# JuliaGraphics/Hikari.jl

Hardware: AMD Instinct MI355X
Metric: Mrays/s (higher is better)
Workload: dtype f32

## Files before the change

hikari.jl_amd/_abi.py:

```python
import ctypes as C

c_f = C.c_float
c_i = C.c_int32
c_u = C.c_uint32
PF = C.POINTER(C.c_float)

HK_OK = 0
HK_ERR_INVALID, HK_ERR_DEVICE, HK_ERR_UNSUPPORTED = -1, -2, -3
HK_UNSET = -100

(HK_MAT_MATTE, HK_MAT_MIRROR, HK_MAT_GLASS, HK_MAT_CONDUCTOR, HK_MAT_COATED_DIFFUSE, HK_MAT_THIN_DIELECTRIC,
 HK_MAT_DIFFUSE_TRANSMISSION, HK_MAT_COATED_DIFFUSE_TRANSMISSION, HK_MAT_COATED_CONDUCTOR, HK_MAT_MIX,
 HK_MAT_FALLBACK) = range(11)
HK_MATF_REMAP_ROUGHNESS, HK_MATF_USE_ETA_K = 1, 2
(HK_LIGHT_POINT, HK_LIGHT_SPOT, HK_LIGHT_DIRECTIONAL, HK_LIGHT_SUN, HK_LIGHT_AMBIENT, HK_LIGHT_ENVIRONMENT,
 HK_LIGHT_DIFFUSE_AREA) = range(7)
HK_SPEC_RGB, HK_SPEC_ILLUMINANT = 0, 1
HK_TONEMAP_NONE, HK_TONEMAP_REINHARD, HK_TONEMAP_REINHARD_EXT, HK_TONEMAP_ACES, HK_TONEMAP_UNCHARTED2, HK_TONEMAP_FILMIC = range(6)
HK_MEDIUM_HOMOGENEOUS, HK_MEDIUM_GRID, HK_MEDIUM_RGB_GRID, HK_MEDIUM_NANOVDB = range(4)
HK_FILTER_BOX, HK_FILTER_TRIANGLE, HK_FILTER_GAUSSIAN, HK_FILTER_MITCHELL, HK_FILTER_LANCZOS = 1, 2, 3, 4, 5
HK_COHERENCE_NONE, HK_COHERENCE_SORTED, HK_COHERENCE_PER_TYPE = 0, 1, 2


class hk_texture(C.Structure):
# ... 20 lines not shown
class hk_medium_interface(C.Structure):
    _fields_ = [("material", c_i), ("inside", c_i), ("outside", c_i)]


class hk_tri_meta(C.Structure):
    _fields_ = [("medium_interface_idx", c_u), ("primitive_index", c_u), ("arealight_flat_idx_1based", c_u)]


class hk_light(C.Structure):
    _fields_ = [("kind", c_i), ("spectrum_kind", c_i), ("i_rgb", c_f * 4), ("poly", c_f * 3), ("illum_scale", c_f),
                ("scale", c_f), ("position", c_f * 3), ("direction", c_f * 3), ("world_to_light", c_f * 16),
                ("light_to_world", c_f * 16), ("cos_total_width", c_f), ("cos_falloff_start", c_f), ("v", c_f * 9),
                ("normal", c_f * 3), ("area", c_f), ("uv", c_f * 6), ("Le", hk_tex_rgba), ("two_sided", c_i),
                ("envmap", c_i)]


class hk_envmap(C.Structure):
    _fields_ = [("width", c_i), ("height", c_i), ("data", PF), ("rotation", c_f * 9), ("nu", c_i), ("nv", c_i),
                ("conditional_func", PF), ("conditional_cdf", PF), ("conditional_func_int", PF), ("marginal_func", PF),
                ("marginal_cdf", PF), ("marginal_func_int", c_f), ("_pad", c_i)]


class hk_medium(C.Structure):
    _fields_ = [("kind", c_i), ("sigma_a", c_f * 4), ("sigma_s", c_f * 4), ("Le", c_f * 4), ("g", c_f),
                ("sigma_scale", c_f), ("Le_scale", c_f), ("bounds_min", c_f * 3), ("bounds_max", c_f * 3),
                ("render_to_medium", c_f * 16), ("medium_to_render", c_f * 16), ("res", c_i * 3), ("density", PF),
                ("sigma_a_grid", PF), ("sigma_s_grid", PF), ("Le_grid", PF), ("majorant_res", c_i * 3),
                ("majorant", PF), ("max_density", c_f), ("nvdb_bytes", C.POINTER(C.c_uint8)), ("nvdb_size", C.c_int64),
                ("root_offset_1based", C.c_int64), ("upper_offset_1based", C.c_int64),
                ("lower_offset_1based", C.c_int64), ("leaf_offset_1based", C.c_int64), ("upper_count", c_i),
                ("lower_count", c_i), ("leaf_count", c_i), ("root_table_size", c_i), ("inv_mat", c_f * 9),
                ("vec", c_f * 3), ("index_bbox_min", c_i * 3), ("index_bbox_max", c_i * 3)]


class hk_scene_desc(C.Structure):
    _fields_ = [("n_triangles", c_i), ("n_materials", c_i), ("n_textures", c_i), ("n_media_interfaces", c_i),
                ("n_lights", c_i), ("n_envmaps", c_i), ("n_media", c_i), ("n_spectra", c_i), ("positions", PF),
                ("normals", PF), ("uvs", PF), ("tangents", PF), ("meta", C.POINTER(hk_tri_meta)),
                ("materials", C.POINTER(hk_material)), ("textures", C.POINTER(hk_texture)),
                ("media_interfaces", C.POINTER(hk_medium_interface)), ("lights", C.POINTER(hk_light)),
                ("envmaps", C.POINTER(hk_envmap)), ("media", C.POINTER(hk_medium)),
                ("spectra", C.POINTER(hk_pl_spectrum))]


class hk_tables(C.Structure):
    _fields_ = [("sobol_matrices", C.POINTER(c_u)), ("sobol_count", c_i), ("rgb2spec_res", c_i), ("cie_x", PF),
                ("cie_y", PF), ("cie_z", PF), ("rgb2spec_scale", PF), ("rgb2spec_coeffs", PF)]


class hk_integrator_params(C.Structure):
    _fields_ = [("max_depth", c_i), ("samples_per_pixel", c_i), ("russian_roulette_depth", c_i), ("regularize", c_i),
                ("material_coherence", c_i), ("max_component_value", c_f), ("filter_type", c_i),
                ("filter_radius", c_f * 2), ("filter_param1", c_f), ("filter_param2", c_f), ("accumulate_f64", c_i),
                ("sampler_seed", c_u), ("samples_per_pass", c_i)]


class hk_postprocess_params(C.Structure):
    _fields_ = [("exposure", c_f), ("tonemap", c_i), ("inv_gamma", c_f), ("apply_gamma", c_i), ("white_point", c_f),
                ("imaging_ratio", c_f), ("apply_wb", c_i), ("wb", c_f * 9), ("mask_escaped", c_i), ("bg", c_f * 3)]


class hk_denoise_params(C.Structure):
    _fields_ = [("iterations", c_i), ("sigma_color", c_f), ("sigma_normal", c_f), ("sigma_depth", c_f), ("use_variance", c_i)]


class hk_camera(C.Structure):
    _fields_ = [("raster_to_camera", c_f * 16), ("camera_to_world", c_f * 16), ("lens_radius", c_f),
                ("focal_distance", c_f), ("shutter_open", c_f), ("shutter_close", c_f), ("dx_camera", c_f * 3),
                ("dy_camera", c_f * 3)]


class hk_stats(C.Structure):
    _fields_ = [("rays_closest", C.c_uint64), ("rays_shadow", C.c_uint64), ("bvh_nodes_visited", C.c_uint64),
                ("tris_tested", C.c_uint64), ("hits_accepted", C.c_uint64), ("path_vertices", C.c_uint64),
                ("medium_collisions", C.c_uint64), ("light_bvh_nodes", C.c_uint64), ("seconds_trace", C.c_double),
                ("seconds_total", C.c_double), ("trace_launches", C.c_uint64), ("trace_nodes", C.c_uint64),
                ("trace_tris", C.c_uint64), ("shadow_nodes", C.c_uint64), ("shadow_tris", C.c_uint64),
                ("shadow_launches", C.c_uint64), ("shade_launches", C.c_uint64), ("seconds_shadow", C.c_double),
                ("seconds_shade", C.c_double), ("seconds_other", C.c_double), ("bytes_algorithmic_trace", C.c_uint64),
                ("bytes_algorithmic_shadow", C.c_uint64), ("bytes_algorithmic_shade", C.c_uint64), ("seconds_media", C.c_double),
                ("track_collisions", C.c_uint64), ("shadow_collisions", C.c_uint64), ("track_dda_steps", C.c_uint64),
                ("shadow_dda_steps", C.c_uint64), ("scatter_vertices", C.c_uint64), ("media_launches", C.c_uint64),
                ("bytes_algorithmic_media", C.c_uint64), ("seconds_select", C.c_double), ("select_launches", C.c_uint64),
                ("fused_passes", C.c_uint64), ("view_cache_hits", C.c_uint64)]


EXPORTED_SYMBOLS = [
    "hk_ctx_create", "hk_ctx_destroy", "hk_last_error", "hk_ctx_set_tables", "hk_scene_create", "hk_scene_destroy",
    "hk_integrator_create", "hk_integrator_destroy", "hk_film_create", "hk_film_destroy", "hk_film_clear", "hk_render",
    "hk_film_read_rgb", "hk_film_read_accum", "hk_film_accum_device_ptr", "hk_sync", "hk_stats_get", "hk_stats_reset",
    "hk_stats_enable_counters", "hk_trace_closest", "hk_test_sobol", "hk_test_camera", "hk_test_uplift",
    "hk_test_light_bvh", "hk_test_bsdf", "hk_film_postprocess", "hk_film_fill_aux", "hk_postprocess", "hk_test_light", "hk_scene_bvh_info", "hk_scene_light_bvh_copy",
    "hk_denoise", "hk_test_mix", "hk_test_medium", "hk_test_trace_lean",
    "hk_render_tile", "hk_comm_create", "hk_comm_unique_id", "hk_comm_create_rank", "hk_comm_destroy", "hk_film_reduce",
    "hk_ctx_set_option", "hk_ctx_get_option", "hk_trim_cache", "hk_flush", "hk_film_read_rgb_async", "hk_film_read_wait",
    "hk_film_pin_host", "hk_film_unpin_host", "hk_scene_set_transform", "hk_scene_update_materials", "hk_scene_update_lights", "hk_scene_update_envmap",
    "hk_film_update_aux", "hk_film_read_aux", "hk_film_present", "hk_film_present_async",
    "hk_scene_update_medium", "hk_scene_medium_copy", "hk_test_medium_bricks",
]
```

hikari.jl_amd/csrc/hk_ctx.cpp:

```cpp
#include "hk_host.h"

thread_local std::string g_err;
SlabCache g_slabs;

namespace hk {
static thread_local const Knobs* tl_knobs = nullptr;
const char* knob(const char* name) {
    if (!tl_knobs) return nullptr;
    auto it = tl_knobs->kv.find(name);
    return it == tl_knobs->kv.end() ? nullptr : it->second.c_str();
}
static const char* const KNOB_NAMES[] = {
    "HK_BATCH_PATHS_M", "HK_BVH_LEAF", "HK_BVH_BINS", "HK_QNODES", "HK_DEBUG_ALLOC", "HK_DELTA_ADVANCE", "HK_DYNAMIC_SEGMENTS", "HK_GREY", "HK_GREY_COMPACT", "HK_GREY_FLAT", "HK_MAX_PATHS_M",
    "HK_MID_LISTS", "HK_MID_PASS_PATHS_M", "HK_NODE_CACHE", "HK_NVDB_DENSE_MB", "HK_OVERLAP", "HK_PIPELINE", "HK_PIPELINE_AFTER", "HK_PIPELINE_MAX_PATHS_M", "HK_PRESELECT",
    "HK_SELECT_MIN_IDLE", "HK_SHADOW_FEED_ROUNDS", "HK_SHADOW_TRACK_BATCH", "HK_SMALL_PASS", "HK_SMALL_PASS_WAVES", "HK_SOBOL_LO_GB", "HK_SOBOL_TABLE_ONLY",
    "HK_STATE_CACHE_GB", "HK_STATE_SLAB", "HK_TICKET_SHARE", "HK_TRACK_ADVANCE", "HK_TRACK_EXTRA_ADVANCE", "HK_TRACK_MIN_PENDING", "HK_TRACK_POOL", "HK_TRACK_REFILL_IDLE",
    "HK_WALK_POOL", "HK_WALK_REFILL_IDLE", "HK_WALK_SPLIT", "HK_WAVES_PER_CU", "HK_READBACK_PIN", "HK_DEFER_EXTERNAL", "HK_SELECT_POOL", "HK_SMALL_PASS_FUSED", "HK_SMALL_PASS_MERGED", "HK_OCC_SCALE", "HK_ESCAPED_UNROLL", "HK_SHADOW_FINAL", "HK_TRI_PACK", "HK_LEAN_RECORDS", "HK_VIEW_CACHE", "HK_MAJORANT_BLOCK_VOXELS"};
static bool known_knob(const char* name) {
    for (const char* k : KNOB_NAMES)
        if (std::strcmp(k, name) == 0) return true;
    return false;
}
}
KnobScope::KnobScope(const hk::Knobs* k) : prev(hk::tl_knobs) { hk::tl_knobs = k; }
KnobScope::~KnobScope() { hk::tl_knobs = prev; }

void quiesce(hk_ctx* c) {
    if (!c) return;
    (void)hipStreamSynchronize(c->stream);
    if (c->aux) (void)hipStreamSynchronize(c->aux);
    for (auto& l : c->lanes)
        if (l.stream) (void)hipStreamSynchronize(l.stream);
}
int join_lanes(hk_ctx* c) {
    if (!c) return HK_OK;
    if (int e = flush_pending(c)) return e;
    if (!c->lanes_dirty) return HK_OK;
    for (auto& l : c->lanes)
        if (l.done) HIP_TRY(hipStreamWaitEvent(c->stream, l.done, 0));
    c->lanes_dirty = false;
    c->film_chain = false;
    if (c->have_span) HIP_TRY(hipEventRecord(c->ev_end, c->stream));
    return HK_OK;
}
hipEvent_t get_event(hk_ctx* c) {
    if (!c->event_pool.empty()) {
        hipEvent_t e = c->event_pool.back();
        c->event_pool.pop_back();
        return e;
    }
    hipEvent_t e;
    (void)hipEventCreate(&e);
    return e;
}
DCamera make_camera(const hk_camera& c) {
    DCamera d;
    std::memcpy(d.r2c, c.raster_to_camera, 64);
    std::memcpy(d.c2w, c.camera_to_world, 64);
    d.lens_radius = c.lens_radius;
    d.focal_distance = c.focal_distance;
    d.shutter_open = c.shutter_open;
    d.shutter_close = c.shutter_close;
    return d;
}

extern "C" const char* hk_last_error(void) { return g_err.c_str(); }

extern "C" int32_t hk_ctx_create(int32_t device_id, void* stream, hk_ctx** out) {
    if (!out) return fail(HK_ERR_INVALID, "out is null");
    int n = 0;
    HIP_TRY(hipGetDeviceCount(&n));
    if (device_id < 0 || device_id >= n) return fail(HK_ERR_INVALID, "bad device id");
    HIP_TRY(hipSetDevice(device_id));
    hk_ctx* c = new hk_ctx();
    c->device = device_id;
    c->stream = (hipStream_t)stream;
    hipDeviceProp_t prop;
    HIP_TRY(hipGetDeviceProperties(&prop, device_id));
    c->n_cu = prop.multiProcessorCount > 0 ? prop.multiProcessorCount : 256;
    c->own_stream_order = stream == nullptr;
    for (const char* name : hk::KNOB_NAMES)
        if (const char* e = std::getenv(name)) c->knobs.kv[name] = e;
    KnobScope knobs(&c->knobs);
    {
        c->waves_per_cu = hk::knob_int_in("HK_WAVES_PER_CU", 1, INT_MAX, 0);
        c->stat_rows = c->n_cu * 32 * 2;
        if (const char* e = hk::knob("HK_OVERLAP")) c->overlap = std::atoi(e) ? 1 : 0;
        else c->overlap = -1;
        if (const char* e = hk::knob("HK_STATE_CACHE_GB"))
            if (std::atol(e) >= 0) g_slabs.cap_bytes = (size_t)std::atol(e) << 30;
    }
    {
        std::vector<DStats> zero((size_t)c->stat_rows);
        std::memset(zero.data(), 0, zero.size() * sizeof(DStats));
        HIP_TRY(c->stats.upload(zero.data(), zero.size() * sizeof(DStats)));
    }
    HIP_TRY(hipEventCreate(&c->ev_begin));
    HIP_TRY(hipEventCreate(&c->ev_end));
// ... 81 lines not shown
    c->h_r2s_coeffs.assign(t->rgb2spec_coeffs, t->rgb2spec_coeffs + nco);
    c->r2s_host.res = res;
    c->r2s_host.scale = c->h_r2s_scale.data();
    c->r2s_host.coeffs = c->h_r2s_coeffs.data();
    HIP_TRY(c->r2s_scale.upload(t->rgb2spec_scale, res * 4));
    HIP_TRY(c->r2s_coeffs.upload(t->rgb2spec_coeffs, nco * 4));
    {
        const size_t R = (size_t)res;
        std::vector<float> pts(3 * R * R * R * 4);
        for (size_t m = 0; m < 3; ++m)
            for (size_t z = 0; z < R; ++z)
                for (size_t y = 0; y < R; ++y)
                    for (size_t x = 0; x < R; ++x) {
                        float* o = &pts[((((m * R + z) * R + y) * R) + x) * 4];
                        for (size_t k = 0; k < 3; ++k) o[k] = t->rgb2spec_coeffs[m + 3 * (z + R * (y + R * (x + R * k)))];
                        o[3] = 0.0f;
                    }
        HIP_TRY(c->r2s_points.upload(pts.data(), pts.size() * 4));
        bool sorted = true;
        for (int i = 1; i < res; ++i)
            if (!(t->rgb2spec_scale[i - 1] <= t->rgb2spec_scale[i])) sorted = false;
        c->tables.rgb2spec_sorted = sorted ? 1 : 0;
    }
    bool closed = true;
    {
        uint32_t col = 0x80000000u;
        for (int b = 0; b < 52; ++b) {
            uint32_t d0 = b < 32 ? (0x80000000u >> b) : 0u;
            if (t->sobol_matrices[b] != d0) closed = false;
            if (b % 32 == 0) col = 0x80000000u;
            if (t->sobol_matrices[52 + b] != col) closed = false;
            col ^= col >> 1;
        }
    }
    c->tables.sobol = closed ? nullptr : c->sobol.as<uint32_t>();
    c->tables.cie = c->cie.as<float>();
    c->tables.rgb2spec_scale = c->r2s_scale.as<float>();
    c->tables.rgb2spec_coeffs = c->r2s_coeffs.as<float>();
    c->tables.rgb2spec_res = res;
    c->tables.rgb2spec_points = c->r2s_points.as<float4>();
    c->have_tables = true;
    c->tables_epoch++;
    return HK_OK;
}

extern "C" int32_t hk_sync(hk_ctx* c) {
    if (!c) return fail(HK_ERR_INVALID, "null ctx");
    HIP_TRY(hipSetDevice(c->device));
    if (int e = join_lanes(c)) return e;
    HIP_TRY(hipStreamSynchronize(c->stream));
    if (c->aux) HIP_TRY(hipStreamSynchronize(c->aux));
    return HK_OK;
}
extern "C" int32_t hk_stats_enable_counters(hk_ctx* c, int32_t flags) {
    if (!c) return fail(HK_ERR_INVALID, "null ctx");
    if (int e = join_lanes(c)) return e;
    c->count_nodes = (flags & 1) ? 1 : 0;
    c->time_kernels = (flags & 2) ? 1 : 0;
    return HK_OK;
}
extern "C" int32_t hk_stats_reset(hk_ctx* c) {
    if (!c) return fail(HK_ERR_INVALID, "null ctx");
    HIP_TRY(hipSetDevice(c->device));
    if (int e = join_lanes(c)) return e;
    HIP_TRY(hipStreamSynchronize(c->stream));
    HIP_TRY(hipMemset(c->stats.p, 0, (size_t)c->stat_rows * sizeof(DStats)));
    for (auto& l : c->lanes)
        if (l.stats.p) HIP_TRY(hipMemset(l.stats.p, 0, (size_t)c->stat_rows * sizeof(DStats)));
    for (auto& e : c->trace_events) {
        c->event_pool.push_back(e.first);
        c->event_pool.push_back(e.second);
    }
    c->trace_events.clear();
    for (auto& v : c->class_events) {
        for (auto& e : v) {
            c->event_pool.push_back(e.first);
            c->event_pool.push_back(e.second);
        }
        v.clear();
    }
    c->seconds_trace = c->seconds_total = 0.0;
    c->trace_launches = c->shadow_launches = c->shade_launches = c->media_launches = c->select_launches = 0;
    c->fused_passes = c->view_cache_hits = 0;
    c->have_span = false;
    return HK_OK;
}
extern "C" int32_t hk_stats_get(hk_ctx* c, hk_stats* out) {
    if (!c || !out) return fail(HK_ERR_INVALID, "null argument");
    HIP_TRY(hipSetDevice(c->device));
    if (int e = join_lanes(c)) return e;
    HIP_TRY(hipStreamSynchronize(c->stream));
    DStats h{};
    {
        std::vector<const void*> blocks{c->stats.p};
        for (const auto& l : c->lanes)
            if (l.stats.p) blocks.push_back(l.stats.p);
        std::vector<DStats> rows((size_t)c->stat_rows * blocks.size());
        for (size_t b = 0; b < blocks.size(); ++b)
            HIP_TRY(hipMemcpy(rows.data() + b * (size_t)c->stat_rows, blocks[b], (size_t)c->stat_rows * sizeof(DStats), hipMemcpyDeviceToHost));
        for (const DStats& r : rows) {
            h.rays_closest += r.rays_closest;
            h.rays_shadow += r.rays_shadow;
            h.nodes += r.nodes;
            h.tris += r.tris;
            h.hits += r.hits;
            h.vertices += r.vertices;
            h.collisions += r.collisions;
            h.light_nodes += r.light_nodes;
            h.sh_nodes += r.sh_nodes;
            h.sh_tris += r.sh_tris;
            h.sh_collisions += r.sh_collisions;
            h.nvdb_collisions += r.nvdb_collisions;
            h.sh_nvdb_collisions += r.sh_nvdb_collisions;
            h.dda_steps += r.dda_steps;
            h.sh_dda_steps += r.sh_dda_steps;
            h.scatter_vertices += r.scatter_vertices;
            h.sc_light_nodes += r.sc_light_nodes;
#ifdef HK_DEBUG_UTIL
            for (int k = 0; k < 32; ++k) h.dbg[k] += r.dbg[k];
#endif
        }
#ifdef HK_DEBUG_UTIL
        for (int k = 0; k < 16; ++k)
            if (h.dbg[2 * k]) std::fprintf(stderr, "HK_DEBUG_UTIL[%d]: %.3f of %llu lane-slots\n", k, (double)h.dbg[2 * k + 1] / (double)h.dbg[2 * k], h.dbg[2 * k]);
#endif
    }
    double tr = 0.0;
    for (auto& e : c->trace_events) {
        float ms = 0.0f;
        if (hipEventElapsedTime(&ms, e.first, e.second) == hipSuccess) tr += ms * 1e-3;
    }
    double total = 0.0;
    if (c->have_span) {
        float ms = 0.0f;
        if (hipEventElapsedTime(&ms, c->ev_begin, c->ev_end) == hipSuccess) total = ms * 1e-3;
    }
    std::memset(out, 0, sizeof *out);
    out->rays_closest = h.rays_closest;
    out->rays_shadow = h.rays_shadow;
    out->bvh_nodes_visited = h.nodes;
    out->tris_tested = h.tris;
    out->hits_accepted = h.hits;
    out->path_vertices = h.vertices;
    out->medium_collisions = h.collisions + h.sh_collisions;
    out->track_collisions = h.collisions;
    out->shadow_collisions = h.sh_collisions;
    out->track_dda_steps = h.dda_steps;
    out->shadow_dda_steps = h.sh_dda_steps;
    out->scatter_vertices = h.scatter_vertices;
    out->light_bvh_nodes = h.light_nodes + h.sc_light_nodes;
    out->seconds_trace = tr;
    out->seconds_total = total;
    out->trace_launches = c->trace_launches;
    out->trace_nodes = h.nodes;
    out->trace_tris = h.tris;
    out->shadow_nodes = h.sh_nodes;
    out->shadow_tris = h.sh_tris;
    out->bvh_nodes_visited = h.nodes + h.sh_nodes;
    out->tris_tested = h.tris + h.sh_tris;
    out->shadow_launches = c->shadow_launches;
    out->shade_launches = c->shade_launches;
    out->media_launches = c->media_launches;
    double cls[6] = {0, 0, 0, 0, 0, 0};
    for (int k = 1; k < 6; ++k)
        for (auto& e : c->class_events[k]) {
            float ms = 0.0f;
            if (hipEventElapsedTime(&ms, e.first, e.second) == hipSuccess) cls[k] += ms * 1e-3;
        }
    out->seconds_shadow = cls[1];
    out->seconds_shade = cls[2] + cls[5];
    out->seconds_other = cls[3];
    out->seconds_media = cls[4];
    out->seconds_select = cls[5];
    out->select_launches = c->select_launches;
    out->fused_passes = c->fused_passes;
    out->view_cache_hits = c->view_cache_hits;
    {
        const uint64_t hits_closest = h.hits < h.rays_closest ? h.hits : h.rays_closest;
        out->bytes_algorithmic_trace = h.rays_closest * (32 + 16) + 64 * h.nodes + 36 * h.tris + 96 * hits_closest;
        out->bytes_algorithmic_shadow = h.rays_shadow * (32 + 16) + 64 * h.sh_nodes + 36 * h.sh_tris;
        out->bytes_algorithmic_shade = h.vertices * (2 * 104 + 64 + 96) + 60 * h.light_nodes;
        out->bytes_algorithmic_media = h.collisions * 36 + h.nvdb_collisions * (84 - 36) + 4 * h.dda_steps + h.scatter_vertices * (2 * 104 + 96) + 60 * h.sc_light_nodes;
        out->bytes_algorithmic_shadow += h.sh_collisions * 36 + h.sh_nvdb_collisions * (84 - 36) + 4 * h.sh_dda_steps;
    }
    return HK_OK;
}
```

hikari.jl_amd/csrc/hk_device.h:

```cpp
#pragma once
#include <hip/hip_runtime.h>
#include <math.h>
#include <stdint.h>

#include "hk_types.h"

#include "hk_nanovdb.h"

#define HKD __device__ __forceinline__

namespace hkd {

static constexpr float PI_F = 3.14159265358979323846f;
static constexpr float INF_F = __builtin_huge_valf();

struct v3 {
    float x, y, z;
};
struct v2 {
    float x, y;
};
HKD v3 mk3(float x, float y, float z) { return v3{x, y, z}; }
HKD v2 mk2(float x, float y) { return v2{x, y}; }
HKD v3 operator+(v3 a, v3 b) { return mk3(a.x + b.x, a.y + b.y, a.z + b.z); }
// ... 238 lines not shown
    return murmur64a_words<2>(w);
}
struct SobolCtx {
    int px, py;
    int pix_slot, x0, y0, tiles_x;
    int sample_idx;
    const uint32_t* mats;
    const uint2* hi;
    const uint16_t* lo;
    int lo_rows;
    uint32_t lo_row_stride;
    int hi_rows, hi_stride;
    int log2_spp, n_digits;
    uint32_t seed;
};
HKD void sobol_ctx_tables(SobolCtx& c, const DSobol& s, const uint32_t* mats, int sample_idx, int pix_slot, int k) {
    c.sample_idx = sample_idx;
    c.pix_slot = pix_slot;
    c.mats = mats;
    const bool cached = s.hi_table != nullptr && pix_slot >= 0 && ((unsigned)sample_idx >> s.log2_spp) == 0u;
    c.hi = cached ? s.hi_table + pix_slot : nullptr;
    const bool low = cached && s.lo_table != nullptr && k >= 0 && (unsigned)(s.lo_offset + k) < (unsigned)s.lo_count;
    c.lo = low ? s.lo_table + ((size_t)pix_slot * s.lo_count + (size_t)(s.lo_offset + k)) : nullptr;
    c.lo_rows = low ? s.lo_rows : 0;
    c.lo_row_stride = (uint32_t)s.hi_stride * (uint32_t)s.lo_count;
    c.hi_rows = s.hi_rows;
    c.hi_stride = s.hi_stride;
    c.log2_spp = s.log2_spp;
    c.n_digits = s.n_base4_digits;
    c.seed = s.seed;
}
HKD SobolCtx sobol_ctx(const DSobol& s, const uint32_t* mats, int px, int py, int sample_idx, int pix_slot = -1, int k = -1) {
    SobolCtx c;
    c.px = px;
    c.py = py;
    c.x0 = c.y0 = 0;
    c.tiles_x = 1;
    sobol_ctx_tables(c, s, mats, sample_idx, pix_slot, k);
    return c;
}
HKD SobolCtx sobol_ctx_slot(const DSobol& s, const uint32_t* mats, int x0, int y0, int tiles_x, int pix_slot, int k, int sample_idx) {
    SobolCtx c;
    c.px = c.py = 0;
    c.x0 = x0;
    c.y0 = y0;
    c.tiles_x = tiles_x;
    sobol_ctx_tables(c, s, mats, sample_idx, pix_slot, k);
    return c;
}
HKD uint64_t sobol_morton_base(const SobolCtx& c) {
    int px = c.px, py = c.py;
    if (px == 0) {
        const int tile = c.pix_slot >> 6, l = c.pix_slot & 63;
        const int ty = tile / c.tiles_x, tx = tile - ty * c.tiles_x;
        px = c.x0 + tx * 8 + (l & 7) + 1;
        py = c.y0 + ty * 8 + (l >> 3) + 1;
    }
    const uint64_t m = (left_shift2((uint64_t)(uint32_t)py) << 1) | left_shift2((uint64_t)(uint32_t)px);
    return (m << c.log2_spp) | (uint64_t)(int64_t)c.sample_idx;
}
template <bool TABLE_ONLY = false>
HKD uint64_t sobol_index(const SobolCtx& c, int dim) {
    const int row = sobol_row(dim);
    if (TABLE_ONLY) return ((uint64_t)c.hi[(size_t)row * c.hi_stride].x << c.log2_spp) | (uint64_t)c.lo[(size_t)row * c.lo_row_stride];
    if (c.hi != nullptr && row >= 0 && row < c.hi_rows) {
        const uint2 e = c.hi[(size_t)row * c.hi_stride];
        if (row < c.lo_rows) return ((uint64_t)e.x << c.log2_spp) | (uint64_t)c.lo[(size_t)row * c.lo_row_stride];
        return zsobol_sample_index_cached(sobol_morton_base(c), dim, c.log2_spp, e.x, e.y);
    }
    return zsobol_sample_index(sobol_morton_base(c), dim, c.log2_spp, c.n_digits);
}
template <bool TABLE_ONLY = false>
HKD float sobol_1d(const SobolCtx& c, int dim) {
    uint64_t idx = sobol_index<TABLE_ONLY>(c, dim);
    uint32_t h = (uint32_t)zsobol_hash(dim + 1, c.seed);
    return sobol_sample(idx, 0, h, c.mats);
}
template <bool TABLE_ONLY = false>
HKD v2 sobol_2d(const SobolCtx& c, int dim) {
    uint64_t idx = sobol_index<TABLE_ONLY>(c, dim);
    uint64_t bits = zsobol_hash(dim + 2, c.seed);
    return mk2(sobol_sample(idx, 0, (uint32_t)bits, c.mats), sobol_sample(idx, 1, (uint32_t)(bits >> 32), c.mats));
}

HKD float jl_sin_kernel(double y) {
    const double S1 = -0.16666666641626524, S2 = 0.008333329385889463, S3 = -0.00019839334836096632, S4 = 2.718311493989822e-6;
    double z = y * y, w = z * z;
    double r = S3 + z * S4, s = z * y;
    return (float)((y + s * (S1 + z * S2)) + s * w * r);
}
HKD float jl_cos_kernel(double y) {
    const double C0 = -0.499999997251031, C1 = 0.04166662332373906, C2 = -0.001388676377460993, C3 = 2.439044879627741e-5;
    double z = y * y, w = z * z;
    double r = C2 + z * C3;
    return (float)(((1.0 + z * C0) + w * C1) + (w * z) * r);
}
HKD int jl_rem_pio2(float x, double& y) {
    const double PI = 3.141592653589793;
    const double xd = (double)x, ax = fabs(xd);
    if (ax <= PI * 5 / 4) {
        if (ax <= PI * 3 / 4) {
            y = x > 0 ? xd - PI / 2 : xd + PI / 2;
            return x > 0 ? 1 : -1;
        }
        y = x > 0 ? xd - PI : xd + PI;
        return x > 0 ? 2 : -2;
    }
    if (ax <= PI * 9 / 4) {
        if (ax <= PI * 7 / 4) {
            y = x > 0 ? xd - 3 * (PI / 2) : xd + 3 * (PI / 2);
            return x > 0 ? 3 : -3;
        }
        y = x > 0 ? xd - 2 * PI : xd + 2 * PI;
        return x > 0 ? 4 : -4;
    }
    const double fn = rint(xd * 6.36619772367581382433e-01);
    const double r = xd - fn * 1.57079631090164184570e+00, w = fn * 1.58932547735281966916e-08;
    y = r - w;
    return (int)fn;
}
HKD void jl_sincos(float x, float& s, float& c) {
    const float ax = fabsf(x);
    if (ax < 0.7853982f) {
        s = ax < 0.00034526698f ? x : jl_sin_kernel((double)x);
        c = ax < 0.00024414062f ? 1.0f : jl_cos_kernel((double)x);
        return;
    }
    if (!(ax < 2.1e8f)) {
        s = sinf(x);
        c = cosf(x);
        return;
    }
    double y;
    const int n = jl_rem_pio2(x, y) & 3;
    const float sk = jl_sin_kernel(y), ck = jl_cos_kernel(y);
    s = n == 0 ? sk : (n == 1 ? ck : (n == 2 ? -sk : -ck));
    c = n == 0 ? ck : (n == 1 ? -sk : (n == 2 ? -ck : sk));
}

HKD v2 concentric_sample_disk(v2 u) {
    float ox = 2.0f * u.x - 1.0f, oy = 2.0f * u.y - 1.0f;
    float sx = ox + 1.0e-10f, sy = oy + 1.0e-10f;
    bool xl = fabsf(ox) > fabsf(oy);
    float r = xl ? ox : oy;
    float theta = xl ? ((oy / sx) * PI_F) / 4.0f : PI_F / 2.0f - ((ox / sy) * PI_F) / 4.0f;
    float st, ct;
    jl_sincos(theta, st, ct);
    return mk2(r * ct, r * st);
}
HKD v3 cosine_sample_hemisphere(v2 u) {
    v2 d = concentric_sample_disk(u);
    float z = sqrtf(maxf(0.0f, 1.0f - d.x * d.x - d.y * d.y));
    return mk3(d.x, d.y, z);
}

HKD float atanh_sampler(float x) { return 0.34657359027997264f * __builtin_amdgcn_logf((1.0f + x) * __builtin_amdgcn_rcpf(1.0f - x)); }
HKD float cosh_sampler(float y) {
    const float e = __builtin_amdgcn_exp2f(1.4426950408889634f * y);
    return 0.5f * (e + __builtin_amdgcn_rcpf(e));
}
HKD float visible_wavelengths_pdf(float l) {
    if (l < 360.0f || l > 830.0f) return 0.0f;
    float c = cosh_sampler(0.0072f * (l - 538.0f));
    return 0.0039398042f / (c * c);
}
HKD float sample_visible_wavelength(float u) { return 538.0f - 138.888889f * atanh_sampler(0.85691062f - 1.82750197f * u); }
// ... 254 lines not shown
}
HKD void filter_sample(const DFilter& f, v2 u, float& px, float& py, float& weight) {
    if (f.type == HK_FILTER_BOX) {
        px = lerpf(-f.rx, f.rx, u.x);
        py = lerpf(-f.ry, f.ry, u.y);
        weight = 1.0f;
        return;
    }
    if (f.type == HK_FILTER_TRIANGLE) {
        px = sample_tent(u.x, f.rx);
        py = sample_tent(u.y, f.ry);
        weight = 1.0f;
        return;
    }
    int ny = f.ny, nx = f.nx;
    int o = clampi(find_interval20(f.marginal_cdf, u.y, ny), 1, ny);
    float du = u.y - f.marginal_cdf[o - 1];
    float diff = f.marginal_cdf[o] - f.marginal_cdf[o - 1];
    du = diff > 0.0f ? du / diff : 0.0f;
    float pdf_y = f.func_integral > 0.0f ? f.marginal_func[o - 1] / f.func_integral : 0.0f;
    py = lerpf(f.dmin_y, f.dmax_y, ((float)(o - 1) + du) / (float)ny);
    float row_integral = f.marginal_func[o - 1];
    const float* row = f.conditional_cdf + (size_t)(o - 1) * (nx + 1);
    int ox = clampi(find_interval20(row, u.x, nx), 1, nx);
    float dux = u.x - row[ox - 1];
    float diffx = row[ox] - row[ox - 1];
    dux = diffx > 0.0f ? dux / diffx : 0.0f;
    float fval = f.func[(size_t)(o - 1) * nx + (ox - 1)];
    float pdf_x = row_integral > 0.0f ? fval / row_integral : 0.0f;
    px = lerpf(f.dmin_x, f.dmax_x, ((float)(ox - 1) + dux) / (float)nx);
    float pdf = pdf_x * pdf_y;
    weight = pdf > 0.0f ? fval / pdf : 0.0f;
}
HKD v3 xform_point(const float* m, v3 p) {
    float x = m[0] * p.x + m[1] * p.y + m[2] * p.z + m[3];
    float y = m[4] * p.x + m[5] * p.y + m[6] * p.z + m[7];
    float z = m[8] * p.x + m[9] * p.y + m[10] * p.z + m[11];
    float w = m[12] * p.x + m[13] * p.y + m[14] * p.z + m[15];
    if (w == 1.0f) return mk3(x, y, z);
    float inv = 1.0f / w;
    return mk3(x * inv, y * inv, z * inv);
}
HKD v3 xform_vector(const float* m, v3 v) {
    return mk3(m[0] * v.x + m[1] * v.y + m[2] * v.z, m[4] * v.x + m[5] * v.y + m[6] * v.z, m[8] * v.x + m[9] * v.y + m[10] * v.z);
}
HKD void generate_ray(const DCamera& cam, v2 film, v2 lens, float time_u, v3& ro, v3& rd, float& time) {
    v3 pc = xform_point(cam.r2c, mk3(film.x, film.y, 0.0f));
    v3 o = mk3(0.0f, 0.0f, 0.0f);
    v3 d = normalize(pc);
    if (cam.lens_radius > 0) {
        v2 dsk = concentric_sample_disk(lens);
        float plx = cam.lens_radius * dsk.x, ply = cam.lens_radius * dsk.y;
        float t = -cam.focal_distance / d.z;
        v3 pf = o + d * t;
        o = mk3(plx, ply, 0.0f);
        d = normalize(pf - o);
    }
    time = lerpf(cam.shutter_open, cam.shutter_close, time_u);
    ro = xform_point(cam.c2w, o);
    rd = normalize(xform_vector(cam.c2w, d));
}

HKD bool intersect_triangle(v3 o, v3 d, float t_max, v3 v0, v3 e1, v3 e2, float& t, float& u, float& v) {
    v3 p = cross(d, e2);
    float det = dot(e1, p);
    if (det == 0.0f) return false;
    float inv = 1.0f / det;
    v3 s = o - v0;
    u = dot(s, p) * inv;
    if (!(u >= 0.0f) || u > 1.0f) return false;
    v3 q = cross(s, e1);
    v = dot(d, q) * inv;
    if (!(v >= 0.0f) || u + v > 1.0f) return false;
    t = dot(e2, q) * inv;
    return t > 0.0f && t < t_max;
}

struct HitRec {
    float t;
    int prim;
    float u, v;
};

struct RaySlab {
    float ix, iy, iz, ox, oy, oz, eps3;
};
HKD RaySlab ray_slab(v3 o, v3 d) {
    RaySlab r;
    r.ix = clampf(1.0f / d.x, -1e30f, 1e30f), r.iy = clampf(1.0f / d.y, -1e30f, 1e30f), r.iz = clampf(1.0f / d.z, -1e30f, 1e30f);
    r.ox = -o.x * r.ix, r.oy = -o.y * r.iy, r.oz = -o.z * r.iz;
    r.eps3 = 3.0f * (2.4e-7f * fmaxf(fmaxf(fabsf(r.ix) < 1e30f ? fabsf(r.ox) : 0.0f, fabsf(r.iy) < 1e30f ? fabsf(r.oy) : 0.0f), fabsf(r.iz) < 1e30f ? fabsf(r.oz) : 0.0f));
    return r;
}
HKD RaySlab ray_slab_grid(const DScene& sc, v3 o, v3 d) {
    RaySlab r = ray_slab(o, d);
    r.ox = fmaf(sc.q_base[0], r.ix, r.ox), r.oy = fmaf(sc.q_base[1], r.iy, r.oy), r.oz = fmaf(sc.q_base[2], r.iz, r.oz);
    r.ix *= sc.q_cell[0], r.iy *= sc.q_cell[1], r.iz *= sc.q_cell[2];
    return r;
}
typedef float hk_f2 __attribute__((ext_vector_type(2)));
typedef float hk_f4v __attribute__((ext_vector_type(4)));
typedef int hk_i2v __attribute__((ext_vector_type(2)));
typedef __attribute__((address_space(3))) hk_f4v lds_float4;
typedef __attribute__((address_space(3))) hk_i2v lds_int2;
struct NodeCache {
    const lds_float4* box;
    const lds_int2* child;
    int nc;
    const lds_float4* tri;
    int nt;
};
template <int NC = 0, bool QN = false>
HKD void node_step(const DScene& sc, const RaySlab& rs, float t_best, int* __restrict__ stack, int lane, int& cur, int& sp, const NodeCache& cache = NodeCache()) {
    float4 A, B, C;
    int c0, c1;
    if (QN && !(NC > 0 && cur < cache.nc)) {
        const uint4* qp = reinterpret_cast<const uint4*>(sc.qnodes) + 2 * (size_t)cur;
        const uint4 P = qp[0], Q = qp[1];
        A = make_float4((float)(P.x & 0xffffu), (float)(P.x >> 16), (float)(P.y & 0xffffu), (float)(P.y >> 16));
        B = make_float4((float)(P.z & 0xffffu), (float)(P.z >> 16), (float)(P.w & 0xffffu), (float)(P.w >> 16));
        C = make_float4((float)(Q.x & 0xffffu), (float)(Q.x >> 16), (float)(Q.y & 0xffffu), (float)(Q.y >> 16));
        c0 = (int)Q.z, c1 = (int)Q.w;
    } else if (NC > 0 && cur < cache.nc) {
        const hk_f4v a = cache.box[cur], b = cache.box[NC + cur], c = cache.box[2 * NC + cur];
        const hk_i2v ch = cache.child[cur];
        A = make_float4(a.x, a.y, a.z, a.w), B = make_float4(b.x, b.y, b.z, b.w), C = make_float4(c.x, c.y, c.z, c.w);
        c0 = ch.x, c1 = ch.y;
        asm volatile("" : "+v"(c0));
    } else {
        const float4* np = reinterpret_cast<const float4*>(sc.nodes) + 4 * (size_t)cur;
        A = np[0], B = np[1], C = np[2];
        const float4 D = np[3];
        c0 = __float_as_int(D.x), c1 = __float_as_int(D.y);
    }
    const hk_f2 IX = {rs.ix, rs.ix}, IY = {rs.iy, rs.iy}, IZ = {rs.iz, rs.iz}, OX = {rs.ox, rs.ox}, OY = {rs.oy, rs.oy}, OZ = {rs.oz, rs.oz};
    const hk_f2 x0 = __builtin_elementwise_fma((hk_f2){A.x, A.y}, IX, OX), y0 = __builtin_elementwise_fma((hk_f2){A.z, A.w}, IY, OY);
    const hk_f2 z0 = __builtin_elementwise_fma((hk_f2){B.x, B.y}, IZ, OZ), x1 = __builtin_elementwise_fma((hk_f2){B.z, B.w}, IX, OX);
    const hk_f2 y1 = __builtin_elementwise_fma((hk_f2){C.x, C.y}, IY, OY), z1 = __builtin_elementwise_fma((hk_f2){C.z, C.w}, IZ, OZ);
    const float n0 = fmaxf(fmaxf(fminf(x0.x, x0.y), fminf(y0.x, y0.y)), fmaxf(fminf(z0.x, z0.y), 0.0f));
    const float f0 = fminf(fminf(fmaxf(x0.x, x0.y), fmaxf(y0.x, y0.y)), fminf(fmaxf(z0.x, z0.y), t_best));
    const float n1 = fmaxf(fmaxf(fminf(x1.x, x1.y), fminf(y1.x, y1.y)), fmaxf(fminf(z1.x, z1.y), 0.0f));
    const float f1 = fminf(fminf(fmaxf(x1.x, x1.y), fmaxf(y1.x, y1.y)), fminf(fmaxf(z1.x, z1.y), t_best));
    const bool h0 = n0 <= fmaf(f0, 1.00003f, rs.eps3);
    const bool h1 = n1 <= fmaf(f1, 1.00003f, rs.eps3);
    const bool both = h0 && h1, any = h0 || h1;
    const bool first0 = n0 <= n1;
    const bool pick0 = h0 & (!h1 | first0);
    const int near_c = pick0 ? c0 : c1;
    if (both) stack[sp * 64 + lane] = pick0 ? c1 : c0;
    sp += both ? 1 : 0;
    const bool pop = !any && sp > 0;
    sp -= pop ? 1 : 0;
    int popped = (int)0x80000000;
    if (pop) popped = stack[sp * 64 + lane];
    cur = any ? near_c : popped;
}

template <int MODE, bool COUNT, int NC = 0, int NT = 0>
HKD HitRec traverse(const DScene& sc, v3 o, v3 d, float t_max, int* __restrict__ stack, int lane, unsigned& n_nodes, unsigned& n_tris, bool& opaque_hit,
                    const NodeCache& cache = NodeCache()) {
    HitRec best;
    best.t = t_max;
    best.prim = -1;
    best.u = best.v = 0.0f;
    opaque_hit = false;
    if (sc.n_tris == 0) return best;
    const RaySlab rs = ray_slab(o, d);
    int sp = 0;
    int cur = sc.root_ref;
    const int DONE = (int)0x80000000;
    while (cur != DONE) {
        for (;;) {
            const unsigned long long in_nodes = __ballot(cur >= 0);
            if (in_nodes == 0ull) break;
// ... 1266 lines not shown
```

hikari.jl_amd/csrc/hk_host.h:

```cpp
#pragma once
#include <hip/hip_runtime.h>

#include <climits>
#include <cstddef>
#include <cmath>
#include <cstdio>
#include <cstdlib>
#include <cstring>
#include <limits>
#include <map>
#include <memory>
#include <mutex>
#include <string>
#include <unordered_map>
#include <vector>

#include "bvh_build.h"
#include "hikari_mi355x.h"
#include "hk_launch.h"
#include "hk_nanovdb.h"
#include "hk_types.h"

#pragma GCC visibility push(hidden)

// ... 70 lines not shown
    void trim(int dev) {
        std::vector<void*> drop;
        {
            std::lock_guard<std::mutex> g(m);
            for (int i = (int)free_list.size() - 1; i >= 0; --i)
                if (dev < 0 || free_list[i].dev == dev) {
                    drop.push_back(free_list[i].p);
                    free_list.erase(free_list.begin() + i);
                }
        }
        for (void* q : drop) (void)hipFree(q);
    }
};
extern SlabCache g_slabs;
struct DevBuf {
    void* p = nullptr;
    size_t bytes = 0;
    int slab_dev = -1;
    void release() {
        if (p && slab_dev >= 0) {
            g_slabs.give(slab_dev, p, bytes);
        } else if (p)
            (void)hipFree(p);
        p = nullptr, bytes = 0, slab_dev = -1;
    }
    ~DevBuf() { release(); }
    hipError_t alloc(size_t n) {
        release();
        bytes = n;
        if (n == 0) return hipSuccess;
        hipError_t e = hipMalloc(&p, n);
        if (e != hipSuccess) {
            (void)hipGetLastError();
            g_slabs.trim(-1);
            e = hipMalloc(&p, n);
        }
        if (e != hipSuccess) p = nullptr, bytes = 0;
        return e;
    }
    hipError_t alloc_slab(int dev, size_t n) {
        release();
        size_t got = 0;
        if (void* q = g_slabs.take(dev, n, got)) {
            p = q, bytes = got, slab_dev = dev;
            return hipSuccess;
        }
        const hipError_t e = alloc(n);
        if (e == hipSuccess) slab_dev = dev;
        return e;
    }
    hipError_t upload(const void* src, size_t n) {
        hipError_t e = alloc(n ? n : 4);
        if (e != hipSuccess) return e;
        if (n) e = hipMemcpy(p, src, n, hipMemcpyHostToDevice);
        return e;
    }
    template <class T>
    T* as() const {
        return reinterpret_cast<T*>(p);
    }
};

struct hk_ctx {
    int device = 0;
    hk::Knobs knobs;
    bool own_stream_order = true;
    hipStream_t stream = nullptr;
    hipStream_t aux = nullptr;
    hipEvent_t ev_fork = nullptr, ev_join = nullptr;
    int overlap = -1;
    int small_streak = 0;
    int n_cu = 256;
    int waves_per_cu = 0;
    int stat_rows = 8192;
    DevBuf sobol, cie, r2s_scale, r2s_coeffs, r2s_points, stats;
    DTables tables{};
    bool have_tables = false;
    unsigned tables_epoch = 0;
    std::vector<float> h_r2s_scale, h_r2s_coeffs;
    hk::RGB2Spec r2s_host;
    int count_nodes = 0, time_kernels = 0;
    unsigned long long fused_passes = 0;
    unsigned long long view_cache_hits = 0;
    std::vector<std::pair<hipEvent_t, hipEvent_t>> trace_events;
    std::vector<std::pair<hipEvent_t, hipEvent_t>> class_events[6];
    uint64_t shadow_launches = 0, shade_launches = 0, media_launches = 0, select_launches = 0;
    std::vector<hipEvent_t> event_pool;
    hipEvent_t ev_begin = nullptr, ev_end = nullptr;
    bool have_span = false;
    double seconds_trace = 0.0, seconds_total = 0.0;
    uint64_t trace_launches = 0;
    DStats host_stats{};
    struct Lane {
        hipStream_t stream = nullptr;
        hipEvent_t done = nullptr;
        DevBuf stats;
    };
    enum { MAX_LANES = 16 };
    Lane lanes[MAX_LANES];
    int next_lane = 0;
    struct Pending {
        bool active = false;
        hk_scene* sc = nullptr;
        hk_integrator* I = nullptr;
        hk_film* film = nullptr;
        hk_camera cam{};
        int first = 0, n = 0, stride = 1, x0 = 0, y0 = 0, x1 = 0, y1 = 0, calls = 0;
    } pending;
    bool lanes_dirty = false;
    bool film_chain = false;
    hipEvent_t ev_main = nullptr, ev_film = nullptr;
};

void quiesce(hk_ctx* c);
int flush_pending(hk_ctx* c);
int join_lanes(hk_ctx* c);
hipEvent_t get_event(hk_ctx* c);
DCamera make_camera(const hk_camera& c);

struct hk_scene {
    hk_ctx* ctx = nullptr;
    DevBuf nodes, qnodes, leaf_tris, positions, normals, uvs, tangents, meta, tri_shade, materials, textures, spectra, mis, lights, lnodes, trails, infinite;
    DevBuf envmaps;
    DevBuf media;
    DScene d{};
    uint32_t kinds_mask = 0;
    int n_materials = 0;
    int bvh_nodes = 0, bvh_leaf_tris = 0, bvh_depth = 0;
    hk::LightBVH lbvh;
    std::vector<hk_material> h_materials;
    std::vector<hk_light> h_lights;
    std::vector<DEnvMap> h_envmaps;
    int n_textures = 0, n_spectra = 0;
    std::vector<int> level_start;
    DevBuf base_pos, base_nrm, base_tan, slot_of_prim;
    bool have_base = false;
    bool qnodes_built = false;
    enum { XF_BLOCK = 1024 };
    std::vector<float> block_box;
    struct Xf {
        int end;
        bool identity;
        float m[12];
    };
    std::map<int, Xf> xf;
    struct Staging {
        void* host = nullptr;
        size_t bytes = 0;
        hipEvent_t ev = nullptr;
    };
    std::vector<Staging> staging;
    struct Medium {
        hk_medium rec{};
        DMedium d{};
        DevBuf *majorant = nullptr, *maj_zero = nullptr, *density = nullptr, *rgb[3] = {nullptr, nullptr, nullptr};
        DevBuf *nvdb = nullptr, *blocks = nullptr, *bricks = nullptr;
    };
    std::vector<Medium> h_media;
    std::vector<std::unique_ptr<DevBuf>> owned;
    DevBuf& own() {
        owned.emplace_back(new DevBuf());
        return *owned.back();
    }
    ~hk_scene() {
        for (auto& st : staging) {
            if (st.ev) (void)hipEventSynchronize(st.ev), (void)hipEventDestroy(st.ev);
            if (st.host) (void)hipHostFree(st.host);
        }
    }
};
void bake_material(const hk::RGB2Spec& t, const hk_material& m, DMaterial& o);
bool material_alpha_tested(const hk_material& m);
void bake_light(const hk::RGB2Spec& r2s, const hk_light& l, DLight& o);
std::string check_medium_record(const hk_medium& m);
void bake_medium_fields(const hk::RGB2Spec& r2s, const hk_medium& m, DMedium& o);
struct NvdbPlan {
    int nvb_min[3] = {0, 0, 0}, nvb_dim[3] = {0, 0, 0};
    float background = 0.0f;
    long long total = 0;
    std::vector<uint2> table;
    bool bricks = false;
    void fill(DMedium& o) const;
};
int plan_nanovdb(const hk_medium& m, NvdbPlan& p);
struct MediaClasses {
    int media_mask = 0, all_grey = 0, grey_pool = 0, grey_bricks = 0;
};
MediaClasses classify_media(const std::vector<DMedium>& dmed, int n_media);
inline size_t light_table_capacity(int n_lights) { return n_lights > 0 ? (size_t)n_lights : 1; }

struct hk_film {
    hk_ctx* ctx = nullptr;
    int width = 0, height = 0;
    bool f64 = false;
    DevBuf own;
    void* accum = nullptr;
    bool external = false;
    bool exposed = false;
    DevBuf readback;
    float* staging[2] = {nullptr, nullptr};
    int staging_next = 0, staging_last = -1;
    bool read_in_flight = false;
    hipEvent_t ev_read = nullptr;
    void* last_out = nullptr;
    void* pinned_user = nullptr;
    bool pinned_explicit = false;
    void* pin_failed = nullptr;
    DevBuf guides, albedo;
    DevBuf frame[2], variance;
    bool have_aux = false;
};

struct hk_integrator {
    hk_ctx* ctx = nullptr;
    hk_integrator_params p{};
    DFilter filter{};
    DevBuf f_func, f_mcdf, f_mfunc, f_ccdf;
    DPathState st{};
    std::vector<std::unique_ptr<DevBuf>> bufs;
    int st_capacity = 0, st_depth = 0, st_media = -1;
    DPathGen cam_gen{};
    bool cam_unfit = false;
    std::string view_key;
    bool mid_pass = false;
    int slab_mode = 0;
    void* slab_base = nullptr;
    size_t slab_off = 0;
    DevBuf sobol_table;
    int sobol_rows = 0, sobol_stride = 0, sobol_log2 = -1, sobol_digits = -1, sobol_x0 = -1, sobol_y0 = -1, sobol_tiles_x = -1;
    DevBuf sobol_lo;
    int lo_rows = 0, lo_base = -1, lo_sample_stride = -1, lo_count = 0;
    struct StateSet {
        DPathState st{};
        std::vector<std::unique_ptr<DevBuf>> bufs;
        int st_capacity = 0, st_depth = 0, st_media = -1;
        DPathGen cam_gen{};
        bool cam_unfit = false;
        std::string view_key;
    };
    std::vector<StateSet> lane_sets;
    void swap_set(StateSet& o) {
        std::swap(st, o.st);
        std::swap(bufs, o.bufs);
        std::swap(st_capacity, o.st_capacity);
        std::swap(st_depth, o.st_depth);
        std::swap(st_media, o.st_media);
        std::swap(cam_gen, o.cam_gen);
        std::swap(cam_unfit, o.cam_unfit);
        std::swap(view_key, o.view_key);
    }
};
int ceil_log2(long v);
DSobol make_sobol(const hk_integrator_params& p, int w, int h);

struct hk_comm {
    std::vector<hk_ctx*> ctxs;
    std::vector<void*> comms;
    int world = 1;
};

#pragma GCC visibility pop
```

hikari.jl_amd/csrc/hk_kernels.hip:

```cpp
#include <hip/hip_runtime.h>
#include <type_traits>
#include <cstdlib>
#include <cstdio>

#include "hikari_mi355x.h"
#include "hk_device.h"

using namespace hkd;

namespace {

__device__ __forceinline__ int lane_id() { return (int)(threadIdx.x & 63); }

struct WaveQ {
    uint32_t* base;
    int count;
};
__device__ __forceinline__ int global_wave() {
    const int w = (int)(threadIdx.x >> 6), b = (int)blockIdx.x;
    if (blockDim.x == 1024 && (gridDim.x & 7) == 0) return ((((b >> 3) * 4 + (w >> 2)) * 8 + (b & 7)) << 2) + (w & 3);
    if (blockDim.x == 512 && (gridDim.x & 7) == 0) return ((((b >> 3) * 2 + (w >> 2)) * 8 + (b & 7)) << 2) + (w & 3);
    return b * (int)(blockDim.x >> 6) + w;
}
__device__ __forceinline__ int physical_waves() { return (int)(gridDim.x * (blockDim.x >> 6)); }
// ... 278 lines not shown
        slot_to_pixel(fr, pix, px, py, inside);
        const int dim = sobol_row_dim(row);
        uint64_t m = (left_shift2((uint64_t)(uint32_t)(py + 1)) << 1) | left_shift2((uint64_t)(uint32_t)(px + 1));
        uint64_t morton = m << sob.log2_spp;
        const int pow2 = sob.log2_spp & 1;
        const uint64_t dmix = 0x55555555ull * (uint64_t)(int64_t)dim;
        uint64_t hi = zsobol_digits(morton, dmix, pow2, sob.n_base4_digits - 1, zsobol_first_pixel_digit(sob.log2_spp));
        table[i] = make_uint2((uint32_t)(hi >> sob.log2_spp), zsobol_top_perms(morton, dmix, sob.log2_spp));
    }
}

struct SegQueues {
    int n;
    int depth[HK_MAX_KINDS + 6], q[HK_MAX_KINDS + 6];
};
#define HK_LIST_SPLIT 8
__global__ void __launch_bounds__(1024) k_segment_lists(DPathState st, SegQueues qs) {
    __shared__ int wave_total[16];
    const int d = qs.depth[blockIdx.x], q = qs.q[blockIdx.x];
    const int* __restrict__ cnt = st.counters + (size_t)(d * Q_COUNT + q) * st.n_waves;
    int* __restrict__ out = st.seg_list + (size_t)(d * Q_COUNT + q) * st.n_waves;
    const int lane = (int)(threadIdx.x & 63), wave = (int)(threadIdx.x >> 6);
    const int share = (st.n_waves + HK_LIST_SPLIT - 1) / HK_LIST_SPLIT;
    const int begin = (int)blockIdx.y * share < st.n_waves ? (int)blockIdx.y * share : st.n_waves, end = begin + share < st.n_waves ? begin + share : st.n_waves;
    int mine = 0;
    for (int i = (int)threadIdx.x; i < begin; i += 1024) mine += cnt[i] != 0 ? 1 : 0;
    for (int off = 32; off > 0; off >>= 1) mine += __shfl_down(mine, off);
    if (lane == 0) wave_total[wave] = mine;
    __syncthreads();
    int base = 0;
    for (int w = 0; w < 16; ++w) base += wave_total[w];
    for (int start = begin; start < end; start += 1024) {
        const int i = start + (int)threadIdx.x;
        const bool nz = i < end && cnt[i] != 0;
        const unsigned long long m = __ballot(nz);
        __syncthreads();
        if (lane == 0) wave_total[wave] = __popcll(m);
        __syncthreads();
        int before = 0, total = 0;
        for (int w = 0; w < 16; ++w) {
            const int t = wave_total[w];
            before += w < wave ? t : 0;
            total += t;
        }
        if (nz) out[base + before + __popcll(m & ((1ull << lane) - 1ull))] = i;
        base += total;
    }
    if (blockIdx.y == HK_LIST_SPLIT - 1 && threadIdx.x == 0) st.seg_list_n[d * Q_COUNT + q] = base;
}

__global__ void __launch_bounds__(256) k_sobol_lo_table(DSobol sob, DFrame fr, uint16_t* table, int rows, int base, int stride, int count) {
    const long groups = count >> 4;
    const long total = (long)rows * fr.n_pixels_padded * groups;
    const uint32_t mask = (1u << sob.log2_spp) - 1u;
    const int pow2 = sob.log2_spp & 1;
    for (long i = (long)blockIdx.x * blockDim.x + threadIdx.x; i < total; i += (long)gridDim.x * blockDim.x) {
        const long rp = i / groups;
        const int q = (int)(i - rp * groups);
        const int row = (int)(rp / fr.n_pixels_padded), pix = (int)(rp - (long)row * fr.n_pixels_padded);
        int px, py;
        bool inside;
        slot_to_pixel(fr, pix, px, py, inside);
        const int dim = sobol_row_dim(row);
        const uint64_t dmix = 0x55555555ull * (uint64_t)(int64_t)dim;
        const uint64_t m = ((left_shift2((uint64_t)(uint32_t)(py + 1)) << 1) | left_shift2((uint64_t)(uint32_t)(px + 1))) << sob.log2_spp;
        const uint2 e = sob.hi_table[(size_t)row * sob.hi_stride + pix];
        uint32_t v[16];
        const int s0 = base + 16 * q * stride;
        if (stride == 1 && pow2 == 0 && (s0 & 15) == 0 && sob.log2_spp >= 4) {
            const uint64_t morton = m | (uint64_t)(uint32_t)s0;
            const uint32_t upper = (uint32_t)zsobol_sample_index_cached(morton, dim, sob.log2_spp, e.x, e.y) & mask & ~15u;
            const int p1 = zsobol_perm_index(morton >> 4, dmix);
            for (int d1 = 0; d1 < 4; ++d1) {
                const uint32_t hi = upper | ((uint32_t)zsobol_permute_digit(p1, d1) << 2);
                const int p0 = zsobol_perm_index((morton | ((uint64_t)d1 << 2)) >> 2, dmix);
                for (int d0 = 0; d0 < 4; ++d0) v[4 * d1 + d0] = hi | (uint32_t)zsobol_permute_digit(p0, d0);
            }
        } else {
            for (int t = 0; t < 16; ++t) v[t] = (uint32_t)zsobol_sample_index_cached(m | (uint64_t)(uint32_t)(s0 + t * stride), dim, sob.log2_spp, e.x, e.y) & mask;
        }
        uint4* out = reinterpret_cast<uint4*>(table) + 2 * i;
        out[0] = make_uint4(v[0] | (v[1] << 16), v[2] | (v[3] << 16), v[4] | (v[5] << 16), v[6] | (v[7] << 16));
        out[1] = make_uint4(v[8] | (v[9] << 16), v[10] | (v[11] << 16), v[12] | (v[13] << 16), v[14] | (v[15] << 16));
    }
}

__device__ __forceinline__ void camera_body(const DPathState& st, const DFrame& fr, const DTables& T, const DFilter& flt, const DCamera& cam, const DSobol& sob, const SegTickets& src) {
    const int total = fr.n_pixels_padded * fr.samples_in_pass;
    const int n_chunks = total >> 6;
    const DPathGen g0 = st.gen_cam;
    HK_FOR_EACH_SEGMENT_FROM(gw, st, src) {
    WavePos out{0};
    const size_t seg = (size_t)gw * st.wave_cap;
    for (int chunk = gw; chunk < n_chunks; chunk += st.n_waves) {
        int slot = chunk * 64 + lane_id();
        int pix, k;
        split_slot(fr, (uint32_t)slot, pix, k);
        int px, py;
        bool active;
        slot_to_pixel(fr, pix, px, py, active);
        const size_t p = seg + (size_t)wp_push(out, active);
        if (active) {
            int sample_idx = fr.first_sample + k * fr.sample_stride;
            int x = px + 1, y = py + 1;
            SobolCtx sc = sobol_ctx(sob, T.sobol, x, y, sample_idx, pix, k);
            float wavelength_u = sobol_1d(sc, 1);
            v2 jit = sobol_2d(sc, 3);
            float time_u = 0.0f;
            v2 lens = mk2(0.0f, 0.0f);
            if (cam.lens_radius > 0) {
                time_u = sobol_1d(sc, 4);
                lens = sobol_2d(sc, 6);
            }
            float fx, fy, fw;
            filter_sample(flt, jit, fx, fy, fw);
            S4 lambda, pdf;
            sample_wavelengths_visible(wavelength_u, lambda, pdf);
            v2 pfilm = mk2((float)x + 0.5f + fx, (float)fr.height - (float)y + 1.0f + 0.5f + fy);
            v3 ro, rd;
            float time;
            generate_ray(cam, pfilm, lens, time_u, ro, rd, time);
            if (!st.const_origin || p == seg) stream_st(&g0.ray_o[p], make_float4(ro.x, ro.y, ro.z, INF_F));
            stream_st(&g0.ray_d[p], make_float4(rd.x, rd.y, rd.z, (st.compact && !fr.implicit_ones) ? 1.0f : 0.0f));
            st_lambda(g0, p, lambda);
            if (!fr.implicit_ones) {
                st4(&g0.beta[p], s4(1.0f));
                st_ru_rl(g0, p, s4(1.0f), s4(1.0f), st.compact != 0);
            }
            st_meta(st, g0, p, (uint32_t)(*st.initial_medium + 1) << 16, (uint32_t)slot);
            stream_st(&st.lambda_s[slot], lambda);
            stream_st(&st.L[slot], s4(0.0f));
            stream_st(&st.filter_w[slot], fw);
        }
    }
    if (lane_id() == 0) *count_ptr(st, 0, Q_RAY, gw) = out.count;
    }
}
__global__ void __launch_bounds__(256) k_camera(DPathState st, DFrame fr, DTables T, DFilter flt, DCamera cam, DSobol sob, int initial_medium) {
    camera_body(st, fr, T, flt, cam, sob, seg_open(st, ticket_ptr(st, st.ticket_rows - 1, TK_CAMERA), st.dynamic_segments != 0, -1, 0));
}

template <int NC, int BLOCK, bool QN = false>
HKD NodeCache node_cache_fill(const DScene& sc, float4* __restrict__ box, int2* __restrict__ child) {
    NodeCache c;
    c.box = (const lds_float4*)box, c.child = (const lds_int2*)child;
    c.tri = nullptr, c.nt = 0;
    c.nc = sc.n_nodes < NC ? sc.n_nodes : NC;
    if (NC > 0) {
        for (int i = threadIdx.x; i < c.nc; i += BLOCK) {
            if (QN) {
                const uint4* qp = reinterpret_cast<const uint4*>(sc.qnodes) + 2 * (size_t)i;
                const uint4 P = qp[0], Q = qp[1];
                box[i] = make_float4((float)(P.x & 0xffffu), (float)(P.x >> 16), (float)(P.y & 0xffffu), (float)(P.y >> 16));
                box[NC + i] = make_float4((float)(P.z & 0xffffu), (float)(P.z >> 16), (float)(P.w & 0xffffu), (float)(P.w >> 16));
                box[2 * NC + i] = make_float4((float)(Q.x & 0xffffu), (float)(Q.x >> 16), (float)(Q.y & 0xffffu), (float)(Q.y >> 16));
                child[i] = make_int2((int)Q.z, (int)Q.w);
                continue;
            }
            const float4* np = reinterpret_cast<const float4*>(sc.nodes) + 4 * (size_t)i;
            const float4 D = np[3];
            box[i] = np[0], box[NC + i] = np[1], box[2 * NC + i] = np[2];
            child[i] = make_int2(__float_as_int(D.x), __float_as_int(D.y));
        }
        __syncthreads();
    }
    return c;
// ... 1428 lines not shown
}

__device__ __forceinline__ bool escaped_one(const DPathState& st, const DScene& sc, const DTables& T, const DPathGen& g, bool ones, uint32_t slot, S4& fin, uint32_t& pslot, int depth) {
    const uint2 meta = ld_meta(st, g, slot, depth);
    pslot = meta.y;
    S4 lambda = ld_lambda(st, g, slot, meta.y);
    S4 Le = s4(0.0f);
    v3 rd = mk3(0, 0, 1);
    bool have_dir = false;
    for (int li = 0; li < sc.n_lights; ++li) {
        const DLight& l = sc.lights[li];
        if (l.kind == HK_LIGHT_AMBIENT) Le = Le + l.scale * light_spectrum(l, lambda);
        if (l.kind == HK_LIGHT_ENVIRONMENT) {
            if (!have_dir) {
                float4 D = g.ray_d[slot];
                rd = mk3(D.x, D.y, D.z);
                have_dir = true;
            }
            float4 t = env_eval(sc.envmaps[l.Le_tex], rd);
            Le = Le + eval_illuminant(coef_illuminant(T, t.x * l.Le_rgba[0], t.y * l.Le_rgba[1], t.z * l.Le_rgba[2]), lambda);
        }
    }
    S4 beta = ld_throughput(g.beta, slot, ones);
    S4 contribution = beta * Le;
    if (is_black(contribution)) return false;
    uint32_t fl = meta.x;
    int pdepth = (int)(fl & 0xff);
    bool specular = (fl >> 8) & 1u;
    S4 r_u = ld_ru(g, slot, ones, st.compact != 0);
    if (pdepth == 0 || specular)
        fin = contribution / average(r_u);
    else {
        float choice = sc.n_lights > 0 ? 1.0f / (float)sc.n_lights : 0.0f;
        float light_pdf = 0.0f;
        if (sc.n_envmaps > 0)
            for (int li = 0; li < sc.n_lights; ++li) {
                const DLight& l = sc.lights[li];
                light_pdf = light_pdf + (l.kind == HK_LIGHT_ENVIRONMENT ? env_pdf_li(sc.envmaps[l.Le_tex], rd) : 0.0f);
            }
        S4 rl = ld_rl(g, slot, ones, st.compact != 0) * choice * light_pdf;
        float den = average(r_u + rl);
        fin = den > 1e-10f ? contribution / den : contribution / average(r_u);
    }
    return true;
}
template <int UNROLL>
__device__ __forceinline__ void escaped_body(const DPathState& st, const DScene& sc, const DTables& T, int depth, int implicit_ones, const SegTickets& src) {
    HK_FOR_EACH_SEGMENT_FROM(gw, st, src) {
    const uint32_t* __restrict__ queue = st.escaped_q + (size_t)gw * st.wave_cap;
    const int n = *count_ptr(st, depth, Q_ESCAPED, gw);
    const DPathGen g = gen_at(st, depth);
    const bool ones = depth == 0 && implicit_ones;
    int i = lane_id();
    if (UNROLL == 2) {
        for (; i + 64 < n; i += 128) {
            const uint32_t slot0 = queue[i], slot1 = queue[i + 64];
            S4 fin0, fin1;
            uint32_t p0, p1;
            const bool a0 = escaped_one(st, sc, T, g, ones, slot0, fin0, p0, depth);
            const bool a1 = escaped_one(st, sc, T, g, ones, slot1, fin1, p1, depth);
            S4 L0 = s4(0.0f), L1 = s4(0.0f);
            if (a0) L0 = ld4(&st.L[p0]);
            if (a1) L1 = ld4(&st.L[p1]);
            if (a0) st4(&st.L[p0], L0 + fin0);
            if (a1) st4(&st.L[p1], L1 + fin1);
        }
    }
    for (; i < n; i += 64) {
        S4 fin;
        uint32_t pslot;
        if (escaped_one(st, sc, T, g, ones, queue[i], fin, pslot, depth)) st4(&st.L[pslot], ld4(&st.L[pslot]) + fin);
    }
    }
}
template <int UNROLL>
__global__ void __launch_bounds__(256) k_escaped(DPathState st, DScene sc, DTables T, int depth, int implicit_ones) {
    escaped_body<UNROLL>(st, sc, T, depth, implicit_ones, seg_open(st, ticket_ptr(st, depth, TK_ESCAPED), st.dynamic_segments != 0, depth, Q_ESCAPED));
}

#define HK_PRESELECT_MIN 64
#ifndef HK_SELECT_MIN_IDLE
#define HK_SELECT_MIN_IDLE 24
#endif
template <bool FT>
__global__ void __launch_bounds__(256) k_light_select(DPathState st, DScene sc, DTables T, DFrame fr, DSobol sob, int depth, uint32_t kinds_mask, int min_idle, DStats* stats) {
    const int lane = lane_id();
    const unsigned long long lt_mask = (1ull << lane) - 1ull;
    unsigned n_lnodes = 0;
    const DPathGen g = gen_at(st, depth);
    const int base_dim = 6 + 7 * depth;
    const int ninf = sc.num_infinite_lights, nbvh = sc.num_bvh_lights;
    const bool has_bvh = nbvh > 0;
    const float p_inf = (float)ninf / (float)(ninf + (has_bvh ? 1 : 0));
    HK_FOR_EACH_WAVE_SEGMENT(gw, st, ticket_ptr(st, depth, TK_SELECT), depth, Q_RAY) {
        int kind = -1, n = 0, cursor = 0;
        const uint32_t* __restrict__ queue = st.mat_q;
        bool more = true;
        bool busy = false, done = false;
        uint32_t slot = 0, bits = 0, child = 0;
        int ni = 1, res_light = 0, lvl = 0;
        float ub = 0.0f, pmf = 0.0f, res_pmf = 0.0f;
        v3 p = mk3(0, 0, 0), nn = mk3(0, 0, 1);
        for (;;) {
            const unsigned long long run_m = __ballot(busy && !done);
            if (run_m == 0ull || (64 - __popcll(run_m) >= min_idle && (cursor < n || more))) {
                if (busy && done) {
                    st.sel_light[slot] = make_uint2((uint32_t)res_light, __float_as_uint(res_pmf));
                    busy = false;
                }
                while (more && cursor >= n) {
                    ++kind;
                    while (kind < HK_MAX_KINDS && !(kinds_mask & (1u << kind))) ++kind;
                    if (kind >= HK_MAX_KINDS) {
                        more = false;
                        break;
                    }
                    queue = st.mat_q + ((size_t)kind * st.n_waves + gw) * st.wave_cap;
                    n = *count_ptr(st, depth, Q_MAT0 + kind, gw);
                    cursor = 0;
                }
                const unsigned long long want = __ballot(!busy);
                const int avail = n - cursor;
                const int rank = __popcll(want & lt_mask);
                if (!busy && rank < avail) {
                    slot = queue[cursor + rank];
                    const float4 H = st.hit[slot], O = ld_ray_o(st, g, slot, depth, (size_t)gw * st.wave_cap), D = g.ray_d[slot];
                    const Surface sf = surface_at(sc, __float_as_int(H.y), H.z, H.w, mk3(O.x, O.y, O.z), mk3(D.x, D.y, D.z), H.x);
                    p = sf.pi;
                    nn = sf.ns;
                    int pix, k;
                    split_slot(fr, ld_meta(st, g, slot, depth).y, pix, k);
                    const SobolCtx sctx = sobol_ctx_slot(sob, T.sobol, fr.x0, fr.y0, fr.tiles_x, pix, k, fr.first_sample + k * fr.sample_stride);
                    const float u = sobol_1d<FT>(sctx, base_dim + 1);
                    busy = true;
                    done = true;
                    res_light = 0;
                    res_pmf = 0.0f;
                    if (ninf + nbvh > 0) {
                        if (ninf > 0 && u < p_inf) {
                            const float ur = u / p_inf;
                            int idx = (int)floorf(ur * (float)ninf);
                            idx = (idx < ninf - 1 ? idx : ninf - 1) + 1;
                            res_pmf = p_inf / (float)ninf;
                            res_light = sc.infinite_lights[idx - 1];
                        } else if (has_bvh) {
                            ub = ninf > 0 ? minf((u - p_inf) / (1.0f - p_inf), 0.99999994f) : minf(u, 0.99999994f);
                            pmf = 1.0f - p_inf;
                            ni = 1;
                            const DLightNode root = load_light_node(sc.lnodes, 0);
                            bits = root.bits, child = root.child1_or_light;
                            lvl = 0;
                            done = false;
                        }
                    }
                }
                const int want_n = __popcll(want);
                cursor += want_n < avail ? want_n : (avail > 0 ? avail : 0);
                if (__ballot(busy) == 0ull) {
                    if (cursor >= n && !more) break;
                    continue;
                }
            }
            if (busy && !done) {
                if (lvl >= 64) {
                    res_light = 0;
                    res_pmf = 0.0f;
                    done = true;
                } else if (bits & 2u) {
                    res_pmf = pmf;
                    res_light = (int)child;
                    done = true;
                } else {
                    ++lvl;
                    const DLightNode n0 = load_light_node(sc.lnodes, (int)child), n1 = load_light_node(sc.lnodes, (int)child + 1);
                    const float c0 = node_importance(n0, p, nn);
                    const float c1 = node_importance(n1, p, nn);
                    n_lnodes += 2;
                    if (c0 == 0.0f && c1 == 0.0f) {
                        res_light = 0;
                        res_pmf = 0.0f;
                        done = true;
                    } else {
                        const float p0 = c0 / (c0 + c1);
                        if (ub < p0) {
                            pmf *= p0;
                            ub = ub / p0;
                            bits = n0.bits, child = n0.child1_or_light;
                        } else {
                            pmf *= (1.0f - p0);
                            ub = (ub - p0) / (1.0f - p0);
                            bits = n1.bits, child = n1.child1_or_light;
                        }
                    }
                }
            }
        }
    }
    stats += global_wave();
    wave_add(&stats->light_nodes, n_lnodes);
}

#ifndef HK_SELECT_NTOP
#define HK_SELECT_NTOP 512
#endif
#ifndef HK_SELECT_BLOCK
#define HK_SELECT_BLOCK 256
#endif
template <int NTOP>
HKD DLightNode lds_light_node(const lds_float4* top, int i) {
    const hk_f4v a = top[i], b = top[NTOP + i], c = top[2 * NTOP + i], d = top[3 * NTOP + i];
    DLightNode n;
    n.centre[0] = a.x, n.centre[1] = a.y, n.centre[2] = a.z, n.half_diag = a.w;
    n.r2 = b.x, n.w[0] = b.y, n.w[1] = b.z, n.w[2] = b.w;
    n.phi = c.x, n.cos_o = c.y, n.cos_e = c.z, n.sin_o = c.w;
    n.bits = __float_as_uint(d.x), n.child1_or_light = __float_as_uint(d.y);
    n.pad[0] = n.pad[1] = 0u;
    return n;
}
#ifndef HK_SELECT_WAVES
#define HK_SELECT_WAVES 4
#endif
template <bool FT, int BLOCK = HK_SELECT_BLOCK, int NTOP = HK_SELECT_NTOP>
__global__ void __attribute__((amdgpu_flat_work_group_size(BLOCK, BLOCK), amdgpu_waves_per_eu(HK_SELECT_WAVES))) k_light_select_pool(DPathState st, DScene sc, DTables T, DFrame fr, DSobol sob, int depth, uint32_t kinds_mask, DStats* stats) {
    __shared__ uint32_t lds_pool[BLOCK / 64][8][64];
    __shared__ float4 lds_top[NTOP > 0 ? 4 * NTOP : 1];
    uint32_t (*pool)[64] = lds_pool[threadIdx.x >> 6];
    const lds_float4* top = (const lds_float4*)lds_top;
    const int n_top = NTOP > 0 ? (2 * sc.num_bvh_lights < NTOP ? 2 * sc.num_bvh_lights : NTOP) : 0;
    if (NTOP > 0) {
        for (int i = threadIdx.x; i < n_top; i += BLOCK) {
            const float4* q = reinterpret_cast<const float4*>(sc.lnodes + i);
            lds_top[i] = q[0], lds_top[NTOP + i] = q[1], lds_top[2 * NTOP + i] = q[2], lds_top[3 * NTOP + i] = q[3];
        }
        __syncthreads();
    }
    const int lane = lane_id();
    const unsigned long long lt_mask = (1ull << lane) - 1ull;
    unsigned n_lnodes = 0;
    const DPathGen g = gen_at(st, depth);
    const int base_dim = 6 + 7 * depth;
    const int ninf = sc.num_infinite_lights, nbvh = sc.num_bvh_lights;
    const bool has_bvh = nbvh > 0;
    const float p_inf = (float)ninf / (float)(ninf + (has_bvh ? 1 : 0));
    uint32_t root_bits = 2u, root_child = 0u;
    if (has_bvh) {
        const DLightNode root = load_light_node(sc.lnodes, 0);
        root_bits = __builtin_amdgcn_readfirstlane(root.bits), root_child = __builtin_amdgcn_readfirstlane(root.child1_or_light);
    }
    SegStream stream = stream_open(st, ticket_ptr(st, depth, TK_SELECT), false, depth, Q_RAY);
    int gw = -1, kind = HK_MAX_KINDS, n = 0, cursor = 0;
    const uint32_t* __restrict__ queue = st.mat_q;
    bool more = true;
    int pool_n = 0, pool_head = 0;
    bool busy = false;
    uint32_t slot = 0, bits = 0, child = 0;
    int lvl = 0;
    float ub = 0.0f, pmf = 0.0f;
    v3 p = mk3(0, 0, 0), nn = mk3(0, 0, 1);
    for (;;) {
        const unsigned long long free_m = __ballot(!busy);
        if (free_m != 0ull) {
            if (pool_head == pool_n && more) {
                while (more && cursor >= n) {
                    ++kind;
                    while (kind < HK_MAX_KINDS && !(kinds_mask & (1u << kind))) ++kind;
                    if (kind >= HK_MAX_KINDS) {
                        gw = stream_next(stream, st.n_waves);
                        if (gw >= st.n_waves) {
                            more = false;
                            break;
                        }
                        kind = -1;
                        continue;
                    }
                    queue = st.mat_q + ((size_t)kind * st.n_waves + gw) * st.wave_cap;
                    n = *count_ptr(st, depth, Q_MAT0 + kind, gw);
                    cursor = 0;
                }
                pool_n = pool_head = 0;
                if (more) {
                    const int take = n - cursor < 64 ? n - cursor : 64;
                    bool descend = false;
                    uint32_t e = 0;
                    float u_b = 0.0f;
                    v3 sp = mk3(0, 0, 0), sn = mk3(0, 0, 1);
                    if (lane < take) {
                        e = queue[cursor + lane];
                        const float4 H = st.hit[e], O = ld_ray_o(st, g, e, depth, (size_t)gw * st.wave_cap), D = g.ray_d[e];
                        const Surface sf = surface_at(sc, __float_as_int(H.y), H.z, H.w, mk3(O.x, O.y, O.z), mk3(D.x, D.y, D.z), H.x);
                        sp = sf.pi;
                        sn = sf.ns;
                        int pix, k;
                        split_slot(fr, ld_meta(st, g, e, depth).y, pix, k);
                        const SobolCtx sctx = sobol_ctx_slot(sob, T.sobol, fr.x0, fr.y0, fr.tiles_x, pix, k, fr.first_sample + k * fr.sample_stride);
                        const float u = sobol_1d<FT>(sctx, base_dim + 1);
                        int res_light = 0;
                        float res_pmf = 0.0f;
                        if (ninf + nbvh > 0) {
                            if (ninf > 0 && u < p_inf) {
                                const float ur = u / p_inf;
                                int idx = (int)floorf(ur * (float)ninf);
                                idx = (idx < ninf - 1 ? idx : ninf - 1) + 1;
                                res_pmf = p_inf / (float)ninf;
                                res_light = sc.infinite_lights[idx - 1];
                            } else if (has_bvh) {
                                u_b = ninf > 0 ? minf((u - p_inf) / (1.0f - p_inf), 0.99999994f) : minf(u, 0.99999994f);
                                if (root_bits & 2u) {
                                    res_pmf = 1.0f - p_inf;
                                    res_light = (int)root_child;
                                } else
                                    descend = true;
                            }
                        }
                        if (!descend) st.sel_light[e] = make_uint2((uint32_t)res_light, __float_as_uint(res_pmf));
                    }
                    cursor += take;
                    const unsigned long long dm = __ballot(descend);
                    if (descend) {
                        const int at = __popcll(dm & lt_mask);
                        pool[0][at] = e;
                        pool[1][at] = __float_as_uint(sp.x), pool[2][at] = __float_as_uint(sp.y), pool[3][at] = __float_as_uint(sp.z);
                        pool[4][at] = __float_as_uint(sn.x), pool[5][at] = __float_as_uint(sn.y), pool[6][at] = __float_as_uint(sn.z);
                        pool[7][at] = __float_as_uint(u_b);
                    }
                    pool_n = __popcll(dm);
                    __builtin_amdgcn_wave_barrier();
                }
            }
            const int avail = pool_n - pool_head;
            if (avail > 0) {
                const int rank = __popcll(free_m & lt_mask);
                if (!busy && rank < avail) {
                    const int at = pool_head + rank;
                    slot = pool[0][at];
                    p = mk3(__uint_as_float(pool[1][at]), __uint_as_float(pool[2][at]), __uint_as_float(pool[3][at]));
                    nn = mk3(__uint_as_float(pool[4][at]), __uint_as_float(pool[5][at]), __uint_as_float(pool[6][at]));
                    ub = __uint_as_float(pool[7][at]);
                    pmf = 1.0f - p_inf;
                    bits = root_bits, child = root_child;
                    lvl = 0;
                    busy = true;
                }
                const int free_n = __popcll(free_m);
                pool_head += free_n < avail ? free_n : avail;
            }
            if (__ballot(busy) == 0ull) {
                if (!more && pool_head == pool_n) break;
                continue;
            }
        }
        if (busy) {
            int res_light = -1;
            float res_pmf = 0.0f;
            if (lvl >= 64) {
                res_light = 0;
            } else {
                ++lvl;
                DLightNode n0, n1;
                if (NTOP > 0 && (int)child + 1 < n_top) {
                    n0 = lds_light_node<NTOP>(top, (int)child), n1 = lds_light_node<NTOP>(top, (int)child + 1);
                    asm volatile("" : "+v"(n0.bits));
                } else
                    n0 = load_light_node(sc.lnodes, (int)child), n1 = load_light_node(sc.lnodes, (int)child + 1);
                const float c0 = node_importance(n0, p, nn);
                const float c1 = node_importance(n1, p, nn);
                n_lnodes += 2;
                if (c0 == 0.0f && c1 == 0.0f) {
                    res_light = 0;
                } else {
                    const float p0 = c0 / (c0 + c1);
                    if (ub < p0) {
                        pmf *= p0;
                        ub = ub / p0;
                        bits = n0.bits, child = n0.child1_or_light;
                    } else {
                        pmf *= (1.0f - p0);
                        ub = (ub - p0) / (1.0f - p0);
                        bits = n1.bits, child = n1.child1_or_light;
                    }
                    if ((bits & 2u) && lvl < 64) {
                        res_light = (int)child;
                        res_pmf = pmf;
                    }
                }
            }
            if (res_light >= 0) {
                st.sel_light[slot] = make_uint2((uint32_t)res_light, __float_as_uint(res_pmf));
                busy = false;
            }
        }
    }
    stats += global_wave();
    wave_add(&stats->light_nodes, n_lnodes);
}

#ifndef HK_SHADE_WAVES_MATTE
#define HK_SHADE_WAVES_MATTE 4
#endif
#ifndef HK_SHADE_WAVES
#define HK_SHADE_WAVES 3
#endif
template <bool TWO_PLANES, bool SIMPLE>
HKD void shade_emission(const DPathState& st, const DPathGen& g, bool ones, const DScene& sc, const DTables& T, uint32_t slot, unsigned& n_lnodes, int depth, size_t seg) {
    const float4 H = st.hit[slot];
    const float4 O = ld_ray_o(st, g, slot, depth, seg), D = g.ray_d[slot];
    const v3 ro = mk3(O.x, O.y, O.z), rd = mk3(D.x, D.y, D.z);
    const float t_hit = H.x;
    const int prim = __float_as_int(H.y);
    const DTriMeta meta = tri_meta(sc, prim);
    if (meta.arealight <= 0) return;
    const Surface sf = surface_at(sc, prim, H.z, H.w, ro, rd, t_hit);
    const v3 wo = -rd;
    const uint2 pmeta = ld_meta(st, g, slot, depth);
    const S4 lambda = ld_lambda(st, g, slot, pmeta.y);
    const DLight& light = sc.lights[meta.arealight - 1];
    S4 Le = arealight_Le<TWO_PLANES, SIMPLE>(sc, T, light, wo, sf.n, sf.uv, lambda);
    if (is_black(Le)) return;
    const S4 beta = ld_throughput(g.beta, slot, ones), r_u = ld_ru(g, slot, ones, st.compact != 0), r_l = ld_rl(g, slot, ones, st.compact != 0);
    const uint32_t fl = pmeta.x;
    const int pdepth = (int)(fl & 0xff);
    const bool specular_bounce = (fl >> 8) & 1u;
    S4 contribution = beta * Le;
    S4 fin;
    if (pdepth == 0 || specular_bounce)
        fin = contribution / average(r_u);
    else {
        float choice = bvh_pmf(sc, sf.pi, sf.n, (int)meta.arealight, n_lnodes);
        float ct = fabsf(dot(sf.n, normalize(rd)));
        float light_pdf = 0.0f;
        if (ct > 0.0f && sf.area > 0.0f) light_pdf = choice * ((t_hit * t_hit) / (ct * sf.area));
        S4 rl = r_l * light_pdf;
        float den = average(r_u + rl);
        fin = den > 1e-10f ? contribution / den : contribution / average(r_u);
    }
    st4(&st.L[pmeta.y], ld4(&st.L[pmeta.y]) + fin);
}

template <int KIND>
struct ShadeWaves {
    static constexpr int value = (KIND == HK_MAT_COATED_DIFFUSE || KIND == HK_MAT_COATED_DIFFUSE_TRANSMISSION) ? 1 : (KIND == HK_MAT_MATTE ? HK_SHADE_WAVES_MATTE : HK_SHADE_WAVES);
};
#ifndef HK_SHADE_MIN_WAVES
#define HK_SHADE_MIN_WAVES 1
#endif
template <int KIND, bool SIMPLE, bool FT, bool PRE>
__device__ __forceinline__ void shade_body(const DPathState& st, const DScene& sc, const DTables& T, const DFrame& fr, const DSobol& sob, int depth, int first_kind, DStats* stats, const SegTickets& src,
                                           uint32_t* __restrict__ elist) {
    const int lane = lane_id();
    unsigned n_vertices = 0, n_lnodes = 0;
    HK_FOR_EACH_SEGMENT_FROM(gw, st, src) {
    const uint32_t* __restrict__ queue = st.mat_q + ((size_t)KIND * st.n_waves + gw) * st.wave_cap;
    const int n = *count_ptr(st, depth, Q_MAT0 + KIND, gw);
    const DPathGen g = gen_at(st, depth), gn = st.gen[(depth + 1) & 1];
    const size_t seg = (size_t)gw * st.wave_cap;
    const bool ones = depth == 0 && fr.implicit_ones;
    WavePos q_shadow{0}, q_next{0};
    if (!first_kind) {
        q_shadow.count = *count_ptr(st, depth, Q_SHADOW, gw);
        q_next.count = *count_ptr(st, depth + 1, Q_RAY, gw);
    }
    {
        int n_emit = 0;
        for (int base = 0; base < n || n_emit > 0; base += 64) {
            if (base < n) {
                const int i = base + lane;
                const uint32_t cand = i < n ? queue[i] : 0u;
                const bool em = i < n && (st.mat_id[cand] & HK_MAT_EMISSIVE_BIT) != 0;
                const unsigned long long m = __ballot(em);
                if (em) elist[n_emit + __popcll(m & ((1ull << lane) - 1ull))] = cand;
                n_emit += __popcll(m);
                if (n_emit < 64 && base + 64 < n) continue;
            }
            __builtin_amdgcn_fence(__ATOMIC_SEQ_CST, "wavefront");
            const int take = n_emit < 64 ? n_emit : 64;
            if (lane < take) shade_emission<KIND == HK_MAT_MATTE, SIMPLE>(st, g, ones, sc, T, elist[lane], n_lnodes, depth, seg);
            const int rest = n_emit - take;
            const uint32_t moved = lane < rest ? elist[64 + lane] : 0u;
            __builtin_amdgcn_fence(__ATOMIC_SEQ_CST, "wavefront");
            if (lane < rest) elist[lane] = moved;
            n_emit = rest;
        }
    }
    for (int base = 0; base < n; base += 64) {
        int i = base + lane;
        bool active = i < n;
        uint32_t slot = active ? queue[i] : 0u;
        bool push_shadow = false, push_ray = false;
        float4 H = make_float4(0, 0, 0, 0);
        Surface sf;
        v3 wo = mk3(0, 0, 1);
        DTriMeta meta{0u, 0u, 0u};
        S4 lambda = s4(0.0f), beta = s4(0.0f), r_u = s4(0.0f), kd_matte = s4(0.0f);
        uint32_t fl = 0, pslot = 0;
        int pdepth = 0, medium = -1;
        bool any_non_specular = false;
        SobolCtx sctx;
        const int base_dim = 6 + 7 * depth;
        float4 shO = make_float4(0, 0, 0, 0), shD = shO;
        S4 shLd = s4(0.0f), shRu = s4(0.0f), shRl = s4(0.0f);
        if (active) {
            ++n_vertices;
            H = stream_ld(&st.hit[slot]);
            float4 O = ld_ray_o(st, g, slot, depth, seg), D = stream_ld(&g.ray_d[slot]);
            v3 ro = mk3(O.x, O.y, O.z), rd = mk3(D.x, D.y, D.z);
            float t_hit = H.x;
            int prim = __float_as_int(H.y);
            sf = surface_at(sc, prim, H.z, H.w, ro, rd, t_hit);
            wo = -rd;
            meta = tri_meta(sc, prim);
            const uint2 pmeta = ld_meta(st, g, slot, depth);
            lambda = ld_lambda(st, g, slot, pmeta.y);
            if (ones)
                beta = s4(1.0f);
            else {
                const float4 bv = stream_ld(&g.beta[slot]);
                beta = s4(bv.x, bv.y, bv.z, bv.w);
            }
            r_u = ld_ru(g, slot, ones, st.compact != 0);
            fl = pmeta.x;
            pslot = pmeta.y;
            pdepth = (int)(fl & 0xff);
            any_non_specular = (fl >> 9) & 1u;
            medium = (int)(fl >> 16) - 1;

            int pix, k;
            split_slot(fr, pslot, pix, k);
            sctx = sobol_ctx_slot(sob, T.sobol, fr.x0, fr.y0, fr.tiles_x, pix, k, fr.first_sample + k * fr.sample_stride);

            if (KIND == HK_MAT_MATTE) kd_matte = matte_kd<SIMPLE>(sc, T, sc.materials[st.mat_id[slot] & ~HK_MAT_EMISSIVE_BIT], TexCtx(sf.uv, meta.prim_index, H.z, H.w), lambda);
#ifdef HK_ABLATE
            {
                float sink = 0.0f;
                if (HK_ABLATE == 1) {
                    uint32_t ps2 = pslot;
                    int d2 = base_dim;
                    asm volatile("" : "+v"(ps2));
                    asm volatile("" : "+s"(d2));
                    int pix2, k2;
                    split_slot(fr, ps2, pix2, k2);
                    SobolCtx c2 = sobol_ctx_slot(sob, T.sobol, fr.x0, fr.y0, fr.tiles_x, pix2, k2, fr.first_sample + k2 * fr.sample_stride);
                    v2 a = sobol_2d(c2, d2 + 3), b = sobol_2d(c2, d2 + 6);
                    sink = sobol_1d(c2, d2 + 1) + a.x + a.y + b.x + b.y + sobol_1d(c2, d2 + 7);
                }
                if (HK_ABLATE == 2 && sc.n_lights > 0) {
                    float u2 = H.z, pmf2;
                    asm volatile("" : "+v"(u2));
                    unsigned dummy = 0;
                    sink = (float)bvh_sample_light(sc, sf.pi, sf.ns, u2, pmf2, dummy) + pmf2;
                }
                if (HK_ABLATE == 3 && sc.n_lights > 0) {
                    uint32_t li = pslot;
                    asm volatile("" : "+v"(li));
                    LightSample l2 = sample_light(sc, T, sc.lights[li % (uint32_t)sc.n_lights], sf.pi, lambda, mk2(H.z, H.w));
                    sink = l2.pdf + l2.Li.x + l2.Li.w + l2.wi.x + l2.p_light.z;
                }
                if (HK_ABLATE == 4) {
                    S4 l2 = lambda;
                    asm volatile("" : "+v"(l2.x), "+v"(l2.y), "+v"(l2.z), "+v"(l2.w));
                    S4 k2 = matte_kd(sc, T, sc.materials[st.mat_id[slot] & ~HK_MAT_EMISSIVE_BIT], TexCtx(sf.uv, meta.prim_index, H.z, H.w), l2);
                    sink = k2.x + k2.y + k2.z + k2.w;
                }
                if (HK_ABLATE == 5) {
                    float b2 = H.z;
                    asm volatile("" : "+v"(b2));
                    Surface s2 = surface_at(sc, prim, b2, H.w, ro, rd, t_hit);
                    sink = s2.pi.x + s2.n.y + s2.ns.z + s2.uv.x + s2.area;
                }
                if (HK_ABLATE == 6) {
                    v3 w2 = wo;
                    asm volatile("" : "+v"(w2.x), "+v"(w2.y), "+v"(w2.z));
                    float p2;
                    S4 f2 = eval_matte_kd(kd_matte, w2, sf.n, sf.ns, p2);
                    BSDFSample s2 = sample_matte_kd(sc, sc.materials[st.mat_id[slot] & ~HK_MAT_EMISSIVE_BIT], kd_matte, w2, sf.ns, TexCtx(sf.uv, meta.prim_index, H.z, H.w), mk2(H.z, H.w));
                    sink = f2.x + f2.w + p2 + s2.pdf + s2.wi.x + s2.f.y;
                }
                asm volatile("" : : "v"(sink));
            }
#endif

            if (sc.n_lights > 0) {
                const DMaterial& mat = sc.materials[st.mat_id[slot] & ~HK_MAT_EMISSIVE_BIT];
                float light_pmf;
                int light_idx;
                if constexpr (PRE) {
                    const uint2 pre = st.sel_light[slot];
                    light_idx = (int)pre.x;
                    light_pmf = __uint_as_float(pre.y);
                } else {
                    float light_select = sobol_1d<FT>(sctx, base_dim + 1);
                    light_idx = bvh_sample_light(sc, sf.pi, sf.ns, light_select, light_pmf, n_lnodes);
                }
                if (light_idx >= 1 && light_idx <= sc.n_lights && light_pmf > 0.0f) {
                    const DLight& sel = sc.lights[light_idx - 1];
                    v2 u_light = mk2(0.0f, 0.0f);
                    if (sel.kind >= HK_LIGHT_AMBIENT) u_light = sobol_2d<FT>(sctx, base_dim + 3);
                    LightSample ls = sample_light<KIND == HK_MAT_MATTE, SIMPLE>(sc, T, sel, sf.pi, lambda, u_light);
                    if (ls.pdf > 0.0f && !is_black(ls.Li)) {
                        float bsdf_pdf;
                        S4 f = KIND == HK_MAT_MATTE ? eval_matte_kd(kd_matte, wo, ls.wi, sf.ns, bsdf_pdf)
                                                    : eval_bsdf<KIND>(sc, T, mat, wo, ls.wi, sf.ns, TexCtx(sf.uv, meta.prim_index, H.z, H.w), lambda, bsdf_pdf);
                        if (!is_black(f)) {
                            float ct = fabsf(dot(ls.wi, sf.ns));
                            S4 Ld = beta * f * ls.Li * ct;
                            if (!is_black(Ld)) {
                                v3 off = 1e-4f * sf.ns;
                                v3 so = dot(ls.wi, sf.ns) > 0.0f ? sf.pi + off : sf.pi - off;
                                v3 tl = ls.p_light - so;
                                float tmax = sqrtf(dot(tl, tl)) - 1e-3f;
                                float nbp = ls.is_delta ? 0.0f : bsdf_pdf;
                                shO = make_float4(so.x, so.y, so.z, tmax);
                                shD = make_float4(ls.wi.x, ls.wi.y, ls.wi.z, __int_as_float(medium));
                                shLd = Ld;
                                shRu = r_u * nbp;
                                shRl = (r_u * ls.pdf) * light_pmf;
                                push_shadow = true;
                            }
                        }
                    }
                }
            }
        }
        {
            const size_t ps = seg + (size_t)wp_push(q_shadow, push_shadow);
            if (push_shadow && st.sh_final) {
                const S4 mis = s4(shRu.x) * s4(1.0f) + s4(shRl.x) * s4(1.0f);
                shD.w = average(mis);
                stream_st(&st.sh_o[ps], shO);
                stream_st(&st.sh_d[ps], shD);
                stream_st(&st.sh_Ld[ps], shLd);
                stream_st(&st.sh_slot[ps], pslot);
            } else if (push_shadow) {
                stream_st(&st.sh_o[ps], shO);
                stream_st(&st.sh_d[ps], shD);
                stream_st(&st.sh_Ld[ps], shLd);
                if (st.compact) {
#if HK_NT
                    __builtin_nontemporal_store((hk_f2){shRu.x, shRl.x}, (hk_f2*)(reinterpret_cast<float2*>(st.sh_ru) + ps));
#else
                    reinterpret_cast<float2*>(st.sh_ru)[ps] = make_float2(shRu.x, shRl.x);
#endif
                } else
                    st_shadow_weights(st, ps, shRu, shRl);
                stream_st(&st.sh_slot[ps], pslot);
            }
        }
        float4 nO = make_float4(0, 0, 0, 0), nD = nO;
        S4 nb = s4(0.0f), nrl = s4(0.0f);
        uint32_t nflags = 0;
        if (active) {
            int new_depth = pdepth + 1;
            if (new_depth < fr.max_depth) {
                const DMaterial& mat = sc.materials[st.mat_id[slot] & ~HK_MAT_EMISSIVE_BIT];
                const DMediumInterface mi = sc.mis[meta.mi];
                float uc = (KIND == HK_MAT_GLASS || KIND > HK_MAT_CONDUCTOR) && KIND != HK_MAT_FALLBACK ? sobol_1d<FT>(sctx, base_dim + 4) : 0.0f;
                v2 u = (KIND == HK_MAT_MIRROR || KIND == HK_MAT_GLASS || KIND == HK_MAT_THIN_DIELECTRIC) ? mk2(0.0f, 0.0f) : sobol_2d<FT>(sctx, base_dim + 6);
                bool regularize = fr.regularize && any_non_specular;
                BSDFSample s = KIND == HK_MAT_MATTE ? sample_matte_kd<SIMPLE>(sc, mat, kd_matte, wo, sf.ns, TexCtx(sf.uv, meta.prim_index, H.z, H.w), u)
                                                    : sample_bsdf<KIND>(sc, T, mat, wo, sf.ns, TexCtx(sf.uv, meta.prim_index, H.z, H.w), lambda, u, uc, regularize);
                if (s.pdf > 0.0f && !is_black(s.f)) {
                    float ct = fabsf(dot(s.wi, sf.ns));
                    nb = s.is_specular ? beta * s.f : beta * s.f * ct / s.pdf;
                    nrl = s.is_specular ? r_u : r_u / s.pdf;
                    bool cont = true;
                    if (new_depth > 3) {
                        float rr = sobol_1d<FT>(sctx, base_dim + 7);
                        float q = maxf(0.05f, 1.0f - max_component(nb));
                        if (rr < q)
                            cont = false;
                        else
                            nb = nb * (1.0f / (1.0f - q));
                    }
                    if (cont) {
                        int new_medium = (mi.inside != mi.outside) ? (dot(s.wi, sf.n) > 0.0f ? mi.outside : mi.inside) : medium;
                        v3 off = dot(s.wi, sf.n) > 0.0f ? sf.n : -sf.n;
                        v3 no = sf.pi + off * 0.0001f;
                        nO = make_float4(no.x, no.y, no.z, INF_F);
                        nD = make_float4(s.wi.x, s.wi.y, s.wi.z, 0.0f);
                        bool ans = any_non_specular || !s.is_specular;
                        nflags = (uint32_t)new_depth | ((s.is_specular ? 1u : 0u) << 8) | ((ans ? 1u : 0u) << 9) | ((uint32_t)(new_medium + 1) << 16);
                        push_ray = true;
                    }
                }
            }
        }
        {
            const size_t pn = seg + (size_t)wp_push(q_next, push_ray);
            if (push_ray) {
                stream_st(&gn.ray_o[pn], nO);
                if (st.compact) nD.w = nrl.x;
                stream_st(&gn.ray_d[pn], nD);
                stream_st(&gn.beta[pn], nb);
                st_ru_rl(gn, pn, r_u, nrl, st.compact != 0);
                st_lambda(gn, pn, lambda);
                st_meta(st, gn, pn, nflags, pslot);
            }
        }
    }
    if (lane == 0) {
        *count_ptr(st, depth, Q_SHADOW, gw) = q_shadow.count;
        *count_ptr(st, depth + 1, Q_RAY, gw) = q_next.count;
    }
    }
    stats += global_wave();
    wave_add(&stats->vertices, n_vertices);
    wave_add(&stats->light_nodes, n_lnodes);
}
template <int KIND, bool SIMPLE = false, bool FT = false, bool PRE = false>
__global__ void __attribute__((amdgpu_flat_work_group_size(256, 256), amdgpu_waves_per_eu(ShadeWaves<KIND>::value))) k_shade(DPathState st, DScene sc, DTables T, DFrame fr, DSobol sob, int depth, int first_kind, DStats* stats) {
    __shared__ uint32_t emit_list[4 * 128];
    shade_body<KIND, SIMPLE, FT, PRE>(st, sc, T, fr, sob, depth, first_kind, stats, seg_open(st, ticket_ptr(st, depth, TK_SHADE0 + KIND), st.dynamic_segments != 0, depth, Q_MAT0 + KIND),
                                      emit_list + (threadIdx.x >> 6) * 128);
}

template <class W> HKD W wone();
template <> HKD float wone<float>() { return 1.0f; }
template <> HKD S4 wone<S4>() { return s4(1.0f); }
HKD S4 wide(S4 v) { return v; }
HKD S4 wide(float v) { return s4(v); }
HKD bool is_black(float v) { return v == 0.0f; }
template <bool COMPACT>
HKD void shadow_contribute(const DPathState& st, uint32_t rec, S4 T_ray, S4 tr_u, S4 tr_l) {
    if (is_black(T_ray)) return;
    S4 w_u, w_l;
    ld_shadow_weights<COMPACT>(st, rec, w_u, w_l);
    S4 mis = w_u * tr_u + w_l * tr_l;
    float den = average(mis);
    if (den > 1e-10f) {
        S4 fin = ld4(&st.sh_Ld[rec]) * T_ray / den;
        if (!is_black(fin)) {
            const uint32_t pslot = st.sh_slot[rec];
            st4(&st.L[pslot], ld4(&st.L[pslot]) + fin);
        }
    }
}

HKD void shadow_contribute_final(const DPathState& st, uint32_t rec, float den) {
    if (den > 1e-10f) {
        const S4 fin = ld4(&st.sh_Ld[rec]) * s4(1.0f) / den;
        if (!is_black(fin)) {
            const uint32_t pslot = st.sh_slot[rec];
            st4(&st.L[pslot], ld4(&st.L[pslot]) + fin);
        }
    }
}
HKD void shadow_contribute_rt(const DPathState& st, uint32_t rec, S4 T_ray, S4 tr_u, S4 tr_l) {
    if (st.compact)
        shadow_contribute<true>(st, rec, T_ray, tr_u, tr_l);
    else
        shadow_contribute<false>(st, rec, T_ray, tr_u, tr_l);
}

template <bool COUNT, int NC, bool QN = false>
__device__ __forceinline__ void shadow_body(const DPathState& st, const DScene& sc, int depth, DStats* stats, SegStream stream, int* __restrict__ stack, const NodeCache& cache) {
    const int lane = lane_id();
    const unsigned long long lt_mask = (1ull << lane) - 1ull;
    const int DONE = (int)0x80000000;
    unsigned n_nodes = 0, n_tris = 0, n_casts = 0, n_hits = 0;
    HK_DBG_DECL
    uint32_t seg = 0;
    int n = 0, cursor = 0;
    bool more = true;
    bool have = false;
    uint32_t slot = 0;
    float rec_den = 0.0f;
    LaneRay r;
    r.cur = r.pend = DONE;
    for (;;) {
        const unsigned long long run_m = __ballot(have && r.cur != DONE);
        if (run_m == 0ull || (64 - __popcll(run_m) >= HK_TRACE_MIN_IDLE && (cursor < n || more))) {
            if (have && r.cur == DONE) {
                if (r.best.prim < 0) {
                    if (st.sh_final)
                        shadow_contribute_final(st, slot, rec_den);
                    else
                        shadow_contribute<true>(st, slot, s4(1.0f), s4(1.0f), s4(1.0f));
                } else
                    ++n_hits;
                have = false;
            }
            while (more && cursor >= n) {
                const int gw = stream_next(stream, st.n_waves);
                if (gw >= st.n_waves) {
                    more = false;
                    break;
                }
                seg = (uint32_t)gw * (uint32_t)st.wave_cap;
                n = *count_ptr(st, depth, Q_SHADOW, gw);
                cursor = 0;
            }
            const unsigned long long want = __ballot(!have);
// ... 1704 lines not shown
```

hikari.jl_amd/csrc/hk_launch.h:

```cpp
#pragma once
#include "hikari_mi355x.h"
#include "hk_types.h"

namespace hk {

inline bool lean_scene(const DScene& sc) { return sc.all_opaque != 0 && sc.n_media == 0; }
inline int walk_split_mode() { return knob_int("HK_WALK_SPLIT", 0); }

bool grey_compact_ok(const DScene& sc);
bool preselect_lights(const DScene& sc, const DPathState& st);
bool small_pass_fusable(const DScene& sc, uint32_t kinds_mask);

void launch_camera(hipStream_t s, int n_cu, const DPathState& st, const DFrame& fr, const DTables& T, const DFilter& flt, const DCamera& cam, const DSobol& sob, int initial_medium);
void launch_trace(hipStream_t s, int n_cu, const DPathState& st, const DScene& sc, const DTables& T, const DFrame& fr, int depth, DStats* stats);
void launch_shadow(hipStream_t s, int n_cu, const DPathState& st, const DScene& sc, const DTables& T, const DFrame& fr, int depth, DStats* stats);
void launch_escaped(hipStream_t s, int n_cu, const DPathState& st, const DScene& sc, const DTables& T, const DFrame& fr, int depth);
void launch_medium(hipStream_t s, int n_cu, const DPathState& st, const DScene& sc, const DTables& T, const DFrame& fr, const DSobol& sob, int depth, DStats* stats);
void launch_detect_camera_medium(hipStream_t s, const DPathState& st, const DScene& sc, float x, float y, float z, DStats* stats);
void launch_light_select(hipStream_t s, int n_cu, const DPathState& st, const DScene& sc, const DTables& T, const DFrame& fr, const DSobol& sob, int depth, uint32_t kinds_mask, DStats* stats);
void launch_shade(hipStream_t s, int n_cu, int kind, const DPathState& st, const DScene& sc, const DTables& T, const DFrame& fr, const DSobol& sob, int depth, int first_kind, DStats* stats);
bool launch_small_pass(hipStream_t s, int n_cu, const DPathState& st, const DScene& sc, const DTables& T, const DFrame& fr, const DFilter& flt, const DCamera& cam, const DSobol& sob, int max_depth,
                       uint32_t kinds_mask, DStats* stats, bool dry, void* accum, int film_mode);
void launch_segment_lists(hipStream_t s, const DPathState& st, int n, const int* depths, const int* queues);
void launch_film(hipStream_t s, const DPathState& st, const DFrame& fr, const DTables& T, void* accum, bool f64);

void launch_sobol_table(hipStream_t s, const DSobol& sob, const DFrame& fr, uint2* table, int rows);
void launch_sobol_lo_table(hipStream_t s, const DSobol& sob, const DFrame& fr, uint16_t* table, int rows, int base, int stride, int count);
template <class Layout> void launch_finalize(hipStream_t s, const void* accum, bool f64, Layout out, int w, int h);
template <class Layout> void launch_aux(hipStream_t s, const DScene& sc, const DCamera& cam, int h, int w, float miss_depth, float* albedo, Layout out);
template <class Layout> void launch_variance(hipStream_t s, Layout src, float* variance, int h, int w);
template <class Layout> void launch_postprocess(hipStream_t s, const hk_postprocess_params& P, Layout src, float* out, int h, int w);
void launch_atrous(hipStream_t s, const hk_denoise_params& P, int step, PlanarPixels src, const float* variance, PlanarPixels dst, int h, int w);
void launch_atrous(hipStream_t s, const hk_denoise_params& P, int step, PackedPixels src, const float* variance, PackedPixels dst, float* out, const hk_postprocess_params* pp, int h, int w);
void launch_slot_of_prim(hipStream_t s, const float4* leaf, int n, int* slot_of_prim);
void launch_xform_tris(hipStream_t s, const DXform& X, int first, int n, const float* bp, const float* bn, const float* bt, const int* slot_of_prim, float* pos, float* nrm, float* tan, float* shade,
                       float4* leaf);
void launch_refit_level(hipStream_t s, int begin, int end, DNode* nodes, DQNode* qnodes, const DQGrid& grid, const float4* leaf, const float* pos);
void launch_envmap_tables(hipStream_t s, const DEnvMap& e, DEnvMap* record);
void launch_majorant_grid(hipStream_t s, const DMedium& m);
void launch_majorant_nanovdb(hipStream_t s, const DMedium& m, const DIndexBox& index_bbox);
void launch_nvdb_bricks(hipStream_t s, const DMedium& m, size_t n_blocks);

void launch_test_trace(hipStream_t s, const DScene& sc, int n, const float* o, const float* d, const float* tmax, float* t, int* prim, float* uv);
void launch_test_trace_lean(hipStream_t s, int n_cu, const DScene& sc, int anyhit, int n, const float* o, const float* d, const float* tmax, float* t, int* prim, float* uv);
void launch_test_sobol(hipStream_t s, const DTables& T, const DSobol& sob, int n, const int* px, const int* py, const int* si, const int* dim, float* o1, float* o2);
void launch_test_camera(hipStream_t s, const DTables& T, const DFilter& flt, const DCamera& cam, const DSobol& sob, int height, int n, const int* px, const int* py, const int* si, float* out);
void launch_test_uplift(hipStream_t s, const DTables& T, int mode, int n, const float* rgb, const float* lam, float* out);
void launch_test_light_bvh(hipStream_t s, const DScene& sc, int n, const float* p, const float* nn, const float* u, int* out_light, float* out_pmf, const int* query, float* out_qpmf);
void launch_test_light(hipStream_t s, const DScene& sc, const DTables& T, int mode, int light_idx, int n, const float* p3, const float* in3, const float* lambda, float* out);
void launch_test_bsdf(hipStream_t s, const DScene& sc, const DTables& T, int mode, int mat_idx, int regularize, int n, const float* wo, const float* wi, const float* ns, const float* lambda,
                      const float* u, const float* uc, float* out);
void launch_test_mix(hipStream_t s, const DScene& sc, int mat_idx, int n, const float* p3, const float* wo3, const float* uv2, int* out);
void launch_test_medium(hipStream_t s, const DScene& sc, const DTables& T, int mode, int medium_idx, int n, const float* a3, const float* b3, const float* tmax, const float* lambda, float* out);
int test_majorant_stride();

}
```

hikari.jl_amd/csrc/hk_launch_impl.h:

```cpp
#pragma once
#include "hk_launch.h"

namespace hk {

template <bool V>
using bool_c = std::bool_constant<V>;
template <int V>
using int_c = std::integral_constant<int, V>;
template <class F>
static void with_bool(bool b, F&& f) {
    if (b) f(bool_c<true>{});
    else f(bool_c<false>{});
}
template <int V0, int... Vs, class F>
static void with_int(int v, F&& f) {
    if constexpr (sizeof...(Vs) == 0) f(int_c<V0>{});
    else if (v == V0) f(int_c<V0>{});
    else with_int<Vs...>(v, f);
}

#ifndef HK_OCC_SCALE_DEFAULT
#define HK_OCC_SCALE_DEFAULT 1.0f
#endif
static inline int grid_for(int n, int block, int cap) {
    long g = ((long)n + block - 1) / block;
    if (g < 1) g = 1;
    if (g > cap) g = cap;
    return (int)g;
}

template <class K>
static int resident_blocks(K kernel, int block) {
    int per_cu = 0;
    if (hipOccupancyMaxActiveBlocksPerMultiprocessor(&per_cu, kernel, block, 0) != hipSuccess || per_cu < 1) per_cu = 1;
    return per_cu;
}
static float occ_scale() {
    const char* e = hk::knob("HK_OCC_SCALE");
    const float v = e ? (float)std::atof(e) : HK_OCC_SCALE_DEFAULT;
    return v >= 0.25f && v <= 8.0f ? v : 1.0f;
}
#define HK_MAX_DEVICES 64
template <auto Kernel>
static int cached_blocks(int block, int n_cu, int cap_per_cu) {
    static int cache[HK_MAX_DEVICES];
    int dev = 0, per_cu;
    if (hipGetDevice(&dev) != hipSuccess || dev < 0 || dev >= HK_MAX_DEVICES)
        per_cu = resident_blocks(Kernel, block);
    else {
        if (cache[dev] == 0) {
            cache[dev] = resident_blocks(Kernel, block);
            if (hk::knob("HK_DEBUG_ALLOC")) std::fprintf(stderr, "HK_DEBUG_ALLOC occupancy API: %d blocks of %d per CU for %s\n", cache[dev], block, __PRETTY_FUNCTION__);
        }
        per_cu = cache[dev];
    }
    per_cu = (int)((float)per_cu * occ_scale() + 0.5f);
    if (per_cu < 1) per_cu = 1;
    if (per_cu > cap_per_cu) per_cu = cap_per_cu;
    return per_cu * n_cu;
}
static int clamp_blocks(int blocks, const DPathState& st, int waves_per_block = 4) {
    const int units = st.n_waves / waves_per_block;
    if (blocks >= units) return units;
    if (st.dynamic_segments) return blocks;
    int best = 1;
    for (int b = blocks; b >= 1; --b)
        if (units % b == 0) {
            best = b;
            break;
        }
    return best * 4 >= blocks * 3 ? best : blocks;
}
template <auto K, class... A>
static void launch_resident(hipStream_t s, int n_cu, const DPathState& st, int block, int cap_per_cu, A&&... args) {
    const int blocks = cached_blocks<K>(block, n_cu, cap_per_cu);
    hipLaunchKernelGGL(K, dim3(clamp_blocks(blocks, st, block / 64)), dim3(block), 0, s, st, args...);
}

static bool node_cache_on() { return knob_on("HK_NODE_CACHE"); }
static int grey_mode() { return knob_int("HK_GREY", 1); }
static int grey_flat_mode() { return knob_int("HK_GREY_FLAT", 1); }
static int walk_pool_mode() { return knob_int("HK_WALK_POOL", 1); }
static int track_pool_mode() { return knob_int("HK_TRACK_POOL", 1); }
static bool sobol_tables_cover(const DSobol& sob, int depth) {
    return sob.hi_table != nullptr && sob.lo_table != nullptr && 9 + 5 * depth < sob.lo_rows && 9 + 5 * depth < sob.hi_rows && knob_on("HK_SOBOL_TABLE_ONLY");
}
static int media_mask_class(const DScene& sc) {
    int m = sc.media_mask;
    return (m == 1 || m == 2 || m == 4 || m == 8) ? m : 15;
}

void launch_camera(hipStream_t s, int n_cu, const DPathState& st, const DFrame& fr, const DTables& T, const DFilter& flt, const DCamera& cam, const DSobol& sob, int initial_medium) {
    launch_resident<k_camera>(s, n_cu, st, 256, 8, fr, T, flt, cam, sob, initial_medium);
}

#ifndef HK_SHADOW_NC16
#define HK_SHADOW_NC16 560
#endif
#ifndef HK_SHADOW_BLOCK16
#define HK_SHADOW_BLOCK16 768
#endif
#ifndef HK_SHADOW_NC32
#define HK_SHADOW_NC32 0
#endif
#ifndef HK_TRACE_NC32
#define HK_TRACE_NC32 128
#endif
template <int B16, int NC16, int NC32, class F>
static void lean_dispatch(const DScene& sc, const DFrame& fr, F&& launch) {
    with_bool(fr.count_nodes != 0, [&](auto COUNT) {
        with_bool(node_cache_on(), [&](auto CACHE) {
            constexpr bool cache = decltype(CACHE)::value;
            if (sc.bvh_depth <= 16) launch(COUNT, int_c<16>{}, int_c<cache ? B16 : HK_TRACE_BLOCK>{}, int_c<cache ? NC16 : 0>{}, bool_c<false>{});
            else with_bool(sc.qnodes != nullptr, [&](auto QN) { launch(COUNT, int_c<HK_LDS_STACK>{}, int_c<HK_TRACE_BLOCK>{}, int_c<cache ? NC32 : 0>{}, QN); });
        });
    });
}
void launch_trace(hipStream_t s, int n_cu, const DPathState& st, const DScene& sc, const DTables& T, const DFrame& fr, int depth, DStats* stats) {
    if (lean_scene(sc)) {
        lean_dispatch<1024, 1536, HK_TRACE_NC32>(sc, fr, [&](auto COUNT, auto STACK, auto BLOCK, auto NC, auto QN) {
            constexpr int block = decltype(BLOCK)::value;
            launch_resident<k_trace_lean<decltype(COUNT)::value, decltype(STACK)::value, block, decltype(NC)::value, decltype(QN)::value>>(s, n_cu, st, block, 8, sc, depth, stats);
        });
        return;
    }
    with_bool(fr.count_nodes != 0, [&](auto COUNT) { launch_resident<k_trace<decltype(COUNT)::value>>(s, n_cu, st, HK_TRACE_BLOCK, 8, sc, T, fr, depth, stats); });
}
template <bool C, int MM>
static void launch_walk_split(hipStream_t s, int n_cu, const DPathState& st, const DScene& sc, const DFrame& fr, int depth, DStats* stats) {
    const int cb = clamp_blocks(cached_blocks<k_walk_cast<C, MM, 16>>(HK_TRACE_BLOCK, n_cu, 8), st);
    const int tb = clamp_blocks(cached_blocks<k_walk_track<MM>>(256, n_cu, 8), st);
    for (int round = 0; round < HK_WALK_ROUNDS; ++round) {
        hipLaunchKernelGGL((k_walk_cast<C, MM, 16>), dim3(cb), dim3(HK_TRACE_BLOCK), 0, s, st, sc, depth, round, stats, sc.media);
        hipLaunchKernelGGL((k_walk_track<MM>), dim3(tb), dim3(256), 0, s, st, sc, depth, round, fr.walk_tune, stats, sc.media);
    }
}
bool grey_compact_ok(const DScene& sc) {
    if (!knob_on("HK_GREY_COMPACT")) return false;
    const int mc = sc.n_media > 0 ? media_mask_class(sc) : 0;
    return sc.n_media == 1 && sc.all_grey && sc.grey_pool && (mc == 2 || mc == 8) && sc.bvh_depth <= 16 && grey_mode() && grey_flat_mode() && track_pool_mode() && walk_pool_mode() &&
           !walk_split_mode();
}
template <bool C, int MM>
static void launch_shadow_walk(hipStream_t s, int n_cu, const DPathState& st, const DScene& sc, const DTables& T, const DFrame& fr, int depth, DStats* stats) {
    constexpr bool grey_kind = MM == 2 || MM == 8;
    constexpr int M2 = grey_kind ? MM : 8;
    const bool shallow = sc.bvh_depth <= 16;
    const int pool = walk_pool_mode();
    if (shallow && grey_kind && sc.grey_pool && grey_mode() && grey_flat_mode() && pool) {
        if (M2 == 8 && sc.grey_bricks && sc.bvh_depth <= 8 && pool == 1)
            launch_resident<k_walk_pool<C, 8, true, 8, 64>>(s, n_cu, st, HK_TRACE_BLOCK, 8, sc, depth, fr.walk_tune, fr.track_gate, stats, sc.media);
        else if (M2 == 8 && sc.grey_bricks)
            launch_resident<k_walk_pool<C, 8, true, 16, 56>>(s, n_cu, st, HK_TRACE_BLOCK, 8, sc, depth, fr.walk_tune, fr.track_gate, stats, sc.media);
        else
            launch_resident<k_walk_pool<C, M2, false, 16, 56>>(s, n_cu, st, HK_TRACE_BLOCK, 8, sc, depth, fr.walk_tune, fr.track_gate, stats, sc.media);
    } else if (shallow && grey_kind && sc.all_grey && grey_mode())
        launch_resident<k_shadow_walk<C, M2, 16, true>>(s, n_cu, st, HK_TRACE_BLOCK, 8, sc, T, depth, fr.walk_tune, stats, sc.media);
    else if (shallow)
        launch_resident<k_shadow_walk<C, MM, 16>>(s, n_cu, st, HK_TRACE_BLOCK, 8, sc, T, depth, fr.walk_tune, stats, sc.media);
    else
        launch_resident<k_shadow_walk<C, MM>>(s, n_cu, st, HK_TRACE_BLOCK, 8, sc, T, depth, fr.walk_tune, stats, sc.media);
}
void launch_shadow(hipStream_t s, int n_cu, const DPathState& st, const DScene& sc, const DTables& T, const DFrame& fr, int depth, DStats* stats) {
    if (lean_scene(sc)) {
        lean_dispatch<HK_SHADOW_BLOCK16, HK_SHADOW_NC16, HK_SHADOW_NC32>(sc, fr, [&](auto COUNT, auto STACK, auto BLOCK, auto NC, auto QN) {
            constexpr int block = decltype(BLOCK)::value;
            launch_resident<k_shadow<decltype(COUNT)::value, decltype(STACK)::value, block, decltype(NC)::value, decltype(QN)::value>>(s, n_cu, st, block, 8, sc, depth, stats);
        });
        return;
    }
    const int mc = sc.n_media > 0 ? media_mask_class(sc) : 0;
    const bool split = sc.all_grey && grey_mode() && walk_split_mode() && sc.bvh_depth <= 16 && st.wq_a != nullptr;
    with_bool(fr.count_nodes != 0, [&](auto COUNT) {
        constexpr bool c = decltype(COUNT)::value;
        if (split && mc == 8) launch_walk_split<c, 8>(s, n_cu, st, sc, fr, depth, stats);
        else if (split && mc == 2) launch_walk_split<c, 2>(s, n_cu, st, sc, fr, depth, stats);
        else with_int<0, 1, 2, 4, 8, 15>(mc, [&](auto MM) { launch_shadow_walk<c, decltype(MM)::value>(s, n_cu, st, sc, T, fr, depth, stats); });
    });
}
void launch_segment_lists(hipStream_t s, const DPathState& st, int n, const int* depths, const int* queues) {
    if (n <= 0) return;
    SegQueues qs;
    qs.n = n;
    for (int i = 0; i < n; ++i) {
        qs.depth[i] = depths[i];
        qs.q[i] = queues[i];
    }
    hipLaunchKernelGGL(k_segment_lists, dim3(n, HK_LIST_SPLIT), dim3(1024), 0, s, st, qs);
}
void launch_medium(hipStream_t s, int n_cu, const DPathState& st, const DScene& sc, const DTables& T, const DFrame& fr, const DSobol& sob, int depth, DStats* stats) {
    {
        const int d = depth, q = Q_MEDIUM;
        launch_segment_lists(s, st, 1, &d, &q);
    }
    const bool grey = sc.all_grey && grey_mode();
    const bool flat = grey && grey_flat_mode();
    const bool pool = flat && track_pool_mode() && sc.grey_pool;
    auto track = [&](auto MM, auto GREY) { launch_resident<k_track<decltype(MM)::value, decltype(GREY)::value>>(s, n_cu, st, 256, 8, sc, T, fr, depth, stats, sc.media); };
    auto track_flat = [&](auto MM, auto BRICKS) {
        constexpr int mm = decltype(MM)::value;
        constexpr bool bricks = decltype(BRICKS)::value;
        if (pool) launch_resident<k_track_pool<mm, bricks>>(s, n_cu, st, 256, 8, sc, fr, depth, stats, sc.media);
        else launch_resident<k_track_flat<mm, bricks>>(s, n_cu, st, 256, 8, sc, fr, depth, stats, sc.media);
    };
    switch (media_mask_class(sc)) {
        case 1: track(int_c<1>{}, bool_c<false>{}); break;
        case 2:
            if (flat) track_flat(int_c<2>{}, bool_c<false>{});
            else with_bool(grey, [&](auto GREY) { track(int_c<2>{}, GREY); });
            break;
        case 4: track(int_c<4>{}, bool_c<false>{}); break;
        case 8:
            if (flat) with_bool(sc.grey_bricks != 0, [&](auto BRICKS) { track_flat(int_c<8>{}, BRICKS); });
            else with_bool(grey, [&](auto GREY) { track(int_c<8>{}, GREY); });
            break;
        default: track(int_c<15>{}, bool_c<false>{}); break;
    }
    {
        const int d = depth, q = Q_SCATTER;
        launch_segment_lists(s, st, 1, &d, &q);
    }
    with_bool(sobol_tables_cover(sob, depth), [&](auto FT) { launch_resident<k_scatter<decltype(FT)::value>>(s, n_cu, st, 256, 8, sc, T, fr, sob, depth, stats); });
}
void launch_detect_camera_medium(hipStream_t s, const DPathState& st, const DScene& sc, float x, float y, float z, DStats* stats) {
    hipLaunchKernelGGL(k_detect_camera_medium, dim3(1), dim3(64), 0, s, st, sc, x, y, z, stats);
}
void launch_escaped(hipStream_t s, int n_cu, const DPathState& st, const DScene& sc, const DTables& T, const DFrame& fr, int depth) {
    with_bool(knob_int("HK_ESCAPED_UNROLL", 1) != 2, [&](auto ONE) { launch_resident<k_escaped<decltype(ONE)::value ? 1 : 2>>(s, n_cu, st, 256, 8, sc, T, depth, fr.implicit_ones); });
}
bool preselect_lights(const DScene& sc, const DPathState& st) {
    return sc.n_media == 0 && sc.num_bvh_lights >= HK_PRESELECT_MIN && st.sel_light != nullptr && knob_on("HK_PRESELECT");
}
void launch_light_select(hipStream_t s, int n_cu, const DPathState& st, const DScene& sc, const DTables& T, const DFrame& fr, const DSobol& sob, int depth, uint32_t kinds_mask, DStats* stats) {
    const int min_idle = knob_int_in("HK_SELECT_MIN_IDLE", 1, 64, HK_SELECT_MIN_IDLE);
    const bool pool = knob_on("HK_SELECT_POOL");
    with_bool(sobol_tables_cover(sob, depth), [&](auto FT) {
        constexpr bool ft = decltype(FT)::value;
        if (pool) launch_resident<k_light_select_pool<ft>>(s, n_cu, st, HK_SELECT_BLOCK, 8, sc, T, fr, sob, depth, kinds_mask, stats);
        else launch_resident<k_light_select<ft>>(s, n_cu, st, 256, 8, sc, T, fr, sob, depth, kinds_mask, min_idle, stats);
    });
}
void launch_shade(hipStream_t s, int n_cu, int kind, const DPathState& st, const DScene& sc, const DTables& T, const DFrame& fr, const DSobol& sob, int depth, int first_kind, DStats* stats) {
    auto shade = [&](auto KIND, auto SIMPLE, auto FT, auto PRE) {
        launch_resident<k_shade<decltype(KIND)::value, decltype(SIMPLE)::value, decltype(FT)::value, decltype(PRE)::value>>(s, n_cu, st, 256, 8, sc, T, fr, sob, depth, first_kind, stats);
    };
    const bool ft = sobol_tables_cover(sob, depth);
    const bool light_kind = kind == HK_MAT_MATTE || kind == HK_MAT_MIRROR || kind == HK_MAT_GLASS || kind == HK_MAT_CONDUCTOR;
    if (light_kind && preselect_lights(sc, st))
        with_int<HK_MAT_MATTE, HK_MAT_MIRROR, HK_MAT_GLASS, HK_MAT_CONDUCTOR>(kind, [&](auto KIND) { with_bool(ft, [&](auto FT) { shade(KIND, bool_c<false>{}, FT, bool_c<true>{}); }); });
    else if (kind == HK_MAT_MATTE && sc.simple_lights)
        with_bool(ft, [&](auto FT) { shade(int_c<HK_MAT_MATTE>{}, bool_c<true>{}, FT, bool_c<false>{}); });
    else if (light_kind && ft)
        with_int<HK_MAT_MATTE, HK_MAT_MIRROR, HK_MAT_GLASS, HK_MAT_CONDUCTOR>(kind, [&](auto KIND) { shade(KIND, bool_c<false>{}, bool_c<true>{}, bool_c<false>{}); });
    else
        with_int<HK_MAT_MATTE, HK_MAT_MIRROR, HK_MAT_GLASS, HK_MAT_CONDUCTOR, HK_MAT_COATED_DIFFUSE, HK_MAT_THIN_DIELECTRIC, HK_MAT_DIFFUSE_TRANSMISSION, HK_MAT_COATED_DIFFUSE_TRANSMISSION,
                 HK_MAT_COATED_CONDUCTOR, HK_MAT_FALLBACK>(kind, [&](auto KIND) { shade(KIND, bool_c<false>{}, bool_c<false>{}, bool_c<false>{}); });
}
#ifndef HK_SMALL_PASS_NC
#define HK_SMALL_PASS_NC 1536
#endif
static int small_pass_class(const DScene& sc, uint32_t kinds_mask) {
    const int mode = knob_int("HK_SMALL_PASS_FUSED", 2);
    if (mode == 0) return 0;
    if (!(lean_scene(sc) && sc.bvh_depth <= HK_LDS_STACK && node_cache_on())) return 0;
    if (kinds_mask == (1u << HK_MAT_MATTE) && sc.simple_lights && !sc.has_escape_lights && sc.bvh_depth <= 16 && sc.num_bvh_lights < HK_PRESELECT_MIN) return 1;
    const uint32_t light_kinds = (1u << HK_MAT_MATTE) | (1u << HK_MAT_MIRROR) | (1u << HK_MAT_GLASS) | (1u << HK_MAT_CONDUCTOR);
    return (mode >= 2 && kinds_mask != 0 && (kinds_mask & ~light_kinds) == 0) ? 2 : 0;
}
bool small_pass_fusable(const DScene& sc, uint32_t kinds_mask) { return small_pass_class(sc, kinds_mask) != 0; }
template <int BLOCK, bool GENERAL, int STACK, class... A>
static bool small_pass_blocks(hipStream_t s, int n_cu, const DPathState& st, bool dry, A&&... args) {
    constexpr auto kernel = k_small_pass<HK_SMALL_PASS_NC, BLOCK, GENERAL, STACK>;
    int blocks = cached_blocks<kernel>(BLOCK, n_cu, 1);
    if (blocks * (BLOCK / 64) > st.n_waves) blocks = st.n_waves / (BLOCK / 64);
    if (blocks < 1) return false;
    if (!dry) hipLaunchKernelGGL(kernel, dim3(blocks), dim3(BLOCK), 0, s, st, args...);
    return true;
}
bool launch_small_pass(hipStream_t s, int n_cu, const DPathState& st, const DScene& sc, const DTables& T, const DFrame& fr, const DFilter& flt, const DCamera& cam, const DSobol& sob, int max_depth,
                       uint32_t kinds_mask, DStats* stats, bool dry, void* accum, int film_mode) {
    const int cls = small_pass_class(sc, kinds_mask);
    if (cls == 0 || !st.small_pass || st.dynamic_segments || fr.count_nodes) return false;
    if (((long)st.capacity + 63) / 64 / 16 > 4L * n_cu) return false;
    for (int depth = 0; depth < max_depth; ++depth)
        if (sobol_tables_cover(sob, depth)) return false;
    const int merged = knob_on("HK_SMALL_PASS_MERGED") ? 1 : 0;
    if (st.n_waves > 8 * n_cu) return false;
    bool launched = false;
    auto pass = [&](auto GENERAL, auto STACK) {
        with_bool(st.n_waves > 4 * n_cu, [&](auto WIDE) {
            launched = small_pass_blocks<decltype(WIDE)::value ? 512 : 256, decltype(GENERAL)::value, decltype(STACK)::value>(s, n_cu, st, dry, sc, T, fr, flt, cam, sob, max_depth, sc.n_lights > 0 ? 1 : 0, merged,
                                                                                                                       accum, film_mode, kinds_mask, stats);
        });
    };
    if (cls == 2 && sc.bvh_depth > 16) pass(bool_c<true>{}, int_c<HK_LDS_STACK>{});
    else if (cls == 2) pass(bool_c<true>{}, int_c<16>{});
    else pass(bool_c<false>{}, int_c<16>{});
    return launched;
}
void launch_film(hipStream_t s, const DPathState& st, const DFrame& fr, const DTables& T, void* accum, bool f64) {
    int g = grid_for(fr.n_pixels_padded >> 6, 4, 4096);
    if (f64)
        hipLaunchKernelGGL(k_film<double>, dim3(g), dim3(256), 0, s, st, fr, T, (double*)accum);
    else
        hipLaunchKernelGGL(k_film<float>, dim3(g), dim3(256), 0, s, st, fr, T, (float*)accum);
}
void launch_sobol_table(hipStream_t s, const DSobol& sob, const DFrame& fr, uint2* table, int rows) {
    hipLaunchKernelGGL(k_sobol_table, dim3(grid_for((long)rows * fr.n_pixels_padded > 0x3fffffff ? 0x3fffffff : rows * fr.n_pixels_padded, 256, 8192)), dim3(256), 0, s, sob, fr, table, rows);
}
void launch_sobol_lo_table(hipStream_t s, const DSobol& sob, const DFrame& fr, uint16_t* table, int rows, int base, int stride, int count) {
    hipLaunchKernelGGL(k_sobol_lo_table, dim3(65536), dim3(256), 0, s, sob, fr, table, rows, base, stride, count);
}
template <class Layout>
void launch_finalize(hipStream_t s, const void* accum, bool f64, Layout out, int w, int h) {
    int g = grid_for(w * h, 256, 4096);
    if (f64)
        hipLaunchKernelGGL((k_finalize<double, Layout>), dim3(g), dim3(256), 0, s, (const double*)accum, out, w, h);
    else
        hipLaunchKernelGGL((k_finalize<float, Layout>), dim3(g), dim3(256), 0, s, (const float*)accum, out, w, h);
}
template <class Layout>
void launch_aux(hipStream_t s, const DScene& sc, const DCamera& cam, int h, int w, float miss_depth, float* albedo, Layout out) {
    hipLaunchKernelGGL(k_aux<Layout>, dim3(grid_for(h * w, HK_TRACE_BLOCK, 2048)), dim3(HK_TRACE_BLOCK), 0, s, sc, cam, h, w, miss_depth, albedo, out);
}
template <class Layout>
void launch_variance(hipStream_t s, Layout src, float* variance, int h, int w) {
    hipLaunchKernelGGL(k_variance<Layout>, dim3(grid_for(h * w, 256, 8192)), dim3(256), 0, s, src, variance, h, w);
}
template <class Layout>
void launch_postprocess(hipStream_t s, const hk_postprocess_params& P, Layout src, float* out, int h, int w) {
    hipLaunchKernelGGL(k_postprocess<Layout>, dim3(grid_for(h * w, 256, 8192)), dim3(256), 0, s, P, src, out, h, w);
}
template void launch_finalize<PlanarPixels>(hipStream_t, const void*, bool, PlanarPixels, int, int);
template void launch_aux<PlanarPixels>(hipStream_t, const DScene&, const DCamera&, int, int, float, float*, PlanarPixels);
template void launch_variance<PlanarPixels>(hipStream_t, PlanarPixels, float*, int, int);
template void launch_postprocess<PlanarPixels>(hipStream_t, const hk_postprocess_params&, PlanarPixels, float*, int, int);
template void launch_finalize<PackedPixels>(hipStream_t, const void*, bool, PackedPixels, int, int);
template void launch_aux<PackedPixels>(hipStream_t, const DScene&, const DCamera&, int, int, float, float*, PackedPixels);
template void launch_variance<PackedPixels>(hipStream_t, PackedPixels, float*, int, int);
template void launch_postprocess<PackedPixels>(hipStream_t, const hk_postprocess_params&, PackedPixels, float*, int, int);
template <class Layout, bool FINAL>
static void atrous(hipStream_t s, const hk_denoise_params& P, int step, Layout src, const float* variance, Layout dst, float* out, const hk_postprocess_params* pp, int h, int w) {
    const hk_postprocess_params PP = pp ? *pp : hk_postprocess_params{};
    hipLaunchKernelGGL((k_atrous<Layout, FINAL>), dim3(grid_for(h * w, 256, 8192)), dim3(256), 0, s, P, PP, pp ? 1 : 0, step, src, variance, dst, out, h, w);
}
void launch_atrous(hipStream_t s, const hk_denoise_params& P, int step, PlanarPixels src, const float* variance, PlanarPixels dst, int h, int w) {
    atrous<PlanarPixels, false>(s, P, step, src, variance, dst, nullptr, nullptr, h, w);
}
void launch_atrous(hipStream_t s, const hk_denoise_params& P, int step, PackedPixels src, const float* variance, PackedPixels dst, float* out, const hk_postprocess_params* pp, int h, int w) {
    with_bool(out != nullptr, [&](auto FINAL) { atrous<PackedPixels, decltype(FINAL)::value>(s, P, step, src, variance, dst, out, pp, h, w); });
}
void launch_slot_of_prim(hipStream_t s, const float4* leaf, int n, int* slot_of_prim) {
    hipLaunchKernelGGL(k_slot_of_prim, dim3(grid_for(n, 256, 8192)), dim3(256), 0, s, leaf, n, slot_of_prim);
}
void launch_xform_tris(hipStream_t s, const DXform& X, int first, int n, const float* bp, const float* bn, const float* bt, const int* slot_of_prim, float* pos, float* nrm,
                       float* tan, float* shade, float4* leaf) {
    hipLaunchKernelGGL(k_xform_tris, dim3(grid_for(n, 256, 8192)), dim3(256), 0, s, X, first, n, bp, bn, bt, slot_of_prim, pos, nrm, tan, shade, leaf);
}
void launch_refit_level(hipStream_t s, int begin, int end, DNode* nodes, DQNode* qnodes, const DQGrid& grid, const float4* leaf, const float* pos) {
    hipLaunchKernelGGL(k_refit_level, dim3(grid_for(end - begin, 256, 8192)), dim3(256), 0, s, begin, end, nodes, qnodes, grid, leaf, pos);
}
void launch_envmap_tables(hipStream_t s, const DEnvMap& e, DEnvMap* record) {
    hipLaunchKernelGGL(k_envmap_rows, dim3((e.nv + 63) / 64), dim3(64), 0, s, e.data, e.nu, e.nv, const_cast<float*>(e.cond_func), const_cast<float*>(e.cond_cdf),
                       const_cast<float*>(e.cond_func_int), const_cast<float*>(e.marg_func));
    hipLaunchKernelGGL(k_envmap_marginal, dim3(1), dim3(64), 0, s, e.nv, e.marg_func, const_cast<float*>(e.marg_cdf), record);
}

static int majorant_block_per_cell(double box_voxels) { return box_voxels > (double)knob_int("HK_MAJORANT_BLOCK_VOXELS", 8192) ? 1 : 0; }
static void majorant_zero_mask(hipStream_t s, const DMedium& m, int ncell) {
    hipLaunchKernelGGL(k_majorant_zero_mask, dim3((unsigned)(((long long)ncell + 255) / 256)), dim3(256), 0, s, m.majorant, ncell, const_cast<uint32_t*>(m.maj_zero));
}
void launch_majorant_grid(hipStream_t s, const DMedium& m) {
    const int ncell = m.mres[0] * m.mres[1] * m.mres[2];
    const int per_block = majorant_block_per_cell((double)m.res[0] * m.res[1] * m.res[2] / ncell);
    const dim3 grid((unsigned)(per_block ? ncell : ((long long)ncell + 3) / 4));
    with_bool(m.kind == HK_MEDIUM_RGB_GRID, [&](auto RGB) {
        hipLaunchKernelGGL((k_majorant_grid<decltype(RGB)::value>), grid, dim3(256), 0, s, m, ncell, per_block, const_cast<float*>(m.majorant));
    });
    majorant_zero_mask(s, m, ncell);
}
void launch_majorant_nanovdb(hipStream_t s, const DMedium& m, const DIndexBox& ib) {
    const int ncell = m.mres[0] * m.mres[1] * m.mres[2];
    double box = 1.0;
    for (int k = 0; k < 3; ++k) box *= ((double)ib.hi[k] - ib.lo[k] + 1.0) / m.mres[k] + 3.0;
    const int per_block = majorant_block_per_cell(box);
    hipLaunchKernelGGL(k_majorant_nanovdb, dim3((unsigned)(per_block ? ncell : ((long long)ncell + 3) / 4)), dim3(256), 0, s, m, ib, ncell, per_block, const_cast<float*>(m.majorant));
    majorant_zero_mask(s, m, ncell);
}
void launch_nvdb_bricks(hipStream_t s, const DMedium& m, size_t n_blocks) {
    const unsigned long long n_out = (unsigned long long)n_blocks * 729u;
    hipLaunchKernelGGL(k_nvdb_bricks, dim3((unsigned)std::min<unsigned long long>((n_out + 255) / 256, 1u << 20)), dim3(256), 0, s, m, n_out, const_cast<float*>(m.nv_bricks));
}

}
```

hikari.jl_amd/csrc/hk_render.cpp:

```cpp
#include "hk_host.h"

namespace {
float gaussian_1d(float x, float sigma) { return std::exp(-(x * x) / (2.0f * (sigma * sigma))); }
float mitchell_1d(float x, float B, float C) {
    x = std::fabs(x);
    if (x <= 1.0f) return ((12.0f - 9.0f * B - 6.0f * C) * (x * x * x) + (-18.0f + 12.0f * B + 6.0f * C) * (x * x) + (6.0f - 2.0f * B)) / 6.0f;
    if (x <= 2.0f) return ((-B - 6.0f * C) * (x * x * x) + (6.0f * B + 30.0f * C) * (x * x) + (-12.0f * B - 48.0f * C) * x + (8.0f * B + 24.0f * C)) / 6.0f;
    return 0.0f;
}
float sinc1(float x) {
    x = std::fabs(x);
    if (x < 1e-5f) return 1.0f;
    x *= 3.14159265358979323846f;
    return std::sin(x) / x;
}
float wsinc(float x, float r, float tau) {
    x = std::fabs(x);
    if (x > r) return 0.0f;
    return sinc1(x) * sinc1(x / tau);
}
float filter_eval(const hk_integrator_params& p, float ex, float ey, float x, float y) {
    float rx = p.filter_radius[0], ry = p.filter_radius[1];
    switch (p.filter_type) {
        case HK_FILTER_BOX: return (std::fabs(x) <= rx && std::fabs(y) <= ry) ? 1.0f : 0.0f;
// ... 220 lines not shown
        if (small) {
            I->st.dynamic_segments = 0;
            const int w = hk::knob_int_in("HK_SMALL_PASS_WAVES", 1, INT_MAX, 0);
            long per_cu = w > 0 ? w : (users ? (media ? 4 : 8) : (((open_scene && !media) || fusable) ? 8 : 16));
            const long chunks = ((long)capacity + 63) / 64;
            while (per_cu > 4 && per_cu * n_cu > chunks) per_cu /= 2;
            if (I->ctx->waves_per_cu <= 0) W_want = (per_cu * n_cu + 3) / 4 * 4;
        }
    }
    const bool want_split = media && hk::walk_split_mode();
    const bool want_cam = !media && !users && hk::knob_on("HK_VIEW_CACHE");
    if (I->st_capacity >= capacity && I->st_depth >= I->p.max_depth && I->st.n_waves == (int)W_want && I->st_media == (media ? 1 : 0) && (!want_split || I->st.wq_a != nullptr) &&
        (!want_cam || I->cam_gen.ray_d != nullptr || I->cam_unfit))
        return HK_OK;
    I->view_key.clear();
    if (users) HIP_TRY(hipStreamSynchronize(users));
    if (!I->bufs.empty()) quiesce(I->ctx);
    I->bufs.clear();
    DPathState& s = I->st;
    const int W = (int)W_want;
    const int chunks = (capacity + 63) / 64;
    s.capacity = capacity;
    s.n_waves = W;
    s.wave_cap = ((chunks + W - 1) / W) * 64;
    if (hk::knob_on("HK_STATE_SLAB")) {
        bool cam = want_cam;
        for (;;) {
            I->slab_mode = 1, I->slab_off = 0;
            if (int e = layout_state(I, media, want_split, cam)) {
                I->slab_mode = 0;
                return e;
            }
            size_t free_b = 0, total_b = 0;
            const bool known = hipMemGetInfo(&free_b, &total_b) == hipSuccess;
            if (!known) (void)hipGetLastError();
            hipError_t he = hipErrorOutOfMemory;
            if (!(cam && known && I->slab_off > free_b + g_slabs.total(I->ctx->device))) {
                I->bufs.emplace_back(new DevBuf());
                he = I->bufs.back()->alloc_slab(I->ctx->device, I->slab_off);
            }
            if (he == hipSuccess) break;
            (void)hipGetLastError();
            I->bufs.clear();
            if (!cam) {
                I->slab_mode = 0;
                return fail(HK_ERR_DEVICE, "path-state slab allocation failed");
            }
            cam = false;
        }
        I->slab_base = I->bufs.back()->p;
        I->slab_mode = 2, I->slab_off = 0;
        const int e = layout_state(I, media, want_split, cam);
        I->slab_mode = 0;
        if (e) return e;
        I->cam_unfit = want_cam && !cam;
    } else if (int e = layout_state(I, media, want_split, want_cam))
        return e;
    I->st_capacity = capacity;
    I->st_depth = I->p.max_depth;
    I->st_media = media ? 1 : 0;
    if (hk::knob("HK_DEBUG_ALLOC"))
        std::fprintf(stderr, "HK_DEBUG_ALLOC capacity %d Q %zu: ray_o %p ray_d %p beta %p hit %p sh_o %p L %p medium_q %p mat_q %p counters %p\n", capacity, (size_t)W * s.wave_cap, (void*)s.gen[0].ray_o,
                     (void*)s.gen[0].ray_d, (void*)s.gen[0].beta, (void*)s.hit, (void*)s.sh_o, (void*)s.L, (void*)s.medium_q, (void*)s.mat_q, (void*)s.counters);
    return HK_OK;
}
}
int ceil_log2(long v) {
    int l = 0;
    while ((1L << l) < v) ++l;
    return l;
}
DSobol make_sobol(const hk_integrator_params& p, int w, int h) {
    DSobol s;
    int spp = p.samples_per_pixel > 4096 ? p.samples_per_pixel : 4096;
    s.log2_spp = ceil_log2(spp < 1 ? 1 : spp);
    int res_log2 = ceil_log2(w > h ? w : h);
    s.n_base4_digits = res_log2 + (s.log2_spp + 1) / 2;
    s.seed = p.sampler_seed;
    s.width = w;
    s.hi_table = nullptr;
    s.hi_rows = s.hi_stride = 0;
    s.lo_table = nullptr;
    s.lo_rows = s.lo_count = s.lo_offset = 0;
    return s;
}

namespace {
int choose_samples_per_pass(hk_ctx* c, const hk_integrator* I, const DFrame& fr, int n_samples, int& S_out) {
    int S = I->p.samples_per_pass;
    if (S <= 0) {
        long max_paths = 192L << 20;
        if (const char* e = hk::knob("HK_MAX_PATHS_M")) max_paths = std::atol(e) > 0 ? std::atol(e) << 20 : max_paths;
        S = (int)(max_paths / fr.n_pixels_padded);
        if (S < 1) S = 1;
        if (S > 256) S = 256;
        size_t free_b = 0, total_b = 0;
        if (hipMemGetInfo(&free_b, &total_b) == hipSuccess) {
            free_b += g_slabs.total(c->device);
            while (S > 1 && (size_t)S * fr.n_pixels_padded * 440 > free_b / 2) S /= 2;
        }
    }
    if (S > n_samples) S = n_samples;
    if ((long)S * fr.n_pixels_padded > 0x3fffffffL) return fail(HK_ERR_INVALID, "pass too large");
    S_out = S;
    return HK_OK;
}
int pick_lane(hk_ctx* c, hk_integrator* I, const DFrame& fr, int S, int n_samples, int& lane_idx) {
    lane_idx = -1;
    int n_lanes = 1;
    long max_paths = 8L << 20;
    n_lanes = hk::knob_int_in("HK_PIPELINE", 1, 16, n_lanes);
    if (const char* e = hk::knob("HK_PIPELINE_MAX_PATHS_M")) max_paths = std::atol(e) > 0 ? std::atol(e) << 20 : max_paths;
    {
        const long by_memory = (8L << 30) / (440L * (long)S * fr.n_pixels_padded);
        if (n_lanes > by_memory) n_lanes = by_memory < 1 ? 1 : (int)by_memory;
    }
    const bool small_call = n_samples <= S && (long)S * fr.n_pixels_padded <= max_paths;
    int after = 4;
    after = hk::knob_int_in("HK_PIPELINE_AFTER", 0, INT_MAX, after);
    c->small_streak = small_call ? c->small_streak + 1 : 0;
    const bool lanes_started = c->ev_main != nullptr;
    if (n_lanes > 1 && !c->time_kernels && small_call && (lanes_started || c->small_streak > after)) {
        if ((int)I->lane_sets.size() < (int)hk_ctx::MAX_LANES) I->lane_sets.resize(hk_ctx::MAX_LANES);
        lane_idx = c->next_lane % n_lanes;
        c->next_lane = (lane_idx + 1) % n_lanes;
        hk_ctx::Lane& L = c->lanes[lane_idx];
        if (!L.stream) HIP_TRY(hipStreamCreateWithFlags(&L.stream, hipStreamNonBlocking));
        if (!L.done) {
            HIP_TRY(hipEventCreateWithFlags(&L.done, hipEventDisableTiming));
            std::vector<DStats> zero((size_t)c->stat_rows);
            std::memset(zero.data(), 0, zero.size() * sizeof(DStats));
            HIP_TRY(L.stats.upload(zero.data(), zero.size() * sizeof(DStats)));
        }
        if (!c->ev_main) {
            HIP_TRY(hipEventCreateWithFlags(&c->ev_main, hipEventDisableTiming));
            HIP_TRY(hipEventCreateWithFlags(&c->ev_film, hipEventDisableTiming));
        }
    } else {
        if (int e = join_lanes(c)) return e;
    }
    return HK_OK;
}
int ensure_sobol_tables(hk_ctx* c, hk_integrator* I, const DFrame& fr, DSobol& sob, int first_sample_idx, int n_samples, int sample_stride) {
    const int x0 = fr.x0, y0 = fr.y0;
    const int rows = 4 + 5 * (I->p.max_depth + 1);
    const bool table_same = !(I->sobol_rows != rows || I->sobol_stride != fr.n_pixels_padded || I->sobol_log2 != sob.log2_spp || I->sobol_digits != sob.n_base4_digits ||
                              I->sobol_x0 != x0 || I->sobol_y0 != y0 || I->sobol_tiles_x != fr.tiles_x);
    if (!table_same) {
        if (c->lanes_dirty) {
            if (int e = join_lanes(c)) return e;
            HIP_TRY(hipStreamSynchronize(c->stream));
        }
        HIP_TRY(I->sobol_table.alloc((size_t)rows * fr.n_pixels_padded * sizeof(uint2)));
        hk::launch_sobol_table(c->stream, sob, fr, I->sobol_table.as<uint2>(), rows);
        HIP_TRY(hipGetLastError());
        I->sobol_rows = rows;
        I->sobol_stride = fr.n_pixels_padded;
        I->sobol_log2 = sob.log2_spp;
        I->sobol_digits = sob.n_base4_digits;
        I->sobol_x0 = x0, I->sobol_y0 = y0, I->sobol_tiles_x = fr.tiles_x;
    }
    sob.hi_table = I->sobol_table.as<uint2>();
    sob.hi_rows = rows;
    sob.hi_stride = fr.n_pixels_padded;
    const long last_idx = (long)first_sample_idx + (long)(n_samples - 1) * sample_stride;
    if (n_samples >= 16 && sob.log2_spp >= 2 && sob.log2_spp <= 16 && (last_idx >> sob.log2_spp) == 0) {
        const int base = sample_stride == 1 ? (first_sample_idx & ~15) : first_sample_idx;
        const int count = (int)((((last_idx - base) / sample_stride + 1) + 15) & ~15L);
        bool same = table_same && I->lo_base == base && I->lo_sample_stride == sample_stride && I->lo_count == count && I->lo_rows > 0;
        if (!same) {
            if (c->lanes_dirty) {
                if (int e = join_lanes(c)) return e;
                HIP_TRY(hipStreamSynchronize(c->stream));
            }
            double gb = 32.0;
            if (const char* e = hk::knob("HK_SOBOL_LO_GB")) gb = std::atof(e);
            size_t budget = (size_t)(gb * 1e9), free_b = 0, total_b = 0;
            if (hipMemGetInfo(&free_b, &total_b) == hipSuccess && (free_b + I->sobol_lo.bytes) / 4 < budget) budget = (free_b + I->sobol_lo.bytes) / 4;
            const size_t per_row = (size_t)fr.n_pixels_padded * count * sizeof(uint16_t);
            int lo_rows = (int)(budget / per_row < (size_t)rows ? budget / per_row : (size_t)rows);
            I->lo_rows = 0;
            if (lo_rows > 0 && (size_t)fr.n_pixels_padded * count < 0xffffffffull) {
                bool have_buf = true;
                if (I->sobol_lo.bytes < per_row * lo_rows || I->sobol_lo.bytes > 2 * per_row * lo_rows) {
                    while (lo_rows > 0 && I->sobol_lo.alloc(per_row * lo_rows) != hipSuccess) {
                        (void)hipGetLastError();
                        lo_rows /= 2;
                    }
                    have_buf = lo_rows > 0;
                }
                if (have_buf) {
                    hk::launch_sobol_lo_table(c->stream, sob, fr, I->sobol_lo.as<uint16_t>(), lo_rows, base, sample_stride, count);
                    HIP_TRY(hipGetLastError());
                    I->lo_rows = lo_rows;
                    I->lo_base = base;
                    I->lo_sample_stride = sample_stride;
                    I->lo_count = count;
                }
            }
        }
        if (I->lo_rows > 0) {
            sob.lo_table = I->sobol_lo.as<uint16_t>();
            sob.lo_rows = I->lo_rows;
            sob.lo_count = I->lo_count;
        }
    }
    return HK_OK;
}
int detect_camera_medium(hipStream_t s, hk_integrator* I, const hk_scene* sc, const hk_camera* cam, DStats* dstats) {
    if (sc->d.n_media > 0) {
        const float* m = cam->camera_to_world;
        float w = m[15];
        float cx = m[3], cy = m[7], cz = m[11];
        if (w != 1.0f) {
            float inv = 1.0f / w;
            cx *= inv;
            cy *= inv;
            cz *= inv;
        }
        hk::launch_detect_camera_medium(s, I->st, sc->d, cx, cy, cz, dstats);
    } else
        HIP_TRY(hipMemsetAsync(I->st.initial_medium, 0xff, sizeof(int), s));
    return HK_OK;
}
struct ShadowStream {
    hk_ctx* c;
    bool overlap;
    bool in_flight = false;
    ~ShadowStream() {
        if (in_flight && c->aux) (void)hipStreamSynchronize(c->aux);
    }
};
struct PassCtx {
    hk_ctx* c;
    hk_scene* sc;
    hk_integrator* I;
    hk_film* film;
    DFrame fr;
    DSobol sob;
    DCamera dc;
    DStats* dstats;
    hipStream_t s;
    bool piped;
    int first_sample_idx, sample_stride;
    int view_mode = 0;
    std::string view_key_of() const;

    template <class F>
    int timed(int cls, F&& fn) {
        hipEvent_t e0 = nullptr, e1 = nullptr;
        if (c->time_kernels) {
            e0 = get_event(c);
            e1 = get_event(c);
            if (hipEventRecord(e0, s) != hipSuccess) return fail(HK_ERR_DEVICE, "event record failed");
        }
        fn();
        if (c->time_kernels) {
            if (hipEventRecord(e1, s) != hipSuccess) return fail(HK_ERR_DEVICE, "event record failed");
            (cls == 0 ? c->trace_events : c->class_events[cls]).emplace_back(e0, e1);
        }
        return HK_OK;
    }
    int lists(std::initializer_list<std::pair<int, int>> dq, bool kinds_of_depth = false, int kd = 0) {
        int dd[HK_MAX_KINDS + 6], qq[HK_MAX_KINDS + 6], n = 0;
        for (auto& e : dq) dd[n] = e.first, qq[n] = e.second, ++n;
        if (kinds_of_depth)
            for (int kind = 0; kind < HK_MAX_KINDS; ++kind)
                if (sc->kinds_mask & (1u << kind)) dd[n] = kd, qq[n] = Q_MAT0 + kind, ++n;
        if (I->st.small_pass) return HK_OK;
        return timed(3, [&] { hk::launch_segment_lists(s, I->st, n, dd, qq); });
    }
    int enqueue_depth(ShadowStream& sh, int depth);
    int enqueue_stages(bool view_hit);
    int enqueue_pass(int k, int done);
};
std::string PassCtx::view_key_of() const {
    std::string k;
    auto put = [&k](const void* p, size_t n) { k.append(static_cast<const char*>(p), n); };
    put(&dc, sizeof dc);
    put(&I->filter, sizeof I->filter);
    const int v[] = {fr.width, fr.height, fr.x0, fr.y0, fr.x1, fr.y1, fr.first_sample, fr.sample_stride, fr.samples_in_pass, sob.log2_spp, sob.n_base4_digits, (int)sob.seed, sob.width,
                     fr.implicit_ones, I->st.compact, I->st.meta32, I->st.const_origin, I->st.n_waves, I->st.wave_cap, I->st.dynamic_segments, view_mode, (int)c->tables_epoch};
    put(v, sizeof v);
    return k;
}
int PassCtx::enqueue_depth(ShadowStream& sh, int depth) {
    if (int e = timed(0, [&] { hk::launch_trace(s, c->n_cu, I->st, sc->d, c->tables, fr, depth, dstats); })) return e;
    c->trace_launches++;
    if (sh.in_flight) {
// ... 12 lines not shown
    } else if (int e = lists({}, true, depth))
        return e;
    if (sc->d.n_lights > 0 && hk::preselect_lights(sc->d, I->st)) {
        if (int e = timed(5, [&] { hk::launch_light_select(s, c->n_cu, I->st, sc->d, c->tables, fr, sob, depth, sc->kinds_mask, dstats); })) return e;
        c->select_launches++;
    }
    for (int kind = 0; kind < HK_MAX_KINDS; ++kind)
        if (sc->kinds_mask & (1u << kind)) {
            if (int e = timed(2, [&] { hk::launch_shade(s, c->n_cu, kind, I->st, sc->d, c->tables, fr, sob, depth, first_kind, dstats); })) return e;
            first_kind = 0;
            c->shade_launches++;
        }
    if (int e = lists({{depth, Q_SHADOW}, {depth + 1, Q_RAY}})) return e;
    if (sc->d.n_lights > 0) {
        if (sh.overlap) {
            HIP_TRY(hipEventRecord(c->ev_fork, s));
            HIP_TRY(hipStreamWaitEvent(c->aux, c->ev_fork, 0));
            hk::launch_shadow(c->aux, c->n_cu, I->st, sc->d, c->tables, fr, depth, dstats + c->stat_rows / 2);
            HIP_TRY(hipEventRecord(c->ev_join, c->aux));
            sh.in_flight = true;
        } else
            if (int e = timed(1, [&] { hk::launch_shadow(s, c->n_cu, I->st, sc->d, c->tables, fr, depth, dstats); })) return e;
        c->shadow_launches++;
    }
    return HK_OK;
}
int PassCtx::enqueue_stages(bool view_hit) {
    HIP_TRY(hipMemsetAsync(I->st.tickets, 0, (size_t)I->st.ticket_rows * HK_TICKET_COLS * HK_TICKET_WAYS * HK_TICKET_STRIDE * sizeof(int), s));
    const size_t kept = view_hit ? (size_t)I->st.n_waves : 0;
    HIP_TRY(hipMemsetAsync(I->st.counters + kept, 0, ((size_t)(I->st_depth + 2) * Q_COUNT * I->st.n_waves - kept) * sizeof(int), s));
    if (I->st.wq_ctl) HIP_TRY(hipMemsetAsync(I->st.wq_ctl, 0, (size_t)(I->st_depth + 2) * 11 * 4 * sizeof(int), s));
    if (!view_hit) {
        if (int e = timed(3, [&] { hk::launch_camera(s, c->n_cu, I->st, fr, c->tables, I->filter, dc, sob, -1); })) return e;
    } else if (view_mode == 2)
        HIP_TRY(hipMemsetAsync(I->st.L, 0, (size_t)fr.n_pixels_padded * fr.samples_in_pass * sizeof(float4), s));
    if (int e = lists({{0, Q_RAY}})) return e;
    if (const char* e = hk::knob("HK_OVERLAP")) c->overlap = std::atoi(e) ? 1 : 0;
    else c->overlap = -1;
    const bool want_overlap = c->overlap < 0 ? sc->d.bvh_depth > 16 : c->overlap != 0;
    const bool overlap = want_overlap && !c->time_kernels && sc->d.n_lights > 0 && sc->d.n_media == 0 && !piped && (!I->mid_pass || c->overlap == 1);
    if (overlap && !c->aux) {
        HIP_TRY(hipStreamCreateWithFlags(&c->aux, hipStreamNonBlocking));
        HIP_TRY(hipEventCreateWithFlags(&c->ev_fork, hipEventDisableTiming));
        HIP_TRY(hipEventCreateWithFlags(&c->ev_join, hipEventDisableTiming));
    }
    ShadowStream sh{c, overlap};
    for (int depth = 0; depth < I->p.max_depth; ++depth)
        if (int e = enqueue_depth(sh, depth)) return e;
    if (sh.in_flight) {
        HIP_TRY(hipStreamWaitEvent(s, c->ev_join, 0));
        sh.in_flight = false;
    }
    return HK_OK;
}
int PassCtx::enqueue_pass(int k, int done) {
    fr.samples_in_pass = k;
    {
        int L = 0;
        while ((1 << L) < k) ++L;
        fr.s_shr = 30 + L;
        fr.s_mul = (uint32_t)((((uint64_t)1 << fr.s_shr) + (uint64_t)k - 1) / (uint64_t)k);
    }
    fr.first_sample = first_sample_idx + done * sample_stride;
    if (sob.lo_table) sob.lo_offset = (fr.first_sample - I->lo_base) / sample_stride;
    const bool fused = !c->time_kernels && !piped && hk::launch_small_pass(s, c->n_cu, I->st, sc->d, c->tables, fr, I->filter, dc, sob, I->p.max_depth, sc->kinds_mask, dstats, true, nullptr, 0);
    const int vm = fused ? 0 : view_mode;
    I->st.view_cache = vm;
    I->st.gen_cam = vm ? I->cam_gen : I->st.gen[0];
    const std::string view_key = vm ? view_key_of() : std::string();
    const bool view_hit = vm && I->view_key == view_key;
    I->view_key.clear();
    bool film_inline = false;
    if (fused) {
        film_inline = fr.samples_in_pass == 1;
        (void)hk::launch_small_pass(s, c->n_cu, I->st, sc->d, c->tables, fr, I->filter, dc, sob, I->p.max_depth, sc->kinds_mask, dstats, false, film->accum, film_inline ? (film->f64 ? 2 : 1) : 0);
        c->fused_passes++;
    } else if (int e = enqueue_stages(view_hit))
        return e;
    if (piped && c->film_chain) HIP_TRY(hipStreamWaitEvent(s, c->ev_film, 0));
    if (!film_inline)
        if (int e = timed(3, [&] { hk::launch_film(s, I->st, fr, c->tables, film->accum, film->f64); })) return e;
    if (vm) I->view_key = view_key;
    if (view_hit) c->view_cache_hits++;
    if (piped) {
        HIP_TRY(hipEventRecord(c->ev_film, s));
        c->film_chain = true;
    }
    return HK_OK;
}
}

extern "C" int32_t hk_render(hk_ctx* c, hk_scene* sc, hk_integrator* I, hk_film* film, const hk_camera* cam, int32_t first_sample_idx, int32_t n_samples,
                             int32_t sample_stride) {
    if (!film) return fail(HK_ERR_INVALID, "null argument");
    return hk_render_tile(c, sc, I, film, cam, first_sample_idx, n_samples, sample_stride, 0, 0, film->width, film->height);
}

static int render_tile_now(hk_ctx* c, hk_scene* sc, hk_integrator* I, hk_film* film, const hk_camera* cam, int32_t first_sample_idx, int32_t n_samples,
                           int32_t sample_stride, int32_t x0, int32_t y0, int32_t x1, int32_t y1);
int flush_pending(hk_ctx* c) {
    if (!c || !c->pending.active) return HK_OK;
    hk_ctx::Pending p = c->pending;
    c->pending.active = false;
    return render_tile_now(c, p.sc, p.I, p.film, &p.cam, p.first, p.n, p.stride, p.x0, p.y0, p.x1, p.y1);
}
extern "C" int32_t hk_render_tile(hk_ctx* c, hk_scene* sc, hk_integrator* I, hk_film* film, const hk_camera* cam, int32_t first_sample_idx, int32_t n_samples,
                                  int32_t sample_stride, int32_t x0, int32_t y0, int32_t x1, int32_t y1) {
    if (!c || !sc || !I || !film || !cam) return fail(HK_ERR_INVALID, "null argument");
    if (x0 < 0 || y0 < 0 || x1 > film->width || y1 > film->height || x0 > x1 || y0 > y1) return fail(HK_ERR_INVALID, "pixel range outside the film");
    if (x0 == x1 || y0 == y1) return HK_OK;
    if (n_samples < 0 || sample_stride < 1 || first_sample_idx < 1) return fail(HK_ERR_INVALID, "bad sample range");
    if (!c->have_tables) return fail(HK_ERR_INVALID, "hk_ctx_set_tables must be called first");
    if (sc->ctx != c || I->ctx != c || film->ctx != c) return fail(HK_ERR_INVALID, "scene / integrator / film belong to another context");
    if (film->f64 != (I->p.accumulate_f64 != 0)) return fail(HK_ERR_INVALID, "film / integrator accumulation type mismatch");
    if (n_samples == 0) return HK_OK;
    KnobScope knobs(&c->knobs);
    {
        long batch_paths = 64L << 20, small_paths = 8L << 20;
        if (const char* e = hk::knob("HK_BATCH_PATHS_M")) batch_paths = std::atol(e) >= 0 ? std::atol(e) << 20 : batch_paths;
        if (const char* e = hk::knob("HK_PIPELINE_MAX_PATHS_M")) small_paths = std::atol(e) > 0 ? std::atol(e) << 20 : small_paths;
        const long px = (long)((x1 - x0 + 7) / 8) * ((y1 - y0 + 7) / 8) * 64;
        hk_ctx::Pending& p = c->pending;
        const bool visible_order = (c->own_stream_order && !film->external && !film->exposed) || hk::knob_int("HK_DEFER_EXTERNAL", 0);
        const bool small = batch_paths > 0 && visible_order && !c->time_kernels && (long)n_samples * px <= small_paths && I->p.samples_per_pass <= 0;
        if (p.active && small && p.sc == sc && p.I == I && p.film == film && std::memcmp(&p.cam, cam, sizeof(hk_camera)) == 0 && p.stride == sample_stride && p.x0 == x0 &&
            p.y0 == y0 && p.x1 == x1 && p.y1 == y1 && (long)p.first + (long)p.n * p.stride == first_sample_idx && (long)(p.n + n_samples) * px <= batch_paths) {
            p.n += n_samples;
            p.calls += 1;
            return HK_OK;
        }
        if (int e = flush_pending(c)) return e;
        if (small) {
            p.active = true;
            p.sc = sc, p.I = I, p.film = film, p.cam = *cam;
            p.first = first_sample_idx, p.n = n_samples, p.stride = sample_stride, p.x0 = x0, p.y0 = y0, p.x1 = x1, p.y1 = y1, p.calls = 1;
            return HK_OK;
        }
    }
    return render_tile_now(c, sc, I, film, cam, first_sample_idx, n_samples, sample_stride, x0, y0, x1, y1);
}
static int render_tile_now(hk_ctx* c, hk_scene* sc, hk_integrator* I, hk_film* film, const hk_camera* cam, int32_t first_sample_idx, int32_t n_samples,
                           int32_t sample_stride, int32_t x0, int32_t y0, int32_t x1, int32_t y1) {
    HIP_TRY(hipSetDevice(c->device));
    KnobScope knobs(&c->knobs);
    const int W = film->width, H = film->height;
    DFrame fr{};
    fr.width = W;
    fr.height = H;
    fr.x0 = x0, fr.y0 = y0, fr.x1 = x1, fr.y1 = y1;
    fr.tiles_x = (x1 - x0 + 7) / 8;
    fr.tiles_y = (y1 - y0 + 7) / 8;
    fr.n_pixels_padded = fr.tiles_x * fr.tiles_y * 64;
    int S = 0, lane_idx = -1;
    if (int e = choose_samples_per_pass(c, I, fr, n_samples, S)) return e;
    if (int e = pick_lane(c, I, fr, S, n_samples, lane_idx)) return e;
    const bool piped = lane_idx >= 0;
    struct SetGuard {
        hk_integrator* I;
        hk_integrator::StateSet* ls;
        ~SetGuard() {
            if (ls) I->swap_set(*ls);
        }
    } set_guard{I, piped ? &I->lane_sets[lane_idx] : nullptr};
    if (piped) I->swap_set(I->lane_sets[lane_idx]);
    if (int e = ensure_state(I, S * fr.n_pixels_padded, pass_traits(sc, c, n_samples, piped), piped ? c->lanes[lane_idx].stream : nullptr)) return e;
    I->st.const_origin = (I->st.meta32 && !(cam->lens_radius > 0)) ? 1 : 0;
    fr.sample_stride = sample_stride;
    fr.max_depth = I->p.max_depth;
    fr.regularize = I->p.regularize;
    fr.max_component_value = I->p.max_component_value;
    fr.count_nodes = c->count_nodes;
    fr.implicit_ones = sc->d.n_media == 0 ? 1 : 0;
    {
        auto knob = [](const char* name, int dflt) { return hk::knob_int_in(name, 1, 255, dflt); };
        fr.track_gate = hk::knob_int_in("HK_TRACK_MIN_PENDING", 0, 64, 0) | (hk::knob_int_in("HK_TRACK_EXTRA_ADVANCE", 0, 255, 4) << 8);
        fr.delta_advance = knob("HK_DELTA_ADVANCE", 3);
        fr.refill_idle = knob("HK_TRACK_REFILL_IDLE", 24);
        fr.walk_tune = knob("HK_SHADOW_TRACK_BATCH", 8) | (knob("HK_TRACK_ADVANCE", 2) << 8) | (knob("HK_SHADOW_FEED_ROUNDS", 3) << 16) | ((knob("HK_WALK_REFILL_IDLE", 16) > 63 ? 63 : knob("HK_WALK_REFILL_IDLE", 16)) << 24);
    }
    DSobol sob = make_sobol(I->p, W, H);
    if (int e = ensure_sobol_tables(c, I, fr, sob, first_sample_idx, n_samples, sample_stride)) return e;
    DCamera dc = make_camera(*cam);
    DStats* dstats = c->stats.as<DStats>();
    hipStream_t s = c->stream;
    if (piped) {
        HIP_TRY(hipEventRecord(c->ev_main, c->stream));
        s = c->lanes[lane_idx].stream;
        HIP_TRY(hipStreamWaitEvent(s, c->ev_main, 0));
        dstats = c->lanes[lane_idx].stats.as<DStats>();
    }
    if (!c->have_span) {
        HIP_TRY(hipEventRecord(c->ev_begin, s));
        c->have_span = true;
    }
    if (int e = detect_camera_medium(s, I, sc, cam, dstats)) return e;
    PassCtx pass{c, sc, I, film, fr, sob, dc, dstats, s, piped, first_sample_idx, sample_stride};
    if (!piped && n_samples == S && I->cam_gen.ray_d != nullptr && I->st.meta32 && fr.implicit_ones) {
        const int mode = hk::knob_int("HK_VIEW_CACHE", 1);
        pass.view_mode = mode == 2 ? 2 : (mode != 0 ? 1 : 0);
    }
    for (int done = 0; done < n_samples;) {
        const int k = n_samples - done < S ? n_samples - done : S;
        if (int e = pass.enqueue_pass(k, done)) return e;
        done += k;
    }
    HIP_TRY(hipGetLastError());
    if (piped) {
        HIP_TRY(hipEventRecord(c->lanes[lane_idx].done, s));
        c->lanes_dirty = true;
    } else
        HIP_TRY(hipEventRecord(c->ev_end, s));
    return HK_OK;
}
```

hikari.jl_amd/csrc/hk_types.h:

```cpp
#pragma once
#include <hip/hip_runtime.h>
#include <stdint.h>
#include <cstdlib>

namespace hk {
const char* knob(const char* name);
inline bool knob_on(const char* name) {
    const char* e = knob(name);
    return !(e && std::atoi(e) == 0);
}
inline int knob_int(const char* name, int dflt) {
    const char* e = knob(name);
    return e ? std::atoi(e) : dflt;
}
inline int knob_int_in(const char* name, int lo, int hi, int dflt) {
    const int v = knob_int(name, dflt);
    return v >= lo && v <= hi ? v : dflt;
}
}

#define HK_TICKET_COLS 16
#define HK_TICKET_WAYS 64
#define HK_TICKET_STRIDE 64
#define HK_MAX_KINDS 11
// ... 155 lines not shown
    int copy;
};
struct DQGrid {
    float base[3], cell[3];
};

struct DScene {
    const DNode* nodes;
    const DQNode* qnodes;
    float q_base[3], q_cell[3];
    const float4* leaf_tris;
    int root_ref;
    int n_tris;
    int n_nodes;
    int pad_nodes;
    const float* positions;
    const float* normals;
    const float* uvs;
    const float* tangents;
    const DTriMeta* meta;
    const DMaterial* materials;
    const DTexture* textures;
    const DPLSpectrum* spectra;
    const DMediumInterface* mis;
    const DLight* lights;
    int n_lights;
    int n_materials;
    const DLightNode* lnodes;
    const uint32_t* bit_trails;
    const int* infinite_lights;
    int num_bvh_lights, num_infinite_lights;
    const DMedium* media;
    int n_media;
    int media_mask;
    const DEnvMap* envmaps;
    int n_envmaps;
    int has_escape_lights;
    int simple_lights;
    int all_opaque;
    int bvh_depth;
    int all_grey;
    int grey_pool;
    int grey_bricks;
    const float* tri_shade;
};

struct DTables {
    const uint32_t* sobol;
    const float* cie;
    const float* rgb2spec_scale;
    const float* rgb2spec_coeffs;
    int rgb2spec_res;
    const float4* rgb2spec_points;
    int rgb2spec_sorted;
};

struct DFilter {
    int type;
    float rx, ry, p1, p2;
    int nx, ny;
    const float* func;
    const float* marginal_cdf;
    const float* marginal_func;
    const float* conditional_cdf;
    float dmin_x, dmin_y, dmax_x, dmax_y;
    float func_integral;
};

struct DCamera {
    float r2c[16];
    float c2w[16];
    float lens_radius, focal_distance, shutter_open, shutter_close;
};

struct DSobol {
    int log2_spp, n_base4_digits;
    uint32_t seed;
    int width;
    const uint2* hi_table;
    int hi_rows, hi_stride;
    const uint16_t* lo_table;
    int lo_rows, lo_count;
    int lo_offset;
};

enum { Q_RAY = 0, Q_SHADOW = 1, Q_ESCAPED = 2, Q_MEDIUM = 3, Q_SCATTER = 4, Q_MAT0 = 5, Q_COUNT = Q_MAT0 + HK_MAX_KINDS };

#ifndef HK_LAMBDA_BY_SLOT
#define HK_LAMBDA_BY_SLOT 1
#endif
struct DPathGen {
    float4* ray_o;
    float4* ray_d;
    float4* beta;
    float4* r_u;
    float4* r_l;
    float4* lambda;
    uint2* meta;
};

struct DPathState {
    int capacity;
    int n_waves;
    int wave_cap;
    DPathGen gen[2];
    float4* hit;
    int* mat_id;
    uint2* sel_light;
    float4* lambda_s;
    float4* pdf;
    float4* L;
    float* filter_w;
    float4* sh_o;
    float4* sh_d;
    float4* sh_Ld;
    float4* sh_ru;
    float4* sh_rl;
    uint32_t* sh_slot;
    float4* sh_T;
    uint32_t* sh_aux;
    float4* sh_it;
    uint32_t* wq_a;
    uint32_t* wq_b;
    int* wq_ctl;
    uint32_t* escaped_q;
    uint32_t* medium_q;
    uint32_t* scatter_q;
    int* initial_medium;
    uint32_t* mat_q;
    int* counters;
    int* tickets;
    int ticket_rows;
    int* seg_list;
    int* seg_list_n;
    int dynamic_segments;
    int small_pass;
    int ticket_share;
    int compact;
    int meta32, const_origin;
    int sh_final;
    DPathGen gen_cam;
    int view_cache;
};

struct DStats {
    unsigned long long rays_closest, rays_shadow, nodes, tris, hits, vertices, collisions, light_nodes, sh_nodes, sh_tris;
    unsigned long long nvdb_collisions, sh_nvdb_collisions;
    unsigned long long sh_collisions, dda_steps, sh_dda_steps, scatter_vertices, sc_light_nodes;
#ifdef HK_DEBUG_UTIL
    unsigned long long dbg[32];
#endif
};

struct DFrame {
    int width, height, tiles_x, tiles_y;
    int x0, y0, x1, y1;
    int n_pixels_padded;
    int samples_in_pass;
    uint32_t s_mul;
    int s_shr;
    int first_sample, sample_stride;
    int max_depth;
    int regularize;
    float max_component_value;
    int count_nodes;
    int implicit_ones;
// ... 31 lines not shown
```

include/hikari_mi355x.h:

```cpp
#ifndef HIKARI_MI355X_H
#define HIKARI_MI355X_H

#include <stdint.h>

#ifdef __cplusplus
extern "C" {
#endif

#define HK_OK 0
#define HK_ERR_INVALID -1
#define HK_ERR_DEVICE -2
#define HK_ERR_UNSUPPORTED -3
#define HK_UNSET -100

typedef struct hk_texture {
    int32_t width, height, channels;
    int32_t kind;
    const float* data;
} hk_texture;

typedef struct hk_tex_rgba {
    float c[4];
    int32_t tex;
} hk_tex_rgba;
// ... 130 lines not shown
    int32_t n_lights;
    int32_t n_envmaps;
    int32_t n_media;
    int32_t n_spectra;
    const float* positions;
    const float* normals;
    const float* uvs;
    const float* tangents;
    const hk_tri_meta* meta;
    const hk_material* materials;
    const hk_texture* textures;
    const hk_medium_interface* media_interfaces;
    const hk_light* lights;
    const hk_envmap* envmaps;
    const hk_medium* media;
    const hk_pl_spectrum* spectra;
} hk_scene_desc;

typedef struct hk_tables {
    const uint32_t* sobol_matrices;
    int32_t sobol_count;
    int32_t rgb2spec_res;
    const float* cie_x;
    const float* cie_y;
    const float* cie_z;
    const float* rgb2spec_scale;
    const float* rgb2spec_coeffs;
} hk_tables;

enum { HK_FILTER_BOX = 1, HK_FILTER_TRIANGLE = 2, HK_FILTER_GAUSSIAN = 3, HK_FILTER_MITCHELL = 4, HK_FILTER_LANCZOS = 5 };
enum { HK_COHERENCE_NONE = 0, HK_COHERENCE_SORTED = 1, HK_COHERENCE_PER_TYPE = 2 };

typedef struct hk_integrator_params {
    int32_t max_depth;
    int32_t samples_per_pixel;
    int32_t russian_roulette_depth;
    int32_t regularize;
    int32_t material_coherence;
    float max_component_value;
    int32_t filter_type;
    float filter_radius[2];
    float filter_param1;
    float filter_param2;
    int32_t accumulate_f64;
    uint32_t sampler_seed;
    int32_t samples_per_pass;
} hk_integrator_params;

typedef struct hk_camera {
    float raster_to_camera[16];
    float camera_to_world[16];
    float lens_radius, focal_distance;
    float shutter_open, shutter_close;
    float dx_camera[3], dy_camera[3];
} hk_camera;

typedef struct hk_stats {
    uint64_t rays_closest;
    uint64_t rays_shadow;
    uint64_t bvh_nodes_visited;
    uint64_t tris_tested;
    uint64_t hits_accepted;
    uint64_t path_vertices;
    uint64_t medium_collisions;
    uint64_t light_bvh_nodes;
    double seconds_trace;
    double seconds_total;
    uint64_t trace_launches;
    uint64_t trace_nodes, trace_tris;
    uint64_t shadow_nodes, shadow_tris;
    uint64_t shadow_launches, shade_launches;
    double seconds_shadow, seconds_shade, seconds_other;
    uint64_t bytes_algorithmic_trace, bytes_algorithmic_shadow, bytes_algorithmic_shade;
    double seconds_media;
    uint64_t track_collisions, shadow_collisions;
    uint64_t track_dda_steps, shadow_dda_steps;
    uint64_t scatter_vertices;
    uint64_t media_launches;
    uint64_t bytes_algorithmic_media;
    double seconds_select;
    uint64_t select_launches;
    uint64_t fused_passes;
    uint64_t view_cache_hits;
} hk_stats;

typedef struct hk_ctx hk_ctx;
typedef struct hk_scene hk_scene;
typedef struct hk_film hk_film;
typedef struct hk_integrator hk_integrator;

int32_t hk_ctx_create(int32_t device_id, void* stream, hk_ctx** out);
int32_t hk_ctx_destroy(hk_ctx* ctx);
const char* hk_last_error(void);
int32_t hk_ctx_set_tables(hk_ctx* ctx, const hk_tables* tables);
int32_t hk_ctx_set_option(hk_ctx* ctx, const char* name, const char* value);
int32_t hk_ctx_get_option(hk_ctx* ctx, const char* name, char* out, int32_t out_bytes);
int32_t hk_trim_cache(hk_ctx* ctx);

int32_t hk_scene_create(hk_ctx* ctx, const hk_scene_desc* desc, hk_scene** out);
int32_t hk_scene_destroy(hk_scene* scene);

int32_t hk_scene_set_transform(hk_scene* scene, int32_t first_tri, int32_t n_tris, const float* m34);
int32_t hk_scene_update_materials(hk_scene* scene, int32_t first, int32_t n, const hk_material* materials);
int32_t hk_scene_update_lights(hk_scene* scene, int32_t first, int32_t n, const hk_light* lights);
int32_t hk_scene_update_envmap(hk_scene* scene, int32_t idx, const float* data, const float* rotation);
int32_t hk_scene_update_medium(hk_scene* scene, int32_t idx, const hk_medium* medium);

int32_t hk_integrator_create(hk_ctx* ctx, const hk_integrator_params* params, hk_integrator** out);
int32_t hk_integrator_destroy(hk_integrator* integ);

int32_t hk_film_create(hk_ctx* ctx, int32_t width, int32_t height, int32_t f64, void* external_accum, hk_film** out);
int32_t hk_film_destroy(hk_film* film);
int32_t hk_film_clear(hk_film* film);

int32_t hk_render(hk_ctx* ctx, hk_scene* scene, hk_integrator* integ, hk_film* film, const hk_camera* cam,
                  int32_t first_sample_idx, int32_t n_samples, int32_t sample_stride);

int32_t hk_render_tile(hk_ctx* ctx, hk_scene* scene, hk_integrator* integ, hk_film* film, const hk_camera* cam,
                       int32_t first_sample_idx, int32_t n_samples, int32_t sample_stride, int32_t x0, int32_t y0, int32_t x1, int32_t y1);

typedef struct hk_comm hk_comm;
int32_t hk_comm_create(hk_ctx* const* ctxs, int32_t n, hk_comm** out);
int32_t hk_comm_unique_id(uint8_t* id_out128);
int32_t hk_comm_create_rank(hk_ctx* ctx, const uint8_t* id128, int32_t rank, int32_t world, hk_comm** out);
int32_t hk_comm_destroy(hk_comm* comm);
int32_t hk_film_reduce(hk_comm* comm, hk_film* const* films, int32_t n_films, int32_t root);

int32_t hk_film_read_rgb(hk_ctx* ctx, hk_film* film, float* out_hw3);
int32_t hk_film_read_rgb_async(hk_ctx* ctx, hk_film* film);
int32_t hk_film_read_wait(hk_ctx* ctx, hk_film* film, float* out_hw3, const float** frame);
int32_t hk_film_pin_host(hk_film* film, float* host_hw3);
int32_t hk_film_unpin_host(hk_film* film);
int32_t hk_film_read_accum(hk_ctx* ctx, hk_film* film, void* out);
void* hk_film_accum_device_ptr(hk_film* film);

int32_t hk_flush(hk_ctx* ctx);
int32_t hk_sync(hk_ctx* ctx);
int32_t hk_stats_get(hk_ctx* ctx, hk_stats* out);
int32_t hk_stats_reset(hk_ctx* ctx);
int32_t hk_stats_enable_counters(hk_ctx* ctx, int32_t flags);

int32_t hk_trace_closest(hk_ctx* ctx, hk_scene* scene, int32_t n, const float* o3, const float* d3, const float* tmax,
                         float* out_t, int32_t* out_prim, float* out_uv2);
int32_t hk_test_sobol(hk_ctx* ctx, int32_t width, int32_t height, int32_t spp, uint32_t seed, int32_t n,
                      const int32_t* px, const int32_t* py, const int32_t* sample_idx, const int32_t* dim,
                      float* out_1d, float* out_2d);
int32_t hk_test_camera(hk_ctx* ctx, hk_integrator* integ, const hk_camera* cam, int32_t width, int32_t height, int32_t n,
                       const int32_t* px, const int32_t* py, const int32_t* sample_idx, float* out15);
int32_t hk_test_uplift(hk_ctx* ctx, int32_t mode, int32_t n, const float* rgb, const float* lambda, float* out);
int32_t hk_test_light_bvh(hk_ctx* ctx, hk_scene* scene, int32_t n, const float* p3, const float* n3, const float* u,
                          int32_t* out_light, float* out_pmf, const int32_t* query_light, float* out_query_pmf);
enum { HK_TONEMAP_NONE = 0, HK_TONEMAP_REINHARD = 1, HK_TONEMAP_REINHARD_EXT = 2, HK_TONEMAP_ACES = 3, HK_TONEMAP_UNCHARTED2 = 4, HK_TONEMAP_FILMIC = 5 };
typedef struct hk_postprocess_params {
    float exposure;
    int32_t tonemap;
    float inv_gamma;
    int32_t apply_gamma;
    float white_point;
    float imaging_ratio;
    int32_t apply_wb;
    float wb[9];
    int32_t mask_escaped;
    float bg[3];
} hk_postprocess_params;
int32_t hk_film_postprocess(hk_ctx* ctx, hk_film* film, const hk_postprocess_params* params, const float* depth, float* dst_rgb);
int32_t hk_postprocess(hk_ctx* ctx, const hk_postprocess_params* params, int32_t width, int32_t height, const float* src_rgb,
// ... 44 lines not shown
```

Measured before the change: 10300.

## Precompute per-depth Sobol draws into a device buffer and use fast slab reciprocals

Adds a kernel that evaluates, for each depth, the light-select, light, BSDF, lobe and roulette Sobol dimensions for every pixel and sample slot into a float buffer. It builds this buffer once the same sampler configuration has been seen twice and keeps it for later calls. Light-select and shade kernels get a new template mode that reads these precomputed values instead of evaluating Sobol per draw, which trades per-draw matrix work for extra memory traffic and a large allocation. Separately, ray-slab setup switches to the hardware approximate reciprocal, uses a different clamp bound for axis-parallel rays, and simplifies the epsilon computation.

```diff
diff --git a/hikari.jl_amd/_abi.py b/hikari.jl_amd/_abi.py
--- a/hikari.jl_amd/_abi.py
+++ b/hikari.jl_amd/_abi.py
@@ -126,7 +126,8 @@
                 ("track_collisions", C.c_uint64), ("shadow_collisions", C.c_uint64), ("track_dda_steps", C.c_uint64),
                 ("shadow_dda_steps", C.c_uint64), ("scatter_vertices", C.c_uint64), ("media_launches", C.c_uint64),
                 ("bytes_algorithmic_media", C.c_uint64), ("seconds_select", C.c_double), ("select_launches", C.c_uint64),
-                ("fused_passes", C.c_uint64), ("view_cache_hits", C.c_uint64)]
+                ("fused_passes", C.c_uint64), ("view_cache_hits", C.c_uint64),
+                ("sobol_value_passes", C.c_uint64), ("sobol_value_builds", C.c_uint64)]
 
 
 EXPORTED_SYMBOLS = [
diff --git a/hikari.jl_amd/csrc/hk_ctx.cpp b/hikari.jl_amd/csrc/hk_ctx.cpp
--- a/hikari.jl_amd/csrc/hk_ctx.cpp
+++ b/hikari.jl_amd/csrc/hk_ctx.cpp
@@ -13,7 +13,7 @@
 static const char* const KNOB_NAMES[] = {
     "HK_BATCH_PATHS_M", "HK_BVH_LEAF", "HK_BVH_BINS", "HK_QNODES", "HK_DEBUG_ALLOC", "HK_DELTA_ADVANCE", "HK_DYNAMIC_SEGMENTS", "HK_GREY", "HK_GREY_COMPACT", "HK_GREY_FLAT", "HK_MAX_PATHS_M",
     "HK_MID_LISTS", "HK_MID_PASS_PATHS_M", "HK_NODE_CACHE", "HK_NVDB_DENSE_MB", "HK_OVERLAP", "HK_PIPELINE", "HK_PIPELINE_AFTER", "HK_PIPELINE_MAX_PATHS_M", "HK_PRESELECT",
-    "HK_SELECT_MIN_IDLE", "HK_SHADOW_FEED_ROUNDS", "HK_SHADOW_TRACK_BATCH", "HK_SMALL_PASS", "HK_SMALL_PASS_WAVES", "HK_SOBOL_LO_GB", "HK_SOBOL_TABLE_ONLY",
+    "HK_SELECT_MIN_IDLE", "HK_SHADOW_FEED_ROUNDS", "HK_SHADOW_TRACK_BATCH", "HK_SMALL_PASS", "HK_SMALL_PASS_WAVES", "HK_SOBOL_DRAWS", "HK_SOBOL_DRAW_GB", "HK_SOBOL_LO_GB", "HK_SOBOL_TABLE_ONLY",
     "HK_STATE_CACHE_GB", "HK_STATE_SLAB", "HK_TICKET_SHARE", "HK_TRACK_ADVANCE", "HK_TRACK_EXTRA_ADVANCE", "HK_TRACK_MIN_PENDING", "HK_TRACK_POOL", "HK_TRACK_REFILL_IDLE",
     "HK_WALK_POOL", "HK_WALK_REFILL_IDLE", "HK_WALK_SPLIT", "HK_WAVES_PER_CU", "HK_READBACK_PIN", "HK_DEFER_EXTERNAL", "HK_SELECT_POOL", "HK_SMALL_PASS_FUSED", "HK_SMALL_PASS_MERGED", "HK_OCC_SCALE", "HK_ESCAPED_UNROLL", "HK_SHADOW_FINAL", "HK_TRI_PACK", "HK_LEAN_RECORDS", "HK_VIEW_CACHE", "HK_MAJORANT_BLOCK_VOXELS"};
 static bool known_knob(const char* name) {
@@ -261,6 +261,7 @@
     c->seconds_trace = c->seconds_total = 0.0;
     c->trace_launches = c->shadow_launches = c->shade_launches = c->media_launches = c->select_launches = 0;
     c->fused_passes = c->view_cache_hits = 0;
+    c->sobol_value_passes = c->sobol_value_builds = 0;
     c->have_span = false;
     return HK_OK;
 }
@@ -354,6 +355,8 @@
     out->select_launches = c->select_launches;
     out->fused_passes = c->fused_passes;
     out->view_cache_hits = c->view_cache_hits;
+    out->sobol_value_passes = c->sobol_value_passes;
+    out->sobol_value_builds = c->sobol_value_builds;
     {
         const uint64_t hits_closest = h.hits < h.rays_closest ? h.hits : h.rays_closest;
         out->bytes_algorithmic_trace = h.rays_closest * (32 + 16) + 64 * h.nodes + 36 * h.tris + 96 * hits_closest;
diff --git a/hikari.jl_amd/csrc/hk_device.h b/hikari.jl_amd/csrc/hk_device.h
--- a/hikari.jl_amd/csrc/hk_device.h
+++ b/hikari.jl_amd/csrc/hk_device.h
@@ -344,6 +344,33 @@
     uint64_t bits = zsobol_hash(dim + 2, c.seed);
     return mk2(sobol_sample(idx, 0, (uint32_t)bits, c.mats), sobol_sample(idx, 1, (uint32_t)(bits >> 32), c.mats));
 }
+struct SobolVals {
+    const float* block;
+    size_t entries;
+    uint32_t e;
+};
+HKD SobolVals sobol_vals(const DSobol& s, int depth, int pix_slot, int k) {
+    SobolVals v;
+    v.entries = (size_t)s.hi_stride * (size_t)s.lo_count;
+    v.block = s.val + (size_t)depth * ((size_t)(6 + s.val_lobe) * v.entries);
+    v.e = (uint32_t)pix_slot * (uint32_t)s.lo_count + (uint32_t)(s.lo_offset + k);
+    return v;
+}
+template <int MODE, int OFF>
+HKD float draw_1d(const SobolCtx& c, const SobolVals& v, int base_dim) {
+    static_assert(OFF == 1 || OFF == 4 || OFF == 7, "a 1-D draw of a bounce");
+    if constexpr (MODE == 2) return OFF == 4 ? v.block[6 * v.entries + v.e] : v.block[2 * (size_t)v.e + (OFF == 7 ? 1 : 0)];
+    else return sobol_1d<MODE == 1>(c, base_dim + OFF);
+}
+template <int MODE, int OFF>
+HKD v2 draw_2d(const SobolCtx& c, const SobolVals& v, int base_dim) {
+    static_assert(OFF == 3 || OFF == 6, "a 2-D draw of a bounce");
+    if constexpr (MODE == 2) {
+        const float2 u = reinterpret_cast<const float2*>(v.block + (OFF == 3 ? 2 : 4) * v.entries)[v.e];
+        return mk2(u.x, u.y);
+    } else
+        return sobol_2d<MODE == 1>(c, base_dim + OFF);
+}
 
 HKD float jl_sin_kernel(double y) {
     const double S1 = -0.16666666641626524, S2 = 0.008333329385889463, S3 = -0.00019839334836096632, S4 = 2.718311493989822e-6;
@@ -764,14 +791,28 @@
     float u, v;
 };
 
+#ifndef HK_SLAB_RCP
+#define HK_SLAB_RCP 1
+#endif
+#define HK_SLAB_PARALLEL 0x1p100f
 struct RaySlab {
     float ix, iy, iz, ox, oy, oz, eps3;
 };
+HKD float slab_rcp(float d) {
+#if HK_SLAB_RCP
+    return __builtin_amdgcn_rcpf(d);
+#else
+    return 1.0f / d;
+#endif
+}
 HKD RaySlab ray_slab(v3 o, v3 d) {
     RaySlab r;
-    r.ix = clampf(1.0f / d.x, -1e30f, 1e30f), r.iy = clampf(1.0f / d.y, -1e30f, 1e30f), r.iz = clampf(1.0f / d.z, -1e30f, 1e30f);
+    r.ix = clampf(slab_rcp(d.x), -HK_SLAB_PARALLEL, HK_SLAB_PARALLEL), r.iy = clampf(slab_rcp(d.y), -HK_SLAB_PARALLEL, HK_SLAB_PARALLEL);
+    r.iz = clampf(slab_rcp(d.z), -HK_SLAB_PARALLEL, HK_SLAB_PARALLEL);
     r.ox = -o.x * r.ix, r.oy = -o.y * r.iy, r.oz = -o.z * r.iz;
-    r.eps3 = 3.0f * (2.4e-7f * fmaxf(fmaxf(fabsf(r.ix) < 1e30f ? fabsf(r.ox) : 0.0f, fabsf(r.iy) < 1e30f ? fabsf(r.oy) : 0.0f), fabsf(r.iz) < 1e30f ? fabsf(r.oz) : 0.0f));
+    const bool free_ray = fabsf(r.ix) < HK_SLAB_PARALLEL && fabsf(r.iy) < HK_SLAB_PARALLEL && fabsf(r.iz) < HK_SLAB_PARALLEL;
+    r.eps3 = 3.0f * (2.4e-7f * fmaxf(fmaxf(fabsf(r.ox), fabsf(r.oy)), fabsf(r.oz)));
+    if (!free_ray) r.eps3 = fmaxf(r.eps3, 0x1p60f);
     return r;
 }
 HKD RaySlab ray_slab_grid(const DScene& sc, v3 o, v3 d) {
diff --git a/hikari.jl_amd/csrc/hk_host.h b/hikari.jl_amd/csrc/hk_host.h
--- a/hikari.jl_amd/csrc/hk_host.h
+++ b/hikari.jl_amd/csrc/hk_host.h
@@ -176,6 +176,7 @@
     int count_nodes = 0, time_kernels = 0;
     unsigned long long fused_passes = 0;
     unsigned long long view_cache_hits = 0;
+    unsigned long long sobol_value_passes = 0, sobol_value_builds = 0;
     std::vector<std::pair<hipEvent_t, hipEvent_t>> trace_events;
     std::vector<std::pair<hipEvent_t, hipEvent_t>> class_events[6];
     uint64_t shadow_launches = 0, shade_launches = 0, media_launches = 0, select_launches = 0;
@@ -324,6 +325,9 @@
     int sobol_rows = 0, sobol_stride = 0, sobol_log2 = -1, sobol_digits = -1, sobol_x0 = -1, sobol_y0 = -1, sobol_tiles_x = -1;
     DevBuf sobol_lo;
     int lo_rows = 0, lo_base = -1, lo_sample_stride = -1, lo_count = 0;
+    DevBuf sobol_val;
+    std::string val_key, val_seen, val_seen2;
+    int val_depths = 0, val_lobe = 0;
     struct StateSet {
         DPathState st{};
         std::vector<std::unique_ptr<DevBuf>> bufs;
diff --git a/hikari.jl_amd/csrc/hk_kernels.hip b/hikari.jl_amd/csrc/hk_kernels.hip
--- a/hikari.jl_amd/csrc/hk_kernels.hip
+++ b/hikari.jl_amd/csrc/hk_kernels.hip
@@ -384,6 +384,29 @@
         uint4* out = reinterpret_cast<uint4*>(table) + 2 * i;
         out[0] = make_uint4(v[0] | (v[1] << 16), v[2] | (v[3] << 16), v[4] | (v[5] << 16), v[6] | (v[7] << 16));
         out[1] = make_uint4(v[8] | (v[9] << 16), v[10] | (v[11] << 16), v[12] | (v[13] << 16), v[14] | (v[15] << 16));
+    }
+}
+
+__global__ void __launch_bounds__(256) k_sobol_values(DSobol sob, DFrame fr, const uint32_t* mats, float* block, int depth, int base, int stride) {
+    const size_t entries = (size_t)sob.hi_stride * (size_t)sob.lo_count;
+    float2* const selrr = reinterpret_cast<float2*>(block);
+    float2* const light = selrr + entries;
+    float2* const bsdf = light + entries;
+    float* const lobe = block + 6 * entries;
+    const int base_dim = 6 + 7 * depth;
+    for (size_t i = (size_t)blockIdx.x * blockDim.x + threadIdx.x; i < entries; i += (size_t)gridDim.x * blockDim.x) {
+        const int pix = (int)(i / (size_t)sob.lo_count), j = (int)(i - (size_t)pix * sob.lo_count);
+        const SobolCtx c = sobol_ctx_slot(sob, mats, fr.x0, fr.y0, fr.tiles_x, pix, j, base + j * stride);
+        float2 a = make_float2(0.0f, 0.0f), b = a, d = a;
+        float l = 0.0f;
+        if (c.hi != nullptr && c.lo != nullptr) {
+            a = make_float2(sobol_1d<true>(c, base_dim + 1), sobol_1d<true>(c, base_dim + 7));
+            const v2 ul = sobol_2d<true>(c, base_dim + 3), ub = sobol_2d<true>(c, base_dim + 6);
+            b = make_float2(ul.x, ul.y), d = make_float2(ub.x, ub.y);
+            if (sob.val_lobe) l = sobol_1d<true>(c, base_dim + 4);
+        }
+        selrr[i] = a, light[i] = b, bsdf[i] = d;
+        if (sob.val_lobe) lobe[i] = l;
     }
 }
 
@@ -1978,7 +2001,7 @@
 #ifndef HK_SELECT_MIN_IDLE
 #define HK_SELECT_MIN_IDLE 24
 #endif
-template <bool FT>
+template <int FT>
 __global__ void __launch_bounds__(256) k_light_select(DPathState st, DScene sc, DTables T, DFrame fr, DSobol sob, int depth, uint32_t kinds_mask, int min_idle, DStats* stats) {
     const int lane = lane_id();
     const unsigned long long lt_mask = (1ull << lane) - 1ull;
@@ -2026,8 +2049,9 @@
                     nn = sf.ns;
                     int pix, k;
                     split_slot(fr, ld_meta(st, g, slot, depth).y, pix, k);
-                    const SobolCtx sctx = sobol_ctx_slot(sob, T.sobol, fr.x0, fr.y0, fr.tiles_x, pix, k, fr.first_sample + k * fr.sample_stride);
-                    const float u = sobol_1d<FT>(sctx, base_dim + 1);
+                    float u;
+                    if constexpr (FT == 2) u = draw_1d<2, 1>(SobolCtx(), sobol_vals(sob, depth, pix, k), base_dim);
+                    else u = sobol_1d<FT == 1>(sobol_ctx_slot(sob, T.sobol, fr.x0, fr.y0, fr.tiles_x, pix, k, fr.first_sample + k * fr.sample_stride), base_dim + 1);
                     busy = true;
                     done = true;
                     res_light = 0;
@@ -2116,7 +2140,7 @@
 #ifndef HK_SELECT_WAVES
 #define HK_SELECT_WAVES 4
 #endif
-template <bool FT, int BLOCK = HK_SELECT_BLOCK, int NTOP = HK_SELECT_NTOP>
+template <int FT, int BLOCK = HK_SELECT_BLOCK, int NTOP = HK_SELECT_NTOP>
 __global__ void __attribute__((amdgpu_flat_work_group_size(BLOCK, BLOCK), amdgpu_waves_per_eu(HK_SELECT_WAVES))) k_light_select_pool(DPathState st, DScene sc, DTables T, DFrame fr, DSobol sob, int depth, uint32_t kinds_mask, DStats* stats) {
     __shared__ uint32_t lds_pool[BLOCK / 64][8][64];
     __shared__ float4 lds_top[NTOP > 0 ? 4 * NTOP : 1];
@@ -2188,8 +2212,9 @@
                         sn = sf.ns;
                         int pix, k;
                         split_slot(fr, ld_meta(st, g, e, depth).y, pix, k);
-                        const SobolCtx sctx = sobol_ctx_slot(sob, T.sobol, fr.x0, fr.y0, fr.tiles_x, pix, k, fr.first_sample + k * fr.sample_stride);
-                        const float u = sobol_1d<FT>(sctx, base_dim + 1);
+                        float u;
+                        if constexpr (FT == 2) u = draw_1d<2, 1>(SobolCtx(), sobol_vals(sob, depth, pix, k), base_dim);
+                        else u = sobol_1d<FT == 1>(sobol_ctx_slot(sob, T.sobol, fr.x0, fr.y0, fr.tiles_x, pix, k, fr.first_sample + k * fr.sample_stride), base_dim + 1);
                         int res_light = 0;
                         float res_pmf = 0.0f;
                         if (ninf + nbvh > 0) {
@@ -2339,7 +2364,7 @@
 #ifndef HK_SHADE_MIN_WAVES
 #define HK_SHADE_MIN_WAVES 1
 #endif
-template <int KIND, bool SIMPLE, bool FT, bool PRE>
+template <int KIND, bool SIMPLE, int FT, bool PRE>
 __device__ __forceinline__ void shade_body(const DPathState& st, const DScene& sc, const DTables& T, const DFrame& fr, const DSobol& sob, int depth, int first_kind, DStats* stats, const SegTickets& src,
                                            uint32_t* __restrict__ elist) {
     const int lane = lane_id();
@@ -2391,6 +2416,7 @@
         int pdepth = 0, medium = -1;
         bool any_non_specular = false;
         SobolCtx sctx;
+        SobolVals svals{nullptr, 0, 0u};
         const int base_dim = 6 + 7 * depth;
         float4 shO = make_float4(0, 0, 0, 0), shD = shO;
         S4 shLd = s4(0.0f), shRu = s4(0.0f), shRl = s4(0.0f);
@@ -2421,7 +2447,8 @@
 
             int pix, k;
             split_slot(fr, pslot, pix, k);
-            sctx = sobol_ctx_slot(sob, T.sobol, fr.x0, fr.y0, fr.tiles_x, pix, k, fr.first_sample + k * fr.sample_stride);
+            if constexpr (FT == 2) svals = sobol_vals(sob, depth, pix, k);
+            else sctx = sobol_ctx_slot(sob, T.sobol, fr.x0, fr.y0, fr.tiles_x, pix, k, fr.first_sample + k * fr.sample_stride);
 
             if (KIND == HK_MAT_MATTE) kd_matte = matte_kd<SIMPLE>(sc, T, sc.materials[st.mat_id[slot] & ~HK_MAT_EMISSIVE_BIT], TexCtx(sf.uv, meta.prim_index, H.z, H.w), lambda);
 #ifdef HK_ABLATE
@@ -2483,13 +2510,13 @@
                     light_idx = (int)pre.x;
                     light_pmf = __uint_as_float(pre.y);
                 } else {
-                    float light_select = sobol_1d<FT>(sctx, base_dim + 1);
+                    float light_select = draw_1d<FT, 1>(sctx, svals, base_dim);
                     light_idx = bvh_sample_light(sc, sf.pi, sf.ns, light_select, light_pmf, n_lnodes);
                 }
                 if (light_idx >= 1 && light_idx <= sc.n_lights && light_pmf > 0.0f) {
                     const DLight& sel = sc.lights[light_idx - 1];
                     v2 u_light = mk2(0.0f, 0.0f);
-                    if (sel.kind >= HK_LIGHT_AMBIENT) u_light = sobol_2d<FT>(sctx, base_dim + 3);
+                    if (sel.kind >= HK_LIGHT_AMBIENT) u_light = draw_2d<FT, 3>(sctx, svals, base_dim);
                     LightSample ls = sample_light<KIND == HK_MAT_MATTE, SIMPLE>(sc, T, sel, sf.pi, lambda, u_light);
                     if (ls.pdf > 0.0f && !is_black(ls.Li)) {
                         float bsdf_pdf;
@@ -2548,8 +2575,8 @@
             if (new_depth < fr.max_depth) {
                 const DMaterial& mat = sc.materials[st.mat_id[slot] & ~HK_MAT_EMISSIVE_BIT];
                 const DMediumInterface mi = sc.mis[meta.mi];
-                float uc = (KIND == HK_MAT_GLASS || KIND > HK_MAT_CONDUCTOR) && KIND != HK_MAT_FALLBACK ? sobol_1d<FT>(sctx, base_dim + 4) : 0.0f;
-                v2 u = (KIND == HK_MAT_MIRROR || KIND == HK_MAT_GLASS || KIND == HK_MAT_THIN_DIELECTRIC) ? mk2(0.0f, 0.0f) : sobol_2d<FT>(sctx, base_dim + 6);
+                float uc = (KIND == HK_MAT_GLASS || KIND > HK_MAT_CONDUCTOR) && KIND != HK_MAT_FALLBACK ? draw_1d<FT, 4>(sctx, svals, base_dim) : 0.0f;
+                v2 u = (KIND == HK_MAT_MIRROR || KIND == HK_MAT_GLASS || KIND == HK_MAT_THIN_DIELECTRIC) ? mk2(0.0f, 0.0f) : draw_2d<FT, 6>(sctx, svals, base_dim);
                 bool regularize = fr.regularize && any_non_specular;
                 BSDFSample s = KIND == HK_MAT_MATTE ? sample_matte_kd<SIMPLE>(sc, mat, kd_matte, wo, sf.ns, TexCtx(sf.uv, meta.prim_index, H.z, H.w), u)
                                                     : sample_bsdf<KIND>(sc, T, mat, wo, sf.ns, TexCtx(sf.uv, meta.prim_index, H.z, H.w), lambda, u, uc, regularize);
@@ -2559,7 +2586,7 @@
                     nrl = s.is_specular ? r_u : r_u / s.pdf;
                     bool cont = true;
                     if (new_depth > 3) {
-                        float rr = sobol_1d<FT>(sctx, base_dim + 7);
+                        float rr = draw_1d<FT, 7>(sctx, svals, base_dim);
                         float q = maxf(0.05f, 1.0f - max_component(nb));
                         if (rr < q)
                             cont = false;
@@ -2601,7 +2628,7 @@
     wave_add(&stats->vertices, n_vertices);
     wave_add(&stats->light_nodes, n_lnodes);
 }
-template <int KIND, bool SIMPLE = false, bool FT = false, bool PRE = false>
+template <int KIND, bool SIMPLE = false, int FT = 0, bool PRE = false>
 __global__ void __attribute__((amdgpu_flat_work_group_size(256, 256), amdgpu_waves_per_eu(ShadeWaves<KIND>::value))) k_shade(DPathState st, DScene sc, DTables T, DFrame fr, DSobol sob, int depth, int first_kind, DStats* stats) {
     __shared__ uint32_t emit_list[4 * 128];
     shade_body<KIND, SIMPLE, FT, PRE>(st, sc, T, fr, sob, depth, first_kind, stats, seg_open(st, ticket_ptr(st, depth, TK_SHADE0 + KIND), st.dynamic_segments != 0, depth, Q_MAT0 + KIND),
diff --git a/hikari.jl_amd/csrc/hk_launch.h b/hikari.jl_amd/csrc/hk_launch.h
--- a/hikari.jl_amd/csrc/hk_launch.h
+++ b/hikari.jl_amd/csrc/hk_launch.h
@@ -26,6 +26,7 @@
 
 void launch_sobol_table(hipStream_t s, const DSobol& sob, const DFrame& fr, uint2* table, int rows);
 void launch_sobol_lo_table(hipStream_t s, const DSobol& sob, const DFrame& fr, uint16_t* table, int rows, int base, int stride, int count);
+void launch_sobol_values(hipStream_t s, const DSobol& sob, const DFrame& fr, const uint32_t* mats, float* block, int depth, int base, int stride);
 template <class Layout> void launch_finalize(hipStream_t s, const void* accum, bool f64, Layout out, int w, int h);
 template <class Layout> void launch_aux(hipStream_t s, const DScene& sc, const DCamera& cam, int h, int w, float miss_depth, float* albedo, Layout out);
 template <class Layout> void launch_variance(hipStream_t s, Layout src, float* variance, int h, int w);
diff --git a/hikari.jl_amd/csrc/hk_launch_impl.h b/hikari.jl_amd/csrc/hk_launch_impl.h
--- a/hikari.jl_amd/csrc/hk_launch_impl.h
+++ b/hikari.jl_amd/csrc/hk_launch_impl.h
@@ -84,6 +84,13 @@
 static int track_pool_mode() { return knob_int("HK_TRACK_POOL", 1); }
 static bool sobol_tables_cover(const DSobol& sob, int depth) {
     return sob.hi_table != nullptr && sob.lo_table != nullptr && 9 + 5 * depth < sob.lo_rows && 9 + 5 * depth < sob.hi_rows && knob_on("HK_SOBOL_TABLE_ONLY");
+}
+static bool sobol_values_cover(const DSobol& sob, int depth) { return sob.val != nullptr && depth < sob.val_depths && sobol_tables_cover(sob, depth); }
+template <class F>
+static void with_sampler_mode(const DSobol& sob, int depth, F&& f) {
+    if (sobol_values_cover(sob, depth)) f(int_c<2>{});
+    else if (sobol_tables_cover(sob, depth)) f(int_c<1>{});
+    else f(int_c<0>{});
 }
 static int media_mask_class(const DScene& sc) {
     int m = sc.media_mask;
@@ -234,8 +241,8 @@
 void launch_light_select(hipStream_t s, int n_cu, const DPathState& st, const DScene& sc, const DTables& T, const DFrame& fr, const DSobol& sob, int depth, uint32_t kinds_mask, DStats* stats) {
     const int min_idle = knob_int_in("HK_SELECT_MIN_IDLE", 1, 64, HK_SELECT_MIN_IDLE);
     const bool pool = knob_on("HK_SELECT_POOL");
-    with_bool(sobol_tables_cover(sob, depth), [&](auto FT) {
-        constexpr bool ft = decltype(FT)::value;
+    with_sampler_mode(sob, depth, [&](auto FT) {
+        constexpr int ft = decltype(FT)::value;
         if (pool) launch_resident<k_light_select_pool<ft>>(s, n_cu, st, HK_SELECT_BLOCK, 8, sc, T, fr, sob, depth, kinds_mask, stats);
         else launch_resident<k_light_select<ft>>(s, n_cu, st, 256, 8, sc, T, fr, sob, depth, kinds_mask, min_idle, stats);
     });
@@ -246,15 +253,23 @@
     };
     const bool ft = sobol_tables_cover(sob, depth);
     const bool light_kind = kind == HK_MAT_MATTE || kind == HK_MAT_MIRROR || kind == HK_MAT_GLASS || kind == HK_MAT_CONDUCTOR;
-    if (light_kind && preselect_lights(sc, st))
-        with_int<HK_MAT_MATTE, HK_MAT_MIRROR, HK_MAT_GLASS, HK_MAT_CONDUCTOR>(kind, [&](auto KIND) { with_bool(ft, [&](auto FT) { shade(KIND, bool_c<false>{}, FT, bool_c<true>{}); }); });
-    else if (kind == HK_MAT_MATTE && sc.simple_lights)
-        with_bool(ft, [&](auto FT) { shade(int_c<HK_MAT_MATTE>{}, bool_c<true>{}, FT, bool_c<false>{}); });
-    else if (light_kind && ft)
-        with_int<HK_MAT_MATTE, HK_MAT_MIRROR, HK_MAT_GLASS, HK_MAT_CONDUCTOR>(kind, [&](auto KIND) { shade(KIND, bool_c<false>{}, bool_c<true>{}, bool_c<false>{}); });
+    auto mode = [&](auto&& f) {
+        if (sobol_values_cover(sob, depth)) f(int_c<2>{});
+        else f(int_c<1>{});
+    };
+    if (light_kind && preselect_lights(sc, st)) {
+        with_int<HK_MAT_MATTE, HK_MAT_MIRROR, HK_MAT_GLASS, HK_MAT_CONDUCTOR>(kind, [&](auto KIND) {
+            if (ft) mode([&](auto FT) { shade(KIND, bool_c<false>{}, FT, bool_c<true>{}); });
+            else shade(KIND, bool_c<false>{}, int_c<0>{}, bool_c<true>{});
+        });
+    } else if (kind == HK_MAT_MATTE && sc.simple_lights) {
+        if (ft) mode([&](auto FT) { shade(int_c<HK_MAT_MATTE>{}, bool_c<true>{}, FT, bool_c<false>{}); });
+        else shade(int_c<HK_MAT_MATTE>{}, bool_c<true>{}, int_c<0>{}, bool_c<false>{});
+    } else if (light_kind && ft)
+        with_int<HK_MAT_MATTE, HK_MAT_MIRROR, HK_MAT_GLASS, HK_MAT_CONDUCTOR>(kind, [&](auto KIND) { mode([&](auto FT) { shade(KIND, bool_c<false>{}, FT, bool_c<false>{}); }); });
     else
         with_int<HK_MAT_MATTE, HK_MAT_MIRROR, HK_MAT_GLASS, HK_MAT_CONDUCTOR, HK_MAT_COATED_DIFFUSE, HK_MAT_THIN_DIELECTRIC, HK_MAT_DIFFUSE_TRANSMISSION, HK_MAT_COATED_DIFFUSE_TRANSMISSION,
-                 HK_MAT_COATED_CONDUCTOR, HK_MAT_FALLBACK>(kind, [&](auto KIND) { shade(KIND, bool_c<false>{}, bool_c<false>{}, bool_c<false>{}); });
+                 HK_MAT_COATED_CONDUCTOR, HK_MAT_FALLBACK>(kind, [&](auto KIND) { shade(KIND, bool_c<false>{}, int_c<0>{}, bool_c<false>{}); });
 }
 #ifndef HK_SMALL_PASS_NC
 #define HK_SMALL_PASS_NC 1536
@@ -311,6 +326,9 @@
 void launch_sobol_lo_table(hipStream_t s, const DSobol& sob, const DFrame& fr, uint16_t* table, int rows, int base, int stride, int count) {
     hipLaunchKernelGGL(k_sobol_lo_table, dim3(65536), dim3(256), 0, s, sob, fr, table, rows, base, stride, count);
 }
+void launch_sobol_values(hipStream_t s, const DSobol& sob, const DFrame& fr, const uint32_t* mats, float* block, int depth, int base, int stride) {
+    hipLaunchKernelGGL(k_sobol_values, dim3(65536), dim3(256), 0, s, sob, fr, mats, block, depth, base, stride);
+}
 template <class Layout>
 void launch_finalize(hipStream_t s, const void* accum, bool f64, Layout out, int w, int h) {
     int g = grid_for(w * h, 256, 4096);
diff --git a/hikari.jl_amd/csrc/hk_render.cpp b/hikari.jl_amd/csrc/hk_render.cpp
--- a/hikari.jl_amd/csrc/hk_render.cpp
+++ b/hikari.jl_amd/csrc/hk_render.cpp
@@ -326,6 +326,8 @@
     s.hi_rows = s.hi_stride = 0;
     s.lo_table = nullptr;
     s.lo_rows = s.lo_count = s.lo_offset = 0;
+    s.val = nullptr;
+    s.val_depths = s.val_lobe = 0;
     return s;
 }
 
@@ -385,7 +387,7 @@
     }
     return HK_OK;
 }
-int ensure_sobol_tables(hk_ctx* c, hk_integrator* I, const DFrame& fr, DSobol& sob, int first_sample_idx, int n_samples, int sample_stride) {
+int ensure_sobol_tables(hk_ctx* c, hk_integrator* I, const DFrame& fr, DSobol& sob, int first_sample_idx, int n_samples, int sample_stride, bool want_lobe) {
     const int x0 = fr.x0, y0 = fr.y0;
     const int rows = 4 + 5 * (I->p.max_depth + 1);
     const bool table_same = !(I->sobol_rows != rows || I->sobol_stride != fr.n_pixels_padded || I->sobol_log2 != sob.log2_spp || I->sobol_digits != sob.n_base4_digits ||
@@ -449,6 +451,61 @@
             sob.lo_count = I->lo_count;
         }
     }
+    if (sob.lo_table != nullptr && hk::knob_int("HK_SOBOL_DRAWS", 1) != 0 && hk::knob_on("HK_SOBOL_TABLE_ONLY")) {
+        double gb = 48.0;
+        if (const char* e = hk::knob("HK_SOBOL_DRAW_GB")) gb = std::atof(e);
+        char key[320];
+        std::snprintf(key, sizeof key, "%d %d %d %d %d %d %d %d|%d %d %d %d|%d %u %u %d|%d %.6g", rows, fr.n_pixels_padded, sob.log2_spp, sob.n_base4_digits, x0, y0, fr.tiles_x, sob.width,
+                      I->lo_base, I->lo_sample_stride, I->lo_count, I->lo_rows, I->p.max_depth, sob.seed, c->tables_epoch, c->tables.sobol == nullptr ? 1 : 0, want_lobe ? 1 : 0, gb);
+        if (I->val_key != key && (I->val_seen == key || I->val_seen2 == key)) {
+            const int lobe = want_lobe ? 1 : 0;
+            const size_t entries = (size_t)fr.n_pixels_padded * (size_t)I->lo_count, per_depth = (size_t)(6 + lobe) * entries * sizeof(float);
+            size_t budget = gb > 0.0 ? (size_t)(gb * 1e9) : 0, free_b = 0, total_b = 0;
+            if (hipMemGetInfo(&free_b, &total_b) == hipSuccess && (free_b + I->sobol_val.bytes) / 4 < budget) budget = (free_b + I->sobol_val.bytes) / 4;
+            int depths = (I->lo_rows - 5) / 5;
+            if (depths > I->p.max_depth) depths = I->p.max_depth;
+            if ((size_t)depths > budget / per_depth) depths = (int)(budget / per_depth);
+            if (depths > 0) {
+                if (c->lanes_dirty) {
+                    if (int e = join_lanes(c)) return e;
+                    HIP_TRY(hipStreamSynchronize(c->stream));
+                }
+                bool have_buf = true;
+                if (I->sobol_val.bytes < per_depth * depths || I->sobol_val.bytes > 2 * per_depth * depths) {
+                    I->val_key.clear();
+                    I->val_depths = 0;
+                    if (I->sobol_val.alloc(per_depth * depths) != hipSuccess) {
+                        (void)hipGetLastError();
+                        have_buf = false;
+                    }
+                }
+                if (have_buf) {
+                    DSobol b = sob;
+                    b.lo_offset = 0;
+                    b.val_lobe = lobe;
+                    for (int d = 0; d < depths; ++d)
+                        hk::launch_sobol_values(c->stream, b, fr, c->tables.sobol, I->sobol_val.as<float>() + (size_t)d * (per_depth / sizeof(float)), d, I->lo_base, I->lo_sample_stride);
+                    HIP_TRY(hipGetLastError());
+                    I->val_key = key;
+                    I->val_depths = depths;
+                    I->val_lobe = lobe;
+                    c->sobol_value_builds++;
+                }
+            }
+        }
+        if (I->val_seen != key) {
+            I->val_seen2 = I->val_seen;
+            I->val_seen = key;
+        }
+        if (I->val_key == key && I->val_depths > 0) {
+            sob.val = I->sobol_val.as<float>();
+            sob.val_depths = I->val_depths;
+            sob.val_lobe = I->val_lobe;
+        }
+    } else {
+        I->val_seen.clear();
+        I->val_seen2.clear();
+    }
     return HK_OK;
 }
 int detect_camera_medium(hipStream_t s, hk_integrator* I, const hk_scene* sc, const hk_camera* cam, DStats* dstats) {
@@ -627,6 +684,7 @@
         if (int e = timed(3, [&] { hk::launch_film(s, I->st, fr, c->tables, film->accum, film->f64); })) return e;
     if (vm) I->view_key = view_key;
     if (view_hit) c->view_cache_hits++;
+    if (sob.val != nullptr && !fused) c->sobol_value_passes++;
     if (piped) {
         HIP_TRY(hipEventRecord(c->ev_film, s));
         c->film_chain = true;
@@ -724,7 +782,7 @@
         fr.walk_tune = knob("HK_SHADOW_TRACK_BATCH", 8) | (knob("HK_TRACK_ADVANCE", 2) << 8) | (knob("HK_SHADOW_FEED_ROUNDS", 3) << 16) | ((knob("HK_WALK_REFILL_IDLE", 16) > 63 ? 63 : knob("HK_WALK_REFILL_IDLE", 16)) << 24);
     }
     DSobol sob = make_sobol(I->p, W, H);
-    if (int e = ensure_sobol_tables(c, I, fr, sob, first_sample_idx, n_samples, sample_stride)) return e;
+    if (int e = ensure_sobol_tables(c, I, fr, sob, first_sample_idx, n_samples, sample_stride, (sc->kinds_mask & (1u << HK_MAT_GLASS)) != 0)) return e;
     DCamera dc = make_camera(*cam);
     DStats* dstats = c->stats.as<DStats>();
     hipStream_t s = c->stream;
diff --git a/hikari.jl_amd/csrc/hk_types.h b/hikari.jl_amd/csrc/hk_types.h
--- a/hikari.jl_amd/csrc/hk_types.h
+++ b/hikari.jl_amd/csrc/hk_types.h
@@ -261,6 +261,8 @@
     const uint16_t* lo_table;
     int lo_rows, lo_count;
     int lo_offset;
+    const float* val;
+    int val_depths, val_lobe;
 };
 
 enum { Q_RAY = 0, Q_SHADOW = 1, Q_ESCAPED = 2, Q_MEDIUM = 3, Q_SCATTER = 4, Q_MAT0 = 5, Q_COUNT = Q_MAT0 + HK_MAX_KINDS };
diff --git a/include/hikari_mi355x.h b/include/hikari_mi355x.h
--- a/include/hikari_mi355x.h
+++ b/include/hikari_mi355x.h
@@ -236,6 +236,7 @@
     uint64_t select_launches;
     uint64_t fused_passes;
     uint64_t view_cache_hits;
+    uint64_t sobol_value_passes, sobol_value_builds;
 } hk_stats;
 
 typedef struct hk_ctx hk_ctx;
```

Result: no change. 10280 (-0.1%).
